# marvinli00/genie2

Hardware: AMD Instinct MI355X
Metric: denoise-steps/sec (N=256, T=1000, batch=8) (higher is better)
Workload: dtype f32 (pair-stack products as 3 f16 MFMAs on 2xf16-split operands, f32 accumulate); 1 GPU; unconditional N=256, T=1000, batch=8 per GPU, random-init base Denoiser (15.7M params), scale=0.6, reverse-loop steps 995..676; parallelism=replica per GPU x1, no data-path collective

## Files before the change

genie2_amd/csrc/common.h:

```cpp
#pragma once
#include <hip/hip_runtime.h>
#include <stdint.h>
#include "../../include/genie_hip.h"

typedef float f32x16 __attribute__((ext_vector_type(16)));
typedef float f32x4 __attribute__((ext_vector_type(4)));

#define GENIE_LN_EPS 1e-5f

#ifdef __HIPCC__

__device__ __forceinline__ f32x16 mfma_8k(const float4 a, const float4 b, f32x16 c) {
    c = __builtin_amdgcn_mfma_f32_32x32x2f32(a.x, b.x, c, 0, 0, 0);
    c = __builtin_amdgcn_mfma_f32_32x32x2f32(a.y, b.y, c, 0, 0, 0);
    c = __builtin_amdgcn_mfma_f32_32x32x2f32(a.z, b.z, c, 0, 0, 0);
    c = __builtin_amdgcn_mfma_f32_32x32x2f32(a.w, b.w, c, 0, 0, 0);
    return c;
}

__device__ __forceinline__ f32x16 zero16() {
    f32x16 z;
#pragma unroll
    for (int i = 0; i < 16; ++i) z[i] = 0.f;
    return z;
}

__device__ __forceinline__ int acc_row(int r, int lane) { return (r & 3) + 8 * (r >> 2) + 4 * (lane >> 5); }

__device__ __forceinline__ float4 wfrag(const float* __restrict__ wp, int KB, int nb, int kb, int lane) {
    return *reinterpret_cast<const float4*>(wp + ((size_t)(nb * KB + kb) * 64 + lane) * 4);
}

typedef float v4f __attribute__((ext_vector_type(4)));

__device__ __forceinline__ const float* wfrag_ptr(const float* __restrict__ wp, int KB, int nb, int kb, int lane) {
    return wp + ((size_t)(nb * KB + kb) * 64 + lane) * 4;
}
__device__ __forceinline__ void wf_issue(v4f& d, const float* p) {
    asm volatile("global_load_dwordx4 %0, %1, off" : "=v"(d) : "v"(p) : "memory");
}
template <int N>
__device__ __forceinline__ void wf_wait(v4f& a) {
    asm volatile("s_waitcnt vmcnt(%1)" : "+v"(a) : "i"(N) : "memory");
    __builtin_amdgcn_sched_barrier(0);
}
template <int N>
__device__ __forceinline__ void wf_wait(v4f& a, v4f& b) {
    asm volatile("s_waitcnt vmcnt(%2)" : "+v"(a), "+v"(b) : "i"(N) : "memory");
    __builtin_amdgcn_sched_barrier(0);
}
__device__ __forceinline__ f32x16 mfma_8k(const v4f a, const float4 b, f32x16 c) {
    c = __builtin_amdgcn_mfma_f32_32x32x2f32(a.x, b.x, c, 0, 0, 0);
    c = __builtin_amdgcn_mfma_f32_32x32x2f32(a.y, b.y, c, 0, 0, 0);
    c = __builtin_amdgcn_mfma_f32_32x32x2f32(a.z, b.z, c, 0, 0, 0);
    c = __builtin_amdgcn_mfma_f32_32x32x2f32(a.w, b.w, c, 0, 0, 0);
    return c;
}
__device__ __forceinline__ f32x16 mfma_8k(const float4 a, const v4f b, f32x16 c) {
    c = __builtin_amdgcn_mfma_f32_32x32x2f32(a.x, b.x, c, 0, 0, 0);
    c = __builtin_amdgcn_mfma_f32_32x32x2f32(a.y, b.y, c, 0, 0, 0);
    c = __builtin_amdgcn_mfma_f32_32x32x2f32(a.z, b.z, c, 0, 0, 0);
    c = __builtin_amdgcn_mfma_f32_32x32x2f32(a.w, b.w, c, 0, 0, 0);
    return c;
}

__device__ __forceinline__ float4 lfrag(const float* lds, int ld, int r0, int kb, int lane) {
    return *reinterpret_cast<const float4*>(lds + (r0 + (lane & 31)) * ld + kb * 8 + 4 * (lane >> 5));
}

__device__ __forceinline__ float4 lfrag_t(const float* lds, int ld, int i0, int kb, int lane) {
    const float* p = lds + (kb * 8 + 4 * (lane >> 5)) * ld + i0 + (lane & 31);
    return make_float4(p[0], p[ld], p[2 * ld], p[3 * ld]);
}

__device__ __forceinline__ float sigmoidf_(float x) { return 1.0f / (1.0f + expf(-x)); }

__device__ __forceinline__ void ln_rows_128(float* tile, int ld, const float* __restrict__ gamma,
                                            const float* __restrict__ beta, int tid) {
    const int row = tid >> 2, part = tid & 3;
    float* p = tile + row * ld + part * 32;
    float v[32];
#pragma unroll
    for (int q = 0; q < 8; ++q) {
        float4 t = *reinterpret_cast<float4*>(p + 4 * q);
        v[4 * q] = t.x; v[4 * q + 1] = t.y; v[4 * q + 2] = t.z; v[4 * q + 3] = t.w;
    }
    float s = 0.f;
#pragma unroll
    for (int q = 0; q < 32; ++q) s += v[q];
    s += __shfl_xor(s, 1); s += __shfl_xor(s, 2);
    const float mean = s * (1.0f / 128.0f);
    float ss = 0.f;
#pragma unroll
    for (int q = 0; q < 32; ++q) { float d = v[q] - mean; ss += d * d; }
    ss += __shfl_xor(ss, 1); ss += __shfl_xor(ss, 2);
    const float rstd = 1.0f / sqrtf(ss * (1.0f / 128.0f) + GENIE_LN_EPS);
#pragma unroll
    for (int q = 0; q < 8; ++q) {
        const int c = part * 32 + 4 * q;
        float4 g = *reinterpret_cast<const float4*>(gamma + c);
        float4 b = *reinterpret_cast<const float4*>(beta + c);
        float4 o;
        o.x = (v[4 * q] - mean) * rstd * g.x + b.x;
        o.y = (v[4 * q + 1] - mean) * rstd * g.y + b.y;
        o.z = (v[4 * q + 2] - mean) * rstd * g.z + b.z;
        o.w = (v[4 * q + 3] - mean) * rstd * g.w + b.w;
        *reinterpret_cast<float4*>(p + 4 * q) = o;
    }
}


__device__ __forceinline__ void rot_to_quat_dev(const float* r, int code, float* q) {
    const float xx = r[0], xy = r[1], xz = r[2], yx = r[3], yy = r[4], yz = r[5], zx = r[6], zy = r[7], zz = r[8];
    const float d0 = 1.f + xx + yy + zz, d1 = 1.f + xx - yy - zz, d2 = 1.f + yy - xx - zz, d3 = 1.f + zz - xx - yy;
    float c0, c1, c2, c3;
    if (d0 >= d1 && d0 >= d2 && d0 >= d3)      { c0 = d0;      c1 = zy - yz; c2 = xz - zx; c3 = yx - xy; }
    else if (d1 >= d2 && d1 >= d3)             { c0 = zy - yz; c1 = d1;      c2 = xy + yx; c3 = xz + zx; }
    else if (d2 >= d3)                         { c0 = xz - zx; c1 = xy + yx; c2 = d2;      c3 = yz + zy; }
    else                                       { c0 = yx - xy; c1 = xz + zx; c2 = yz + zy; c3 = d3; }
    const float inv = 1.0f / sqrtf(c0 * c0 + c1 * c1 + c2 * c2 + c3 * c3);
    q[0] = c0 * inv; q[1] = c1 * inv; q[2] = c2 * inv; q[3] = c3 * inv;
    if (code > 0) {
        const int m = (code - 1) >> 1;
        const bool want_neg = ((code - 1) & 1) != 0;
        const float comp = q[m];
        if ((comp < 0.f) != want_neg) { q[0] = -q[0]; q[1] = -q[1]; q[2] = -q[2]; q[3] = -q[3]; }
    }
}

#endif


enum KernelClass {
    KC_SINGLE_INPUT = 0, KC_GEMM_ROWS, KC_LAYERNORM, KC_PAIR_STATIC, KC_PAIR_INIT,
    KC_TRIMUL_PROJ, KC_TRIMUL_CONTRACT, KC_TRIMUL_OUT, KC_PAIR_TRANSITION,
    KC_IPA_BIAS, KC_IPA_PREP, KC_IPA_ATTN, KC_BB_UPDATE, KC_STRUCT_ROWS, KC_P_SAMPLE, KC_MISC, KC_PAIR_FUSED_A, KC_PAIR_FUSED_B,
    KC_TR_GEMM, KC_TR_EW, KC_TR_LN, KC_TR_TRANSPOSE, KC_TR_IPA, KC_TR_MISC,
    KC_TRIATT_PROJ, KC_TRIATT_CORE, KC_TRIATT_TRANSPOSE, KC_COUNT
};

struct HxTransW { const unsigned char* img; float *b1s, *b2s; float sx, c1, c2; };

struct HxTriW {
    const unsigned char *img_proj, *img_out;
    float *bias_proj, *bgs, *bzs;
    float sx, cpa, cpb, cg, cx, cgo, cz;
};
struct HxFusedW { const unsigned char* img; };
struct TriMulW {
    float *proj_w;
    float *proj_b;
    float *g_w, *g_b;
    float *z_w, *z_b;
    float *ln_in_g, *ln_in_b, *ln_out_g, *ln_out_b;
    HxTriW hx;
};
struct TriAttW {
    float *ln_g, *ln_b;
    float *wb;
    float *proj_w, *proj_b;
    float *out_w, *out_b;
    float sq, sk, sv;
};
struct PairLayerW {
    TriMulW out, in;
    TriAttW ta_start, ta_end;
    float *pt_ln_g, *pt_ln_b, *pt_w1, *pt_b1, *pt_w2, *pt_b2;
    HxTransW hx_pt;
    HxFusedW fa, fb;
};
struct StructLayerW {
    float *proj_w, *proj_b;
    float *head_w;
    float *out_w, *out_b;
    float *ln_ipa_g, *ln_ipa_b;
    float *t1_w, *t1_b, *t2_w, *t2_b, *t3_w, *t3_b;
    float *ln_tr_g, *ln_tr_b;
    float *bb_w, *bb_b;
};

struct HxGemmW { const float* w; const unsigned char* img; float inv_s; };

struct genie_train_ws;
struct genie_ctx {
    genie_dims_t d;
    genie_train_ws* train;
    int device;
    char err[512];

    bool have_weights;
    float* wdev;
    bool hx;
    unsigned char* hxdev;
    HxGemmW hxg[128]; int n_hxg;
    unsigned hx_launches;
    size_t wdev_floats;
    float *single_w;
    float *pij_w;
    float *relpos_t;
    float *templ_w;
    float *motif_w;
    float *ipa_bias_w, *ipa_bias_b;
    PairLayerW* pair;
    StructLayerW* st;

    bool have_tables;
    float *pos_tab, *chain_tab, *t_tab, *sched;
    int n_pos, n_chain;
    float* sched_host;

    int B, N, NP;
    bool have_feats, has_motif;
    int32_t *f_aatype, *f_rmask, *f_ridx, *f_cidx;
    float *f_pos;
    uint8_t *f_fsm, *f_fstm, *f_ifm;
    float *rmaskf;

    void* ws; size_t ws_bytes;
    float *p, *acm, *bcm, *xcm, *pstatic, *ipa_bias;
    float *spart;
    unsigned *pmax;
    float *xsingle, *s0, *s, *s1, *s2, *h1, *h2, *pij, *proj, *cat;
    float *kT, *v, *qp, *kpT, *vp;
    float *vf, *vmax;
    float *ta_tb, *ta_xn, *ta_qkvg;
    float *rots_w, *trans_w;
    int32_t* tsteps;
    float *loop_z;

    bool prof;
    struct ProfRec { int cls; hipEvent_t a, b; };
    ProfRec* prof_recs; int prof_n, prof_cap;
    double prof_ms[KC_COUNT]; int64_t prof_cnt[KC_COUNT];
    double train_gemm_flop;

    hipStream_t st2; hipEvent_t ev_fork, ev_join;
};

void launch_single_input(genie_ctx* h, hipStream_t st, const int32_t* timesteps);
void launch_gemm_rows(genie_ctx* h, hipStream_t st, const float* A, int lda, int M, int K,
                      const float* Wp, int Nout, const float* bias, const float* res, int ldr,
                      const float* rowmask, int relu, float* out, int ldo, int prof_class = KC_GEMM_ROWS);
void launch_layernorm_rows(genie_ctx* h, hipStream_t st, const float* in, float* out, int M, int C,
                           const float* g, const float* b);
void launch_pair_static(genie_ctx* h, hipStream_t st);
void launch_pair_init(genie_ctx* h, hipStream_t st, const float* trans, const float* rots,
                      const int8_t* codes);
void launch_trimul(genie_ctx* h, hipStream_t st, const TriMulW& w, bool outgoing);
void launch_pair_transition(genie_ctx* h, hipStream_t st, const PairLayerW& w);
void launch_triatt(genie_ctx* h, hipStream_t st, const TriAttW& w, bool starting);
void triatt_ws_floats(const genie_dims_t& d, int B, int N, size_t* tb, size_t* xn, size_t* qkvg);
bool launch_pair_stack_fused(genie_ctx* h, hipStream_t st, float* tap_trimul_out0, float* tap_layer0);
void launch_ipa_bias(genie_ctx* h, hipStream_t st);
void launch_ipa_prep(genie_ctx* h, hipStream_t st, int b0 = 0, int nb = -1);
void launch_ipa_attn(genie_ctx* h, hipStream_t st, int layer, const float* head_w, int b0 = 0, int nb = -1);
size_t ipa_vf_floats(const genie_dims_t& d, int B, int N);
bool ipa_attn_splits(const genie_ctx* h);
void launch_q_sample(genie_ctx* h, hipStream_t st, const float* x0, const float* z, const float* c0, const float* c1, float* trans_out);
void launch_training_loss(genie_ctx* h, hipStream_t st, const float* zp, const float* z, float w, float* losses, float* grad);
void launch_adam(hipStream_t st, size_t n, float* p, const float* g, float* m, float* v, double lr, double b1, double b2, double eps, int step);
void launch_any_nonzero(genie_ctx* h, hipStream_t st, const uint8_t* x, size_t n, unsigned* flag);
bool launch_struct_tail(genie_ctx* h, hipStream_t st, const StructLayerW& S, const float* trans_in, float* z_out, int b0 = 0, int nb = -1);
bool struct_tail_fused(const genie_ctx* h, const StructLayerW& S);
void launch_bb_update(genie_ctx* h, hipStream_t st, const StructLayerW& w, const float* trans_in,
                      float* z_out);
void launch_frenet(genie_ctx* h, hipStream_t st, int mode, int step, float scale, float* trans,
                   float* rots, const float* z, const float* eps);
void launch_reverse_step(genie_ctx* h, hipStream_t st, float a, float bz, float c_scaled, float* trans, float* rots, const float* z,
                         const float* eps);
void launch_fill_i32(genie_ctx* h, hipStream_t st, int32_t* p, int n, int v);
void train_ws_free(genie_ctx* h);

void prof_begin(genie_ctx* h, hipStream_t st, int cls);
void prof_end(genie_ctx* h, hipStream_t st);

struct ProfScope {
    genie_ctx* h; hipStream_t st; bool on;
    ProfScope(genie_ctx* h_, hipStream_t st_, int cls, bool enable = true) : h(h_), st(st_), on(enable && h_->prof) { if (on) prof_begin(h, st, cls); }
    ~ProfScope() { if (on) prof_end(h, st); }
};
```

genie2_amd/csrc/genie_api.hip:

```cpp
#include <stdio.h>
#include <stdlib.h>
#include <string.h>
#include <math.h>
#include <algorithm>
#include <cmath>
#include <new>
#include <string>
#include <vector>

#include "common.h"

void pair_kernels_init();
void pair_fused_kernels_init();
void single_kernels_init(const genie_dims_t& d, int n_max);
void launch_scale_copy(genie_ctx* h, hipStream_t st, const float* in, float* out, int n, float s);
size_t ipa_attn_lds(const genie_dims_t& d, int N);

static char g_create_err[512] = "";

void set_handle_free_error(const char* msg) { snprintf(g_create_err, sizeof g_create_err, "%s", msg); }

#define SET_ERR(h, ...) do { snprintf((h)->err, sizeof((h)->err), __VA_ARGS__); } while (0)
#define HIP_TRY(h, call) do { hipError_t e_ = (call); if (e_ != hipSuccess) { \
    SET_ERR(h, "%s failed: %s (%s:%d)", #call, hipGetErrorString(e_), __FILE__, __LINE__); return GENIE_E_HIP; } } while (0)

static const char* kKernelNames[KC_COUNT] = {
    "single_input", "gemm_rows", "layernorm_rows", "pair_static", "pair_init", "trimul_proj", "trimul_contract",
    "trimul_out", "pair_transition", "ipa_bias", "ipa_prep", "ipa_attn", "bb_update", "struct_rows", "p_sample_frenet", "misc",
    "pair_fused_a", "pair_fused_b", "train_gemm", "train_elementwise", "train_layernorm", "train_transpose", "train_ipa", "train_misc",
    "tri_att_proj", "tri_att_core", "tri_att_transpose"};

void prof_begin(genie_ctx* h, hipStream_t st, int cls) {
    if (h->prof_n == h->prof_cap) {
        const int nc = h->prof_cap ? h->prof_cap * 2 : 1024;
        h->prof_recs = (genie_ctx::ProfRec*)realloc(h->prof_recs, nc * sizeof(genie_ctx::ProfRec));
        h->prof_cap = nc;
    }
    genie_ctx::ProfRec& r = h->prof_recs[h->prof_n];
    r.cls = cls;
    (void)hipEventCreate(&r.a);
    (void)hipEventCreate(&r.b);
    (void)hipEventRecord(r.a, st);
}
void prof_end(genie_ctx* h, hipStream_t st) {
    (void)hipEventRecord(h->prof_recs[h->prof_n].b, st);
    h->prof_n++;
}

static int single_in(const genie_dims_t& d) { return d.c_pos_emb + d.c_chain_emb + d.c_timestep_emb + 23; }
static int ipa_proj_n(const genie_dims_t& d) {
    return d.n_head_ipa * (3 * d.c_hidden_ipa + 3 * d.n_qk_point + 3 * (d.n_qk_point + d.n_v_point));
}
static int ipa_cat_n(const genie_dims_t& d) { return d.n_head_ipa * (d.c_p + d.c_hidden_ipa + 4 * d.n_v_point); }

static const char* check_dims(const genie_dims_t& d) {
    if (d.c_p != 128 || d.c_hidden_mul != 128) return "kernels are specialised for c_p == c_hidden_mul == 128";
    if (d.c_s % 8 || d.c_s > 512) return "c_s must be a multiple of 8 and <= 512";
    if (d.template_dist_n_bin > 40 || d.template_dist_n_bin < 1) return "template_dist_n_bin must be in [1, 40]";
    if (d.n_head_ipa > 16) return "n_head_ipa must be <= 16";
    if (d.pair_transition_n < 1 || d.n_timestep < 1 || d.relpos_k < 0) return "bad dims";
    if (d.n_structure_layer < 1 || d.n_structure_block < 1 || d.n_pair_transform_layer < 0) return "bad layer counts";
    if ((d.n_head_ipa * d.c_hidden_ipa) % 4 || ipa_cat_n(d) % 4 || ipa_proj_n(d) % 4) return "IPA widths must be multiples of 4";
    if (d.n_head_tri < 0) return "n_head_tri must be >= 0";
    if (d.n_head_tri > 0 && d.c_hidden_tri_att != 16 && d.c_hidden_tri_att != 32) return "c_hidden_tri_att must be 16 or 32";
    if (d.n_head_tri > 0 && d.n_head_tri * d.c_hidden_tri_att != 128) return "n_head_tri * c_hidden_tri_att must be 128 (4 heads of 32 or 8 of 16)";
    return nullptr;
}

size_t genie_weight_count(const genie_dims_t* dp) {
    const genie_dims_t& d = *dp;
    size_t n = 0;
    const size_t cs = d.c_s, cp = d.c_p, ch = d.c_hidden_mul;
    n += cs * single_in(d);
    n += 2 * cp * cs + cp * (2 * d.relpos_k + 3) + cp * (d.template_dist_n_bin + 6) + cp * (d.template_dist_n_bin + 2);
    const size_t tm = 4 * (ch * cp + ch) + (cp * cp + cp) + (cp * ch + cp) + 2 * cp + 2 * ch;
    const size_t pt = 2 * cp + (d.pair_transition_n * cp * cp + d.pair_transition_n * cp) + (cp * d.pair_transition_n * cp + cp);
    const size_t hc = (size_t)d.n_head_tri * d.c_hidden_tri_att;
    const size_t ta = d.n_head_tri > 0 ? 2 * cp + d.n_head_tri * cp + 3 * hc * cp + (cp * hc + cp) + (hc * cp + hc) : 0;
    n += (size_t)d.n_pair_transform_layer * (2 * tm + 2 * ta + pt);
    const size_t H = d.n_head_ipa, C = d.c_hidden_ipa, Pq = d.n_qk_point, Pv = d.n_v_point;
    size_t sl = H;
    sl += (H * C) * cs + H * C + (2 * H * C) * cs + 2 * H * C + (3 * H * Pq) * cs + 3 * H * Pq + (3 * H * (Pq + Pv)) * cs + 3 * H * (Pq + Pv);
    sl += H * cp + H + cs * ipa_cat_n(d) + cs;
    sl += 2 * cs + 3 * (cs * cs + cs) + 2 * cs + 6 * cs + 6;
    n += (size_t)d.n_structure_layer * sl;
    return n;
}

int genie_create(const genie_dims_t* dims, int device, genie_handle_t* out) {
    if (!dims || !out) { snprintf(g_create_err, sizeof g_create_err, "genie_create: null argument"); return GENIE_E_ARG; }
    if (const char* m = check_dims(*dims)) { snprintf(g_create_err, sizeof g_create_err, "genie_create: %s", m); return GENIE_E_ARG; }
    int ndev = 0;
    if (hipGetDeviceCount(&ndev) != hipSuccess || device < 0 || device >= ndev) {
        snprintf(g_create_err, sizeof g_create_err, "genie_create: no HIP device %d (found %d)", device, ndev);
        return GENIE_E_HIP;
    }
    genie_ctx* h = new (std::nothrow) genie_ctx();
    if (!h) return GENIE_E_NOMEM;
    memset(h, 0, sizeof(*h));
    h->d = *dims;
    h->device = device;
    if (hipSetDevice(device) != hipSuccess) { delete h; snprintf(g_create_err, sizeof g_create_err, "hipSetDevice failed"); return GENIE_E_HIP; }
    h->pair = new PairLayerW[dims->n_pair_transform_layer > 0 ? dims->n_pair_transform_layer : 1]();
    h->st = new StructLayerW[dims->n_structure_layer]();
    pair_kernels_init();
    pair_fused_kernels_init();
    {
        const char* m = getenv("GENIE_MATH");
        h->hx = !(m && !strcmp(m, "f32"));
    }
    {
        int lo = 0, hi = 0;
        (void)hipDeviceGetStreamPriorityRange(&lo, &hi);
        if (hipStreamCreateWithPriority(&h->st2, hipStreamNonBlocking, hi) != hipSuccess) h->st2 = nullptr;
    }
    if (h->st2 && (hipEventCreateWithFlags(&h->ev_fork, hipEventDisableTiming) != hipSuccess ||
                   hipEventCreateWithFlags(&h->ev_join, hipEventDisableTiming) != hipSuccess)) {
        (void)hipStreamDestroy(h->st2);
        h->st2 = nullptr;
    }
    *out = h;
    return GENIE_OK;
}

static void free_batch(genie_ctx* h) {
    if (h->ws) { (void)hipFree(h->ws); h->ws = nullptr; h->ws_bytes = 0; }
    h->have_feats = false;
}

void genie_destroy(genie_handle_t h) {
    if (!h) return;
    (void)hipSetDevice(h->device);
    free_batch(h);
    train_ws_free(h);
    if (h->wdev) (void)hipFree(h->wdev);
    if (h->hxdev) (void)hipFree(h->hxdev);
    if (h->pos_tab) (void)hipFree(h->pos_tab);
    free(h->sched_host);
    for (int i = 0; i < h->prof_n; ++i) { (void)hipEventDestroy(h->prof_recs[i].a); (void)hipEventDestroy(h->prof_recs[i].b); }
    free(h->prof_recs);
    if (h->st2) { (void)hipStreamSynchronize(h->st2); (void)hipEventDestroy(h->ev_fork); (void)hipEventDestroy(h->ev_join); (void)hipStreamDestroy(h->st2); }
    delete[] h->pair;
    delete[] h->st;
    delete h;
}

const char* genie_last_error(genie_handle_t h) { return h ? h->err : g_create_err; }
size_t genie_workspace_bytes(genie_handle_t h) { return h ? h->ws_bytes : 0; }

namespace {
struct Img {
    std::vector<float> data;
    size_t add(size_t n) {
        const size_t off = (data.size() + 63) & ~(size_t)63;
        data.resize(off + n, 0.f);
        return off;
    }
    size_t raw(const float* src, size_t n) { const size_t o = add(n); memcpy(&data[o], src, n * sizeof(float)); return o; }
    size_t pack(const float* W, int rows, int cols) {
        const int NB = (rows + 31) / 32, KB = (cols + 7) / 8;
        const size_t o = add((size_t)NB * KB * 256);
        float* p = &data[o];
        for (int nb = 0; nb < NB; ++nb)
            for (int kb = 0; kb < KB; ++kb)
                for (int lane = 0; lane < 64; ++lane)
                    for (int e = 0; e < 4; ++e) {
                        const int r = nb * 32 + (lane & 31), k = kb * 8 + 4 * (lane >> 5) + e;
                        p[(((size_t)nb * KB + kb) * 64 + lane) * 4 + e] = (r < rows && k < cols) ? W[(size_t)r * cols + k] : 0.f;
                    }
        return o;
    }
};
uint16_t f2h(float f) {
    uint32_t x; memcpy(&x, &f, 4);
    const uint16_t sign = (uint16_t)((x >> 16) & 0x8000);
    x &= 0x7FFFFFFFu;
    if (x >= 0x7F800000u) return (uint16_t)(sign | (x > 0x7F800000u ? 0x7E00 : 0x7C00));
    if (x >= 0x477FF000u) return (uint16_t)(sign | 0x7C00);
    if (x < 0x38800000u) {
        float a; memcpy(&a, &x, 4);
        return (uint16_t)(sign | (uint16_t)nearbyintf(a * 16777216.0f));
    }
    const uint32_t mant = x & 0x7FFFFFu, rem = mant & 0x1FFFu;
    uint32_t r = (((x >> 23) - 112u) << 10) | (mant >> 13);
    if (rem > 0x1000u || (rem == 0x1000u && (r & 1u))) ++r;
    return (uint16_t)(sign | r);
}
float h2f(uint16_t v) {
    const int e = (v >> 10) & 31, m = v & 1023;
    float r = e == 0 ? ldexpf((float)m, -24) : e == 31 ? (m ? NAN : INFINITY) : ldexpf((float)(1024 + m), e - 25);
    return (v & 0x8000) ? -r : r;
}
float p2floor(double x) { return (x > 0 && std::isfinite(x)) ? (float)ldexp(1.0, (int)floor(log2(x))) : 1.0f; }
struct HxImg {
    std::vector<uint16_t> d;
    size_t begin() { d.resize((d.size() + 127) & ~(size_t)127); return d.size() * 2; }
    template <class F> void unit(F get) {
        const size_t o = d.size();
        d.resize(o + 1024);
        for (int lane = 0; lane < 64; ++lane)
            for (int e = 0; e < 8; ++e) {
                const float v = get(lane & 31, lane >> 5, e);
                const uint16_t hi = f2h(v);
                d[o + lane * 8 + e] = hi;
                d[o + 512 + lane * 8 + e] = f2h(v - h2f(hi));
            }
    }
};
double max_abs(const float* w, size_t n) { double m = 0; for (size_t i = 0; i < n; ++i) m = std::max(m, (double)fabsf(w[i])); return m; }
double hx_bound(const float* W, const float* b, int rows, int cols) {
    double m = 0;
    for (int r = 0; r < rows; ++r) {
        double ss = 0;
        for (int k = 0; k < cols; ++k) ss += (double)W[(size_t)r * cols + k] * W[(size_t)r * cols + k];
        m = std::max(m, sqrt(ss * cols) + fabs((double)b[r]));
    }
    return m;
}
constexpr float HX_SX = 1024.0f;

struct Cur {
    const float* p; size_t left;
    const float* take(size_t n) { if (n > left) { left = 0; return nullptr; } const float* r = p; p += n; left -= n; return r; }
};
void fold_ln(std::vector<float>& W, std::vector<float>& b, int rows, int cols, const float* g, const float* beta) {
    for (int r = 0; r < rows; ++r) {
        double acc = b[r];
        for (int k = 0; k < cols; ++k) acc += (double)W[(size_t)r * cols + k] * beta[k];
        b[r] = (float)acc;
        for (int k = 0; k < cols; ++k) W[(size_t)r * cols + k] *= g[k];
    }
}
std::vector<float> vcat(std::initializer_list<std::pair<const float*, size_t>> parts) {
    std::vector<float> v;
    for (auto& pr : parts) v.insert(v.end(), pr.first, pr.first + pr.second);
    return v;
}
}

int genie_load_weights(genie_handle_t h, const float* blob, size_t n_floats) {
    if (!h || !blob) return GENIE_E_ARG;
    const genie_dims_t& d = h->d;
    if (n_floats != genie_weight_count(&d)) {
        SET_ERR(h, "genie_load_weights: got %zu floats, dims need %zu", n_floats, genie_weight_count(&d));
        return GENIE_E_ARG;
    }
    HIP_TRY(h, hipSetDevice(h->device));
    const size_t cs = d.c_s, cp = d.c_p, ch = d.c_hidden_mul;
    Cur c{blob, n_floats};
    Img img;
    HxImg hx;
    std::vector<std::pair<float**, size_t>> fix;
    std::vector<std::pair<const unsigned char**, size_t>> hxfix;
    auto slot = [&](float** s, size_t off) { fix.push_back({s, off}); };
    struct GemmFix { float** slot; size_t hx_off; float inv_s; };
    std::vector<GemmFix> gfix;
    auto pack_gemm = [&](float** s, const float* W, int rows, int cols) {
        slot(s, img.pack(W, rows, cols));
        const float sw = p2floor(16384.0 / max_abs(W, (size_t)rows * cols));
        gfix.push_back({s, hx.begin(), 1.0f / sw});
        const int NB = (rows + 31) / 32, KC = (cols + 15) / 16;
        for (int nb = 0; nb < NB; ++nb)
            for (int kc = 0; kc < KC; ++kc)
                hx.unit([&](int j, int hh, int e) {
                    const int r = 32 * nb + j, k = 16 * kc + 8 * hh + e;
                    return (r < rows && k < cols) ? W[(size_t)r * cols + k] * sw : 0.f; });
    };

    size_t ones_off, zeros_off;
    {
        std::vector<float> one(512, 1.f), zero(512, 0.f);
        ones_off = img.raw(one.data(), one.size());
        zeros_off = img.raw(zero.data(), zero.size());
    }
    const int nsi = single_in(d);
    pack_gemm(&h->single_w, c.take(cs * nsi), (int)cs, nsi);
    {
        const float* wi = c.take(cp * cs);
        const float* wj = c.take(cp * cs);
        auto v = vcat({{wi, cp * cs}, {wj, cp * cs}});
        pack_gemm(&h->pij_w, v.data(), (int)(2 * cp), (int)cs);
    }
    {
        const int nr = 2 * d.relpos_k + 3;
        const float* w = c.take(cp * nr);
        std::vector<float> t((size_t)nr * cp);
        for (int o = 0; o < (int)cp; ++o) for (int k = 0; k < nr; ++k) t[(size_t)k * cp + o] = w[(size_t)o * nr + k];
        slot(&h->relpos_t, img.raw(t.data(), t.size()));
    }
    {
        const int kt = d.template_dist_n_bin + 6, km = d.template_dist_n_bin + 2;
        const float* wt = c.take(cp * kt);
        const float* wm = c.take(cp * km);
        std::vector<float> t((size_t)cp * 48, 0.f), m((size_t)cp * 48, 0.f);
        for (int o = 0; o < (int)cp; ++o) {
            for (int k = 0; k < kt; ++k) t[(size_t)o * 48 + k] = wt[(size_t)o * kt + k];
            for (int k = 0; k < km; ++k) m[(size_t)o * 48 + k] = wm[(size_t)o * km + k];
        }
        slot(&h->templ_w, img.pack(t.data(), (int)cp, 48));
        slot(&h->motif_w, img.pack(m.data(), (int)cp, 48));
    }
    struct TmSave { std::vector<float> w, gw, zw; float sp, sg, sgo, szo; };
    struct PtSave { std::vector<float> w1v, w2; float s1, s2; };
    std::vector<TmSave> tm_save(2 * (size_t)d.n_pair_transform_layer);
    std::vector<PtSave> pt_save(d.n_pair_transform_layer);
    for (int l = 0; l < d.n_pair_transform_layer; ++l) {
        PairLayerW& L = h->pair[l];
        for (int dir = 0; dir < 2; ++dir) {
            TriMulW& T = dir == 0 ? L.out : L.in;
            const float* ap_w = c.take(ch * cp); const float* ap_b = c.take(ch);
            const float* ag_w = c.take(ch * cp); const float* ag_b = c.take(ch);
            const float* bp_w = c.take(ch * cp); const float* bp_b = c.take(ch);
            const float* bg_w = c.take(ch * cp); const float* bg_b = c.take(ch);
            const float* g_w = c.take(cp * cp);  const float* g_b = c.take(cp);
            const float* z_w = c.take(cp * ch);  const float* z_b = c.take(cp);
            const float* li_g = c.take(cp); const float* li_b = c.take(cp);
            const float* lo_g = c.take(ch); const float* lo_b = c.take(ch);
            auto w = vcat({{ap_w, ch * cp}, {bp_w, ch * cp}, {ag_w, ch * cp}, {bg_w, ch * cp}});
            auto bb = vcat({{ap_b, ch}, {bp_b, ch}, {ag_b, ch}, {bg_b, ch}});
            fold_ln(w, bb, (int)(4 * ch), (int)cp, li_g, li_b);
            for (size_t r = 2 * ch; r < 4 * ch; ++r) {
                bb[r] = (float)(-1.4426950408889634 * bb[r]);
                for (size_t k = 0; k < cp; ++k) w[r * cp + k] = (float)(-1.4426950408889634 * w[r * cp + k]);
            }
            std::vector<float> gw(g_w, g_w + cp * cp), gb(g_b, g_b + cp), zw(z_w, z_w + cp * ch), zb(z_b, z_b + cp);
            fold_ln(gw, gb, (int)cp, (int)cp, li_g, li_b);
            for (size_t r = 0; r < cp; ++r) {
                gb[r] = (float)(-1.4426950408889634 * gb[r]);
                for (size_t k = 0; k < cp; ++k) gw[r * cp + k] = (float)(-1.4426950408889634 * gw[r * cp + k]);
            }
            fold_ln(zw, zb, (int)cp, (int)ch, lo_g, lo_b);
            slot(&T.proj_w, img.pack(w.data(), (int)(4 * ch), (int)cp));
            slot(&T.proj_b, img.raw(bb.data(), bb.size()));
            slot(&T.g_w, img.pack(gw.data(), (int)cp, (int)cp)); slot(&T.g_b, img.raw(gb.data(), cp));
            slot(&T.z_w, img.pack(zw.data(), (int)cp, (int)ch)); slot(&T.z_b, img.raw(zb.data(), cp));
            {
                HxTriW& X = T.hx;
                const float sp = p2floor(16384.0 / max_abs(w.data(), 2 * ch * cp)), sg = p2floor(16384.0 / max_abs(w.data() + 2 * ch * cp, 2 * ch * cp));
                const float sa = p2floor(32768.0 / hx_bound(w.data(), bb.data(), (int)ch, (int)cp));
                const float sb = p2floor(32768.0 / hx_bound(w.data() + ch * cp, bb.data() + ch, (int)ch, (int)cp));
                const float sgo = p2floor(16384.0 / max_abs(gw.data(), cp * cp)), szo = p2floor(16384.0 / max_abs(zw.data(), cp * ch));
                X.sx = HX_SX; X.cpa = sa / (HX_SX * sp); X.cpb = sb / (HX_SX * sp); X.cg = 1.0f / (HX_SX * sg); X.cx = 1.0f / (sa * sb);
                X.cgo = 1.0f / (HX_SX * sgo); X.cz = 1.0f / (HX_SX * szo);
                hxfix.push_back({&X.img_proj, hx.begin()});
                for (size_t pass = 0; pass < 8; ++pass)
                    for (int kc = 0; kc < 8; ++kc) {
                        hx.unit([&](int i, int hh, int e) { return w[(32 * pass + i) * cp + 16 * kc + 8 * hh + e] * sp; });
                        hx.unit([&](int i, int hh, int e) { return w[(2 * ch + 32 * pass + i) * cp + 16 * kc + 8 * hh + e] * sg; });
                    }
                hxfix.push_back({&X.img_out, hx.begin()});
                for (int st = 0; st < 4; ++st)
                    for (int obl = 0; obl < 2; ++obl)
                        for (int kc = 0; kc < 8; ++kc) {
                            const std::vector<float>& m = (st & 1) ? zw : gw;
                            const float sc = (st & 1) ? szo : sgo;
                            const size_t ob = 2 * (st >> 1) + obl;
                            hx.unit([&](int j, int hh, int e) { return m[(32 * ob + j) * cp + 16 * kc + 8 * hh + e] * sc; });
                        }
                std::vector<float> bp(4 * ch), bgs(cp), bzs(cp);
                for (size_t r = 0; r < 4 * ch; ++r) bp[r] = bb[r] * HX_SX * (r < 2 * ch ? sp : sg);
                for (size_t r = 0; r < cp; ++r) { bgs[r] = gb[r] * HX_SX * sgo; bzs[r] = zb[r] * HX_SX * szo; }
                slot(&X.bias_proj, img.raw(bp.data(), bp.size()));
                slot(&X.bgs, img.raw(bgs.data(), cp)); slot(&X.bzs, img.raw(bzs.data(), cp));
                tm_save[2 * l + dir] = TmSave{w, gw, zw, sp, sg, sgo, szo};
            }
            slot(&T.ln_in_g, ones_off); slot(&T.ln_in_b, zeros_off);
            slot(&T.ln_out_g, ones_off); slot(&T.ln_out_b, zeros_off);
        }
        for (int node = 0; node < (d.n_head_tri > 0 ? 2 : 0); ++node) {
            TriAttW& A = node == 0 ? L.ta_start : L.ta_end;
            const size_t hc = (size_t)d.n_head_tri * d.c_hidden_tri_att;
            const float* ln_g = c.take(cp); const float* ln_b = c.take(cp);
            const float* b_w = c.take(d.n_head_tri * cp);
            const float* q_w = c.take(hc * cp); const float* k_w = c.take(hc * cp); const float* v_w = c.take(hc * cp);
            const float* o_w = c.take(cp * hc); const float* o_b = c.take(cp);
            const float* g_w = c.take(hc * cp); const float* g_b = c.take(hc);
            if (!g_b) { SET_ERR(h, "genie_load_weights: blob too short"); return GENIE_E_ARG; }
            slot(&A.ln_g, img.raw(ln_g, cp)); slot(&A.ln_b, img.raw(ln_b, cp));
            slot(&A.wb, img.raw(b_w, d.n_head_tri * cp));
            auto w = vcat({{q_w, hc * cp}, {k_w, hc * cp}, {v_w, hc * cp}, {g_w, hc * cp}});
            std::vector<float> bv(4 * hc, 0.f);
            memcpy(&bv[3 * hc], g_b, hc * sizeof(float));
            pack_gemm(&A.proj_w, w.data(), (int)(4 * hc), (int)cp);
            slot(&A.proj_b, img.raw(bv.data(), bv.size()));
            pack_gemm(&A.out_w, o_w, (int)cp, (int)hc); slot(&A.out_b, img.raw(o_b, cp));
            auto scale_of = [&](const float* W) {
                std::vector<float> wf(W, W + hc * cp), bf(hc, 0.f);
                fold_ln(wf, bf, (int)hc, (int)cp, ln_g, ln_b);
                return p2floor(32768.0 / hx_bound(wf.data(), bf.data(), (int)hc, (int)cp));
            };
            A.sq = scale_of(q_w); A.sk = scale_of(k_w); A.sv = scale_of(v_w);
        }
        const size_t nh = (size_t)d.pair_transition_n * cp;
        const float* lg = c.take(cp); const float* lb = c.take(cp);
        const float* w1 = c.take(nh * cp); const float* b1 = c.take(nh);
        const float* w2 = c.take(cp * nh); const float* b2 = c.take(cp);
        {
            std::vector<float> w1v(w1, w1 + nh * cp), b1v(b1, b1 + nh);
            fold_ln(w1v, b1v, (int)nh, (int)cp, lg, lb);
            slot(&L.pt_ln_g, ones_off); slot(&L.pt_ln_b, zeros_off);
            slot(&L.pt_w1, img.pack(w1v.data(), (int)nh, (int)cp)); slot(&L.pt_b1, img.raw(b1v.data(), nh));
            HxTransW& X = L.hx_pt;
            const float s1 = p2floor(16384.0 / max_abs(w1v.data(), nh * cp)), s2 = p2floor(16384.0 / max_abs(w2, cp * nh));
            const float sh = p2floor(32768.0 / hx_bound(w1v.data(), b1v.data(), (int)nh, (int)cp));
            X.sx = HX_SX; X.c1 = sh / (HX_SX * s1); X.c2 = 1.0f / (sh * s2);
            hxfix.push_back({&X.img, hx.begin()});
            for (size_t hb = 0; hb < nh / 32; ++hb) {
                for (int kc = 0; kc < 8; ++kc)
                    hx.unit([&](int i, int hh, int e) { return w1v[(32 * hb + i) * cp + 16 * kc + 8 * hh + e] * s1; });
                for (int cc = 0; cc < 2; ++cc)
                    for (int ob = 0; ob < 4; ++ob)
                        hx.unit([&](int j, int hh, int e) {
                            return w2[(size_t)(32 * ob + j) * nh + 32 * hb + 16 * cc + (e & 3) + 8 * (e >> 2) + 4 * hh] * s2; });
            }
            std::vector<float> b1s(nh), b2s(cp);
            for (size_t r = 0; r < nh; ++r) b1s[r] = b1v[r] * HX_SX * s1;
            for (size_t r = 0; r < cp; ++r) b2s[r] = b2[r] * sh * s2;
            slot(&X.b1s, img.raw(b1s.data(), nh)); slot(&X.b2s, img.raw(b2s.data(), cp));
            pt_save[l] = PtSave{w1v, std::vector<float>(w2, w2 + cp * nh), s1, s2};
        }
        slot(&L.pt_w2, img.pack(w2, (int)cp, (int)nh)); slot(&L.pt_b2, img.raw(b2, cp));
    }
    {
        auto ck = [](int kc, int hh, int e) { return 16 * kc + (e & 3) + 8 * (e >> 2) + 4 * hh; };
        auto emit_O = [&](const TmSave& t) {
            for (int which = 0; which < 2; ++which)
                for (int st = 0; st < 2; ++st)
                    for (int obl = 0; obl < 2; ++obl)
                        for (int kc = 0; kc < 8; ++kc) {
                            const std::vector<float>& m = which == 0 ? t.zw : t.gw;
                            const float sc = which == 0 ? t.szo : t.sgo;
                            const size_t ob = 2 * st + obl;
                            hx.unit([&](int i, int hh, int e) { return m[(32 * ob + i) * cp + ck(kc, hh, e)] * sc; });
                        }
        };
        auto emit_T = [&](const PtSave& t) {
            const size_t nh = (size_t)d.pair_transition_n * cp;
            for (size_t hb = 0; hb < nh / 32; ++hb) {
                for (int kc = 0; kc < 8; ++kc)
                    hx.unit([&](int i, int hh, int e) { return t.w1v[(32 * hb + i) * cp + ck(kc, hh, e)] * t.s1; });
                for (int cc = 0; cc < 2; ++cc)
                    for (int ob = 0; ob < 4; ++ob)
                        hx.unit([&](int j, int hh, int e) { return t.w2[(size_t)(32 * ob + j) * nh + 32 * hb + ck(cc, hh, e)] * t.s2; });
            }
        };
        auto emit_P = [&](const TmSave& t) {
            for (size_t pass = 0; pass < 8; ++pass)
                for (int kc = 0; kc < 8; ++kc) {
                    hx.unit([&](int i, int hh, int e) { return t.w[(32 * pass + i) * cp + ck(kc, hh, e)] * t.sp; });
                    hx.unit([&](int i, int hh, int e) { return t.w[(2 * ch + 32 * pass + i) * cp + ck(kc, hh, e)] * t.sg; });
                }
        };
        for (int l = 0; l < d.n_pair_transform_layer; ++l) {
            hxfix.push_back({&h->pair[l].fa.img, hx.begin()});
            emit_O(tm_save[2 * l]); emit_P(tm_save[2 * l + 1]);
            hxfix.push_back({&h->pair[l].fb.img, hx.begin()});
            emit_O(tm_save[2 * l + 1]); emit_T(pt_save[l]);
            if (l + 1 < d.n_pair_transform_layer) emit_P(tm_save[2 * l + 2]);
        }
    }
    const size_t H = d.n_head_ipa, C = d.c_hidden_ipa, Pq = d.n_qk_point, Pv = d.n_v_point;
    const size_t ncat = ipa_cat_n(d);
    std::vector<float> wb_all, bb_all;
    for (int l = 0; l < d.n_structure_layer; ++l) {
        StructLayerW& S = h->st[l];
        const float* hw = c.take(H);
        const float* q_w = c.take(H * C * cs);            const float* q_b = c.take(H * C);
        const float* kv_w = c.take(2 * H * C * cs);       const float* kv_b = c.take(2 * H * C);
        const float* qp_w = c.take(3 * H * Pq * cs);      const float* qp_b = c.take(3 * H * Pq);
        const float* kp_w = c.take(3 * H * (Pq + Pv) * cs); const float* kp_b = c.take(3 * H * (Pq + Pv));
        const float* b_w = c.take(H * cp);                const float* b_b = c.take(H);
        const float* o_w = c.take(cs * ncat);             const float* o_b = c.take(cs);
        const float* li_g = c.take(cs); const float* li_b = c.take(cs);
        const float* t1w = c.take(cs * cs); const float* t1b = c.take(cs);
        const float* t2w = c.take(cs * cs); const float* t2b = c.take(cs);
        const float* t3w = c.take(cs * cs); const float* t3b = c.take(cs);
        const float* lt_g = c.take(cs); const float* lt_b = c.take(cs);
        const float* bw = c.take(6 * cs); const float* bbs = c.take(6);
        if (!bbs) { SET_ERR(h, "genie_load_weights: blob too short"); return GENIE_E_ARG; }
        slot(&S.head_w, img.raw(hw, H));
        auto w = vcat({{q_w, H * C * cs}, {kv_w, 2 * H * C * cs}, {qp_w, 3 * H * Pq * cs}, {kp_w, 3 * H * (Pq + Pv) * cs}});
        auto bv = vcat({{q_b, H * C}, {kv_b, 2 * H * C}, {qp_b, 3 * H * Pq}, {kp_b, 3 * H * (Pq + Pv)}});
        pack_gemm(&S.proj_w, w.data(), ipa_proj_n(d), (int)cs);
        slot(&S.proj_b, img.raw(bv.data(), bv.size()));
        wb_all.insert(wb_all.end(), b_w, b_w + H * cp);
        bb_all.insert(bb_all.end(), b_b, b_b + H);
        pack_gemm(&S.out_w, o_w, (int)cs, (int)ncat); slot(&S.out_b, img.raw(o_b, cs));
        slot(&S.ln_ipa_g, img.raw(li_g, cs)); slot(&S.ln_ipa_b, img.raw(li_b, cs));
        pack_gemm(&S.t1_w, t1w, (int)cs, (int)cs); slot(&S.t1_b, img.raw(t1b, cs));
        pack_gemm(&S.t2_w, t2w, (int)cs, (int)cs); slot(&S.t2_b, img.raw(t2b, cs));
        pack_gemm(&S.t3_w, t3w, (int)cs, (int)cs); slot(&S.t3_b, img.raw(t3b, cs));
        slot(&S.ln_tr_g, img.raw(lt_g, cs)); slot(&S.ln_tr_b, img.raw(lt_b, cs));
        slot(&S.bb_w, img.raw(bw, 6 * cs)); slot(&S.bb_b, img.raw(bbs, 6));
    }
    pack_gemm(&h->ipa_bias_w, wb_all.data(), (int)(d.n_structure_layer * H), (int)cp);
    slot(&h->ipa_bias_b, img.raw(bb_all.data(), bb_all.size()));
    if (c.left != 0) { SET_ERR(h, "genie_load_weights: %zu floats left over", c.left); return GENIE_E_ARG; }

    if (h->wdev) { (void)hipFree(h->wdev); h->wdev = nullptr; }
    img.add(64);
    HIP_TRY(h, hipMalloc((void**)&h->wdev, img.data.size() * sizeof(float)));
    HIP_TRY(h, hipMemcpy(h->wdev, img.data.data(), img.data.size() * sizeof(float), hipMemcpyHostToDevice));
    h->wdev_floats = img.data.size();
    for (auto& f : fix) *f.first = h->wdev + f.second;
    if (h->hxdev) { (void)hipFree(h->hxdev); h->hxdev = nullptr; }
    hx.begin();
    HIP_TRY(h, hipMalloc((void**)&h->hxdev, hx.d.size() * 2 + 256));
    HIP_TRY(h, hipMemcpy(h->hxdev, hx.d.data(), hx.d.size() * 2, hipMemcpyHostToDevice));
    for (auto& f : hxfix) *f.first = h->hxdev + f.second;
    h->n_hxg = 0;
    const int hxg_cap = (int)(sizeof(h->hxg) / sizeof(h->hxg[0]));
    if ((int)gfix.size() > hxg_cap) { SET_ERR(h, "genie_load_weights: %zu row-GEMM weights exceed the %d hx image slots", gfix.size(), hxg_cap); return GENIE_E_ARG; }
    for (auto& g : gfix) h->hxg[h->n_hxg++] = HxGemmW{*g.slot, h->hxdev + g.hx_off, g.inv_s};
    h->have_weights = true;
    return GENIE_OK;
}

int genie_set_tables(genie_handle_t h, const float* pos_tab, int n_pos, const float* chain_tab, int n_chain,
                     const float* t_tab, const float* sched) {
    if (!h || !pos_tab || !chain_tab || !t_tab || !sched || n_pos < 1 || n_chain < 1) return GENIE_E_ARG;
    HIP_TRY(h, hipSetDevice(h->device));
    const genie_dims_t& d = h->d;
    const size_t T1 = d.n_timestep + 1;
    const size_t a = (size_t)n_pos * d.c_pos_emb, b = (size_t)n_chain * d.c_chain_emb, c = T1 * d.c_timestep_emb, s = 4 * T1;
    if (h->pos_tab) (void)hipFree(h->pos_tab);
    HIP_TRY(h, hipMalloc((void**)&h->pos_tab, (a + b + c + s) * sizeof(float)));
    h->chain_tab = h->pos_tab + a;
    h->t_tab = h->chain_tab + b;
    h->sched = h->t_tab + c;
    HIP_TRY(h, hipMemcpy(h->pos_tab, pos_tab, a * sizeof(float), hipMemcpyHostToDevice));
    HIP_TRY(h, hipMemcpy(h->chain_tab, chain_tab, b * sizeof(float), hipMemcpyHostToDevice));
    HIP_TRY(h, hipMemcpy(h->t_tab, t_tab, c * sizeof(float), hipMemcpyHostToDevice));
    HIP_TRY(h, hipMemcpy(h->sched, sched, s * sizeof(float), hipMemcpyHostToDevice));
    free(h->sched_host);
    h->sched_host = (float*)malloc(s * sizeof(float));
    memcpy(h->sched_host, sched, s * sizeof(float));
    h->n_pos = n_pos;
    h->n_chain = n_chain;
    h->have_tables = true;
    return GENIE_OK;
}

__global__ void k_mask_to_float(const int32_t* m, float* f, int n) {
    const int i = blockIdx.x * blockDim.x + threadIdx.x;
    if (i < n) f[i] = (float)m[i];
}

int genie_prepare_features(genie_handle_t h, genie_stream_t stream, int B, int N, const genie_features_t* f) {
    if (!h || !f || B < 1 || N < 2) return GENIE_E_ARG;
    if (!h->have_weights) { SET_ERR(h, "genie_prepare_features: weights not loaded"); return GENIE_E_STATE; }
    const genie_dims_t& d = h->d;
    if (ipa_attn_lds(d, N) > 160 * 1024) { SET_ERR(h, "N = %d exceeds the attention kernel's LDS budget", N); return GENIE_E_ARG; }
    if ((size_t)24 * N * sizeof(float) > 160 * 1024) { SET_ERR(h, "N = %d exceeds the Frenet kernel's LDS budget (96 B per residue)", N); return GENIE_E_ARG; }
    {
        const size_t np = (size_t)((N + 31) / 32 * 32);
        const size_t pair_bytes = (size_t)B * np * np * d.c_p * sizeof(float);
        if (pair_bytes >= ((size_t)1 << 31)) {
            SET_ERR(h, "batch %d x N %d: a pair tensor of %zu bytes exceeds the 2 GiB the kernels address; split the batch", B, N, pair_bytes);
            return GENIE_E_ARG;
        }
    }
    HIP_TRY(h, hipSetDevice(h->device));
    hipStream_t st = (hipStream_t)stream;
    const int NP = (N + 31) / 32 * 32;
    const size_t M = (size_t)B * N, P = M * N;
    const size_t cs = d.c_s, cp = d.c_p;
    const int H = d.n_head_ipa, C = d.c_hidden_ipa, Pq = d.n_qk_point, Pv = d.n_v_point;
    const int ldx = (single_in(d) + 7) / 8 * 8;

    struct Seg { void** p; size_t bytes; };
    std::vector<Seg> segs;
    auto want = [&](void* pp, size_t bytes) { segs.push_back({(void**)pp, (bytes + 255) & ~(size_t)255}); };
    want(&h->p, P * cp * 4); want(&h->pstatic, P * cp * 4);
    want(&h->acm, (size_t)B * cp * NP * NP * 4); want(&h->bcm, (size_t)B * cp * NP * NP * 4); want(&h->xcm, (size_t)B * cp * NP * NP * 4);
    want(&h->ipa_bias, (size_t)d.n_structure_layer * H * P * 4);
    want(&h->xsingle, M * ldx * 4);
    want(&h->s0, M * cs * 4); want(&h->s, M * cs * 4); want(&h->s1, M * cs * 4); want(&h->s2, M * cs * 4);
    want(&h->h1, M * cs * 4); want(&h->h2, M * cs * 4);
    want(&h->pij, M * 2 * cp * 4); want(&h->proj, M * ipa_proj_n(d) * 4); want(&h->cat, M * ipa_cat_n(d) * 4);
    want(&h->kT, M * H * C * 4); want(&h->v, M * H * C * 4); want(&h->qp, M * H * Pq * 3 * 4);
    want(&h->kpT, M * H * Pq * 3 * 4); want(&h->vp, M * H * Pv * 3 * 4);
    want(&h->vf, ipa_vf_floats(d, B, N) * 4); want(&h->vmax, M * 2 * 4);
    want(&h->rots_w, M * 9 * 4); want(&h->trans_w, M * 3 * 4); want(&h->loop_z, M * 3 * 4);
    want(&h->tsteps, (size_t)B * 4); want(&h->rmaskf, M * 4); want(&h->pmax, 4); want(&h->spart, 3 * M * cs * 4);
    want(&h->f_aatype, M * 20 * 4); want(&h->f_rmask, M * 4); want(&h->f_ridx, M * 4); want(&h->f_cidx, M * 4);
    want(&h->f_pos, M * 3 * 4); want(&h->f_fsm, M); want(&h->f_fstm, P); want(&h->f_ifm, M);
    if (d.n_head_tri > 0) {
        size_t ntb, nxn, nq;
        triatt_ws_floats(d, B, N, &ntb, &nxn, &nq);
        want(&h->ta_tb, ntb * 4); want(&h->ta_xn, nxn * 4); want(&h->ta_qkvg, nq * 4);
    }
    size_t total = 0;
    for (auto& s : segs) total += s.bytes;
    if (total > h->ws_bytes) {
        free_batch(h);
        hipError_t e = hipMalloc(&h->ws, total);
        if (e != hipSuccess) { SET_ERR(h, "workspace hipMalloc(%zu MB) failed: %s", total >> 20, hipGetErrorString(e)); return GENIE_E_NOMEM; }
        h->ws_bytes = total;
    }
    size_t off = 0;
    for (auto& s : segs) { *s.p = (char*)h->ws + off; off += s.bytes; }
    h->B = B; h->N = N; h->NP = NP;

    HIP_TRY(h, hipMemcpyAsync(h->f_aatype, f->aatype, M * 20 * 4, hipMemcpyDeviceToDevice, st));
    HIP_TRY(h, hipMemcpyAsync(h->f_pos, f->atom_positions, M * 3 * 4, hipMemcpyDeviceToDevice, st));
    HIP_TRY(h, hipMemcpyAsync(h->f_rmask, f->residue_mask, M * 4, hipMemcpyDeviceToDevice, st));
    HIP_TRY(h, hipMemcpyAsync(h->f_ridx, f->residue_index, M * 4, hipMemcpyDeviceToDevice, st));
    HIP_TRY(h, hipMemcpyAsync(h->f_cidx, f->chain_index, M * 4, hipMemcpyDeviceToDevice, st));
    HIP_TRY(h, hipMemcpyAsync(h->f_fsm, f->fixed_sequence_mask, M, hipMemcpyDeviceToDevice, st));
    HIP_TRY(h, hipMemcpyAsync(h->f_fstm, f->fixed_structure_mask, P, hipMemcpyDeviceToDevice, st));
    HIP_TRY(h, hipMemcpyAsync(h->f_ifm, f->interface_mask, M, hipMemcpyDeviceToDevice, st));
    hipLaunchKernelGGL(k_mask_to_float, dim3((unsigned)((M + 255) / 256)), dim3(256), 0, st, h->f_rmask, h->rmaskf, (int)M);
    HIP_TRY(h, hipMemsetAsync(h->acm, 0, (size_t)B * cp * NP * NP * 4, st));
    HIP_TRY(h, hipMemsetAsync(h->vf, 0, ipa_vf_floats(d, B, N) * 4, st));
    HIP_TRY(h, hipMemsetAsync(h->bcm, 0, (size_t)B * cp * NP * NP * 4, st));
    single_kernels_init(d, N);
    {
        unsigned any = 0;
        HIP_TRY(h, hipMemsetAsync(h->pmax, 0, sizeof(unsigned), st));
        launch_any_nonzero(h, st, h->f_fstm, P, h->pmax);
        HIP_TRY(h, hipMemcpyAsync(&any, h->pmax, sizeof(unsigned), hipMemcpyDeviceToHost, st));
        HIP_TRY(h, hipStreamSynchronize(st));
        h->has_motif = any != 0;
    }
    launch_pair_static(h, st);
    HIP_TRY(h, hipGetLastError());
    h->have_feats = true;
    return GENIE_OK;
}

static int denoise_internal(genie_ctx* h, hipStream_t st, const float* trans, const float* rots, const int32_t* ts_dev,
                            const int8_t* codes, float* z_out, const genie_taps_t* taps) {
    const genie_dims_t& d = h->d;
    const int B = h->B, N = h->N, M = B * N;
    const size_t P = (size_t)M * N;
    const int cs = d.c_s, cp = d.c_p;
    const int ldx = (single_in(d) + 7) / 8 * 8;
    auto d2d = [&](void* dst, const void* src, size_t bytes) { return hipMemcpyAsync(dst, src, bytes, hipMemcpyDeviceToDevice, st); };

    h->hx_launches = 1;
    launch_scale_copy(h, st, trans, h->trans_w, M * 3, d.rescale);
    HIP_TRY(h, d2d(h->rots_w, rots, (size_t)M * 9 * 4));

    launch_single_input(h, st, ts_dev);
    launch_gemm_rows(h, st, h->xsingle, ldx, M, ldx, h->single_w, cs, nullptr, nullptr, 0, h->rmaskf, 0, h->s0, cs);
    if (taps && taps->s) HIP_TRY(h, d2d(taps->s, h->s0, (size_t)M * cs * 4));

    launch_gemm_rows(h, st, h->s0, cs, M, cs, h->pij_w, 2 * cp, nullptr, nullptr, 0, nullptr, 0, h->pij, 2 * cp);
    launch_pair_init(h, st, h->trans_w, h->rots_w, codes);
    if (taps && taps->p_init) HIP_TRY(h, d2d(taps->p_init, h->p, P * cp * 4));

    const bool fused = launch_pair_stack_fused(h, st, taps ? taps->p_trimul_out0 : nullptr, taps ? taps->p_layer0 : nullptr);
    for (int l = 0; l < (fused ? 0 : d.n_pair_transform_layer); ++l) {
        launch_trimul(h, st, h->pair[l].out, true);
        if (l == 0 && taps && taps->p_trimul_out0) HIP_TRY(h, d2d(taps->p_trimul_out0, h->p, P * cp * 4));
        launch_trimul(h, st, h->pair[l].in, false);
        if (d.n_head_tri > 0) {
            launch_triatt(h, st, h->pair[l].ta_start, true);
            launch_triatt(h, st, h->pair[l].ta_end, false);
            if (l == 0 && taps && taps->p_tri_att0) HIP_TRY(h, d2d(taps->p_tri_att0, h->p, P * cp * 4));
        }
        launch_pair_transition(h, st, h->pair[l]);
        if (l == 0 && taps && taps->p_layer0) HIP_TRY(h, d2d(taps->p_layer0, h->p, P * cp * 4));
    }
    if (taps && taps->p) HIP_TRY(h, d2d(taps->p, h->p, P * cp * 4));

    launch_ipa_bias(h, st);
    HIP_TRY(h, d2d(h->s, h->s0, (size_t)M * cs * 4));
    if (taps && taps->states) HIP_TRY(h, d2d(taps->states, h->s0, (size_t)M * cs * 4));
    int n_state = 1;
    const int nproj = ipa_proj_n(d), ncat = ipa_cat_n(d);
    bool split = h->st2 && B >= 2 && M >= 1024 && ipa_attn_splits(h) && !getenv("GENIE_NO_STRUCT_SPLIT");
    for (int l = 0; split && l < d.n_structure_layer; ++l) split = struct_tail_fused(h, h->st[l]);
    const int n_half = split ? 2 : 1;
    const int n_layers = d.n_structure_block * d.n_structure_layer;
    hipStream_t hstream[2] = {st, h->st2};
    if (split) {
        HIP_TRY(h, hipEventRecord(h->ev_fork, st));
        HIP_TRY(h, hipStreamWaitEvent(h->st2, h->ev_fork, 0));
    }
    for (int half = 0; half < n_half; ++half) {
        hipStream_t hs = hstream[half];
        const int b0 = (int)((long long)B * half / n_half), nb = (int)((long long)B * (half + 1) / n_half) - b0;
        const size_t r0 = (size_t)b0 * N, nr = (size_t)nb * N;
        int li = 0;
        for (int blk = 0; blk < d.n_structure_block; ++blk) {
            for (int l = 0; l < d.n_structure_layer; ++l, ++li) {
                const StructLayerW& S = h->st[l];
                const bool last = li == n_layers - 1;
                launch_gemm_rows(h, hs, h->s + r0 * cs, cs, (int)nr, cs, S.proj_w, nproj, S.proj_b, nullptr, 0, nullptr, 0, h->proj + r0 * nproj, nproj);
                launch_ipa_prep(h, hs, b0, nb);
                launch_ipa_attn(h, hs, l, S.head_w, b0, nb);
                if (li == 0 && taps && taps->ipa_cat0) HIP_TRY(h, hipMemcpyAsync(taps->ipa_cat0 + r0 * ncat, h->cat + r0 * ncat, nr * ncat * 4, hipMemcpyDeviceToDevice, hs));
                auto state_tap = [&]() -> hipError_t {
                    return (taps && taps->states) ? hipMemcpyAsync(taps->states + (size_t)(1 + li) * M * cs + r0 * cs, h->s + r0 * cs, nr * cs * 4, hipMemcpyDeviceToDevice, hs)
                                                  : hipSuccess;
                };
                if (launch_struct_tail(h, hs, S, last ? trans : nullptr, last ? z_out : nullptr, b0, nb)) { HIP_TRY(h, state_tap()); continue; }
                launch_gemm_rows(h, hs, h->cat, ncat, M, ncat, S.out_w, cs, S.out_b, h->s, cs, nullptr, 0, h->s1, cs);
                launch_layernorm_rows(h, hs, h->s1, h->s2, M, cs, S.ln_ipa_g, S.ln_ipa_b);
                launch_gemm_rows(h, hs, h->s2, cs, M, cs, S.t1_w, cs, S.t1_b, nullptr, 0, nullptr, 1, h->h1, cs);
                launch_gemm_rows(h, hs, h->h1, cs, M, cs, S.t2_w, cs, S.t2_b, nullptr, 0, nullptr, 1, h->h2, cs);
                launch_gemm_rows(h, hs, h->h2, cs, M, cs, S.t3_w, cs, S.t3_b, h->s2, cs, nullptr, 0, h->s1, cs);
                launch_layernorm_rows(h, hs, h->s1, h->s, M, cs, S.ln_tr_g, S.ln_tr_b);
                launch_bb_update(h, hs, S, last ? trans : nullptr, last ? z_out : nullptr);
                HIP_TRY(h, state_tap());
            }
        }
    }
    if (split) {
        for (int q = 1; q < n_half; ++q) {
            HIP_TRY(h, hipEventRecord(h->ev_join, hstream[q]));
            HIP_TRY(h, hipStreamWaitEvent(st, h->ev_join, 0));
        }
    }
    (void)n_state;
    if (taps && taps->s_final) HIP_TRY(h, d2d(taps->s_final, h->s, (size_t)M * cs * 4));
    if (taps && taps->rots_out) HIP_TRY(h, d2d(taps->rots_out, h->rots_w, (size_t)M * 9 * 4));
    if (taps && taps->trans_out) launch_scale_copy(h, st, h->trans_w, taps->trans_out, M * 3, 1.0f / d.rescale);
    HIP_TRY(h, hipGetLastError());
    return GENIE_OK;
}

static int check_ready(genie_ctx* h, const char* who) {
    if (!h) return GENIE_E_ARG;
    if (!h->have_weights || !h->have_tables || !h->have_feats) {
        SET_ERR(h, "%s: call genie_load_weights, genie_set_tables and genie_prepare_features first", who);
        return GENIE_E_STATE;
    }
    if (hipSetDevice(h->device) != hipSuccess) { SET_ERR(h, "hipSetDevice failed"); return GENIE_E_HIP; }
    return GENIE_OK;
}

int genie_denoise(genie_handle_t h, genie_stream_t stream, const float* trans, const float* rots, const int32_t* timesteps,
                  const int8_t* quat_codes, float* z_out, const genie_taps_t* taps) {
    if (int rc = check_ready(h, "genie_denoise")) return rc;
    if (!trans || !rots || !timesteps || !z_out) { SET_ERR(h, "genie_denoise: null tensor"); return GENIE_E_ARG; }
    return denoise_internal(h, (hipStream_t)stream, trans, rots, timesteps, quat_codes, z_out, taps);
}

int genie_frenet(genie_handle_t h, genie_stream_t stream, const float* trans, float* rots_out) {
    if (!h || !h->have_feats) { if (h) SET_ERR(h, "genie_frenet: no batch bound"); return h ? GENIE_E_STATE : GENIE_E_ARG; }
    if (!trans || !rots_out) return GENIE_E_ARG;
    HIP_TRY(h, hipSetDevice(h->device));
    launch_frenet(h, (hipStream_t)stream, 0, 0, 0.f, const_cast<float*>(trans), rots_out, nullptr, nullptr);
    HIP_TRY(h, hipGetLastError());
    return GENIE_OK;
}

int genie_adam_step(genie_stream_t stream, size_t n, float* p, const float* g, float* m, float* v, double lr, double beta1, double beta2,
                    double eps, int step) {
    if (!p || !g || !m || !v || step < 1) return GENIE_E_ARG;
    if (n == 0) return GENIE_OK;
    launch_adam((hipStream_t)stream, n, p, g, m, v, lr, beta1, beta2, eps, step);
    return hipGetLastError() == hipSuccess ? GENIE_OK : GENIE_E_HIP;
}

int genie_q_sample(genie_handle_t h, genie_stream_t stream, const float* x0, const float* z, const float* c_x0, const float* c_z,
                   float* trans_out, float* rots_out) {
    if (!h || !h->have_feats) { if (h) SET_ERR(h, "genie_q_sample: no batch bound"); return h ? GENIE_E_STATE : GENIE_E_ARG; }
    if (!x0 || !z || !c_x0 || !c_z || !trans_out || !rots_out) { SET_ERR(h, "genie_q_sample: null tensor"); return GENIE_E_ARG; }
    HIP_TRY(h, hipSetDevice(h->device));
    launch_q_sample(h, (hipStream_t)stream, x0, z, c_x0, c_z, trans_out);
    launch_frenet(h, (hipStream_t)stream, 0, 0, 0.f, trans_out, rots_out, nullptr, nullptr);
    HIP_TRY(h, hipGetLastError());
    return GENIE_OK;
}

int genie_training_loss(genie_handle_t h, genie_stream_t stream, const float* z_pred, const float* z, float condition_loss_weight,
                        float* losses_out, float* grad_out) {
    if (!h || !h->have_feats) { if (h) SET_ERR(h, "genie_training_loss: no batch bound"); return h ? GENIE_E_STATE : GENIE_E_ARG; }
    if (!z_pred || !z || !losses_out) { SET_ERR(h, "genie_training_loss: null tensor"); return GENIE_E_ARG; }
    HIP_TRY(h, hipSetDevice(h->device));
    launch_training_loss(h, (hipStream_t)stream, z_pred, z, condition_loss_weight, losses_out, grad_out);
    HIP_TRY(h, hipGetLastError());
    return GENIE_OK;
}

int genie_p_sample(genie_handle_t h, genie_stream_t stream, int step, float scale, float* trans_inout, float* rots_out,
                   const float* z, const float* eps) {
    if (int rc = check_ready(h, "genie_p_sample")) return rc;
    if (step < 1 || step > h->d.n_timestep || !trans_inout || !rots_out || !z) { SET_ERR(h, "genie_p_sample: bad argument"); return GENIE_E_ARG; }
    launch_frenet(h, (hipStream_t)stream, 1, step, scale, trans_inout, rots_out, z, eps);
    HIP_TRY(h, hipGetLastError());
    return GENIE_OK;
}

int genie_sample_loop(genie_handle_t h, genie_stream_t stream, float scale, const float* noise, const int8_t* quat_codes,
                      int first_step, int last_step, float* trans_io, float* rots_io, float* record) {
    if (int rc = check_ready(h, "genie_sample_loop")) return rc;
    const int T = h->d.n_timestep;
    if (!noise || !trans_io || !rots_io || first_step > T || last_step < 1 || first_step < last_step) {
        SET_ERR(h, "genie_sample_loop: bad argument");
        return GENIE_E_ARG;
    }
    hipStream_t st = (hipStream_t)stream;
    const size_t n3 = (size_t)h->B * h->N * 3, nn = (size_t)h->B * h->N * h->N;
    if (first_step == T) {
        HIP_TRY(h, hipMemcpyAsync(trans_io, noise, n3 * 4, hipMemcpyDeviceToDevice, st));
        launch_frenet(h, st, 0, 0, 0.f, trans_io, rots_io, nullptr, nullptr);
    }
    int it = 0;
    for (int step = first_step; step >= last_step; --step, ++it) {
        launch_fill_i32(h, st, h->tsteps, h->B, step);
        const int8_t* codes = quat_codes ? quat_codes + (size_t)it * nn : nullptr;
        if (int rc = denoise_internal(h, st, trans_io, rots_io, h->tsteps, codes, h->loop_z, nullptr)) return rc;
        const float* eps = (step == 1) ? nullptr : noise + (size_t)(T - step + 1) * n3;
        launch_frenet(h, st, 1, step, scale, trans_io, rots_io, h->loop_z, eps);
        if (record) HIP_TRY(h, hipMemcpyAsync(record + (size_t)it * n3, trans_io, n3 * 4, hipMemcpyDeviceToDevice, st));
    }
    HIP_TRY(h, hipGetLastError());
    return GENIE_OK;
}

int genie_reverse_step(genie_handle_t h, genie_stream_t stream, float a, float bz, float c_scaled, float* trans_inout, float* rots_out,
                       const float* z, const float* eps) {
    if (int rc = check_ready(h, "genie_reverse_step")) return rc;
    if (!trans_inout || !rots_out || !z) { SET_ERR(h, "genie_reverse_step: null tensor"); return GENIE_E_ARG; }
    if (!std::isfinite(a) || !std::isfinite(bz) || !std::isfinite(c_scaled)) {
        SET_ERR(h, "genie_reverse_step: non-finite coefficient (a = %g, bz = %g, c_scaled = %g)", a, bz, c_scaled);
        return GENIE_E_ARG;
    }
    launch_reverse_step(h, (hipStream_t)stream, a, bz, c_scaled, trans_inout, rots_out, z, eps);
    HIP_TRY(h, hipGetLastError());
    return GENIE_OK;
}

int genie_sample_loop_steps(genie_handle_t h, genie_stream_t stream, int n_iter, const int32_t* steps, const float* coef, const float* noise,
                            const int8_t* quat_codes, int start_from_noise, float* trans_io, float* rots_io, float* record) {
    if (int rc = check_ready(h, "genie_sample_loop_steps")) return rc;
    const int T = h->d.n_timestep;
    if (n_iter < 1) { SET_ERR(h, "genie_sample_loop_steps: n_iter = %d, needs at least 1", n_iter); return GENIE_E_ARG; }
    if (!steps || !coef || !trans_io || !rots_io) { SET_ERR(h, "genie_sample_loop_steps: null steps, coef, trans_io or rots_io"); return GENIE_E_ARG; }
    if (!noise && (start_from_noise || n_iter > 1)) {
        SET_ERR(h, "genie_sample_loop_steps: null noise (needed for the initial state and for every iteration but the last)");
        return GENIE_E_ARG;
    }
    for (int i = 0; i < n_iter; ++i) {
        if (steps[i] < 1 || steps[i] > T) { SET_ERR(h, "genie_sample_loop_steps: steps[%d] = %d outside 1..%d", i, steps[i], T); return GENIE_E_ARG; }
        if (i && steps[i] >= steps[i - 1]) {
            SET_ERR(h, "genie_sample_loop_steps: steps not strictly decreasing (steps[%d] = %d after %d)", i, steps[i], steps[i - 1]);
            return GENIE_E_ARG;
        }
        for (int k = 0; k < 3; ++k)
            if (!std::isfinite(coef[3 * i + k])) { SET_ERR(h, "genie_sample_loop_steps: non-finite coefficient coef[%d][%d]", i, k); return GENIE_E_ARG; }
    }
    hipStream_t st = (hipStream_t)stream;
    const size_t n3 = (size_t)h->B * h->N * 3, nn = (size_t)h->B * h->N * h->N;
    if (start_from_noise) {
        HIP_TRY(h, hipMemcpyAsync(trans_io, noise, n3 * 4, hipMemcpyDeviceToDevice, st));
        launch_frenet(h, st, 0, 0, 0.f, trans_io, rots_io, nullptr, nullptr);
    }
    for (int it = 0; it < n_iter; ++it) {
        launch_fill_i32(h, st, h->tsteps, h->B, steps[it]);
        const int8_t* codes = quat_codes ? quat_codes + (size_t)it * nn : nullptr;
        if (int rc = denoise_internal(h, st, trans_io, rots_io, h->tsteps, codes, h->loop_z, nullptr)) return rc;
        const float* eps = (it == n_iter - 1) ? nullptr : noise + (size_t)(it + 1) * n3;
        launch_reverse_step(h, st, coef[3 * it], coef[3 * it + 1], coef[3 * it + 2], trans_io, rots_io, h->loop_z, eps);
        if (record) HIP_TRY(h, hipMemcpyAsync(record + (size_t)it * n3, trans_io, n3 * 4, hipMemcpyDeviceToDevice, st));
    }
    HIP_TRY(h, hipGetLastError());
    return GENIE_OK;
}

int genie_set_math(genie_handle_t h, int mode) {
    if (!h || (mode != GENIE_MATH_F32 && mode != GENIE_MATH_HX)) return GENIE_E_ARG;
    h->hx = mode == GENIE_MATH_HX;
    return GENIE_OK;
}
int genie_get_math(genie_handle_t h) { return h && h->hx ? GENIE_MATH_HX : GENIE_MATH_F32; }

int genie_profile_enable(genie_handle_t h, int enable) {
    if (!h) return GENIE_E_ARG;
    h->prof = enable != 0;
    return GENIE_OK;
}

int genie_profile_read(genie_handle_t h, const char** names, double* total_ms, int64_t* launches, int cap) {
    if (!h) return GENIE_E_ARG;
    (void)hipSetDevice(h->device);
    for (int i = 0; i < h->prof_n; ++i) {
        genie_ctx::ProfRec& r = h->prof_recs[i];
        (void)hipEventSynchronize(r.b);
        float ms = 0.f;
        if (hipEventElapsedTime(&ms, r.a, r.b) == hipSuccess) { h->prof_ms[r.cls] += ms; h->prof_cnt[r.cls] += 1; }
        (void)hipEventDestroy(r.a);
        (void)hipEventDestroy(r.b);
    }
    h->prof_n = 0;
    int n = 0;
    for (int k = 0; k < KC_COUNT && n < cap; ++k) {
        if (names) names[n] = kKernelNames[k];
        if (total_ms) total_ms[n] = h->prof_ms[k];
        if (launches) launches[n] = h->prof_cnt[k];
        ++n;
    }
    for (int k = 0; k < KC_COUNT; ++k) { h->prof_ms[k] = 0; h->prof_cnt[k] = 0; }
    return n;
}
```

genie2_amd/csrc/hx_fused.h:

```cpp
#pragma once
#include "hx_pair.h"

#define FZ_SB_BZ 0
#define FZ_SB_BG 128
#define FZ_SB_B1 256
#define FZ_SB_B2 768
#define FZ_SB_BP 896
#define FZ_SB_FLOATS 1408
#define FZ_OOR 0x7FFFFFF0
#define FZ_COMPILER_FENCE() asm volatile("" ::: "memory")

struct FusedArgs {
    float* z; const float* xcm; const float* rmask; const unsigned char* wimg;
    const float *bzs, *bgs, *b1s, *b2s, *bproj;
    unsigned *acm, *bcm;
    int N, NP, n_wtiles, n_hb;
    unsigned cm_bytes, z_bytes;
    float sx, cgo, cz, c1, c2, inv_c2, cpa, cpb, cg;
    int rev;
};

__device__ __forceinline__ void fz_zt_read(float4 (&raw)[16], const unsigned char* zt, int pl, int h, int half) {
#pragma unroll
    for (int q = 0; q < 4; ++q) {
        const int g = 4 * q + h;
        raw[2 * (4 * half + q)] = *reinterpret_cast<const float4*>(zt + pl * 256 + ((g ^ (pl & 15)) << 4));
        raw[2 * (4 * half + q) + 1] = *reinterpret_cast<const float4*>(zt + pl * 256 + (((g + 2) ^ (pl & 15)) << 4));
    }
}

__device__ __forceinline__ void fz_zt_chunk(float4& a, float4& b, const unsigned char* zt, int pl, int h, int q) {
    const int g = 4 * q + h;
    a = *reinterpret_cast<const float4*>(zt + pl * 256 + ((g ^ (pl & 15)) << 4));
    b = *reinterpret_cast<const float4*>(zt + pl * 256 + (((g + 2) ^ (pl & 15)) << 4));
}

__device__ __forceinline__ void fz_store_half(rsrc_t rz, unsigned char* zt, const f32x16& v0, const f32x16& v1, int lane, int soff,
                                              int row_stride, int nvalid, int hf) {
    const int pl = lane & 31, h = lane >> 5;
    FZ_COMPILER_FENCE();
#pragma unroll
    for (int q = 0; q < 4; ++q) {
        const f32x16& v = (q < 2) ? v0 : v1;
        const int r0 = 8 * (q & 1);
        const int g = 4 * q + h;
        *reinterpret_cast<float4*>(zt + pl * 256 + ((g ^ (pl & 15)) << 4)) = make_float4(v[r0], v[r0 + 1], v[r0 + 2], v[r0 + 3]);
        *reinterpret_cast<float4*>(zt + pl * 256 + (((g + 2) ^ (pl & 15)) << 4)) = make_float4(v[r0 + 4], v[r0 + 5], v[r0 + 6], v[r0 + 7]);
    }
    hx_lds_done();
#pragma unroll
    for (int j = 0; j < 8; ++j) {
        const int r = 4 * j + (lane >> 4);
        u32x4 d = *reinterpret_cast<const u32x4*>(zt + j * 1024 + lane * 16);
        const int g = (lane & 15) ^ (r & 15);
        const int voff = r < nvalid ? r * row_stride + (g << 4) : FZ_OOR;
        __builtin_amdgcn_raw_buffer_store_b128(d, rz, voff, soff + hf * 256, 0);
        asm volatile("s_nop 1" : "+v"(d) : : "memory");
    }
    FZ_COMPILER_FENCE();
}

__device__ __forceinline__ void fz_stats(const f32x16 (&v)[4], float sx, float& mean, float& sc) {
    float s = 0.f;
#pragma unroll
    for (int ob = 0; ob < 4; ++ob)
#pragma unroll
        for (int r = 0; r < 16; ++r) s += v[ob][r];
    s += __shfl_xor(s, 32);
    mean = s * (1.0f / 128.0f);
    float ss = 0.f;
#pragma unroll
    for (int ob = 0; ob < 4; ++ob)
#pragma unroll
        for (int r = 0; r < 16; ++r) { const float d = v[ob][r] - mean; ss += d * d; }
    ss += __shfl_xor(ss, 32);
    sc = sx / sqrtf(ss * (1.0f / 128.0f) + GENIE_LN_EPS);
}
__device__ __forceinline__ void fz_split_tile(h8 (&zh)[8], h8 (&zl)[8], const f32x16 (&v)[4], float mean, float sc) {
#pragma unroll
    for (int c = 0; c < 8; ++c) {
        float x[8];
#pragma unroll
        for (int e = 0; e < 8; ++e) x[e] = v[c >> 1][8 * (c & 1) + e] - mean;
        hx_split8(x, sc, zh[c], zl[c]);
    }
}
```

genie2_amd/csrc/pair_fused_kernels.hip:

```cpp
#include <string.h>
#include "hx_fused.h"

#define FZ_LDS_BYTES (2 * HX_STAGE_BYTES + 6144 + 8 * HX_ZT_BYTES)

template <bool COL, bool HAS_T, bool HAS_P = true>
__global__ __launch_bounds__(512, 1) void k_pair_fused(const FusedArgs A) {
    extern __shared__ __attribute__((aligned(16))) unsigned char smb[];
    float* sb = reinterpret_cast<float*>(smb + 2 * HX_STAGE_BYTES);
    const int lane = threadIdx.x & 63, wave = UNI(threadIdx.x >> 6);
    const int h = lane >> 5, pl = lane & 31;
    const int N = A.N, NP = A.NP, n_wtiles = A.n_wtiles;
    const int ntile = (N + 31) >> 5;
    const int n_tiles = (n_wtiles + 7) / 8;
    const int rev = A.rev;
    const int n_hb = HAS_T ? A.n_hb : 0;
    const int PBASE = 4 + n_hb;
    const rsrc_t rw = hx_rsrc(A.wimg, (unsigned)((PBASE + (HAS_P ? 8 : 0)) * HX_STAGE_BYTES));
    const rsrc_t rx = hx_rsrc(A.xcm, A.cm_bytes), rz = hx_rsrc(A.z, A.z_bytes);
    const rsrc_t ra = hx_rsrc(A.acm, A.cm_bytes), rb = hx_rsrc(A.bcm, A.cm_bytes);
    const int lane16 = lane * 16;
    const int sstride = NP * NP * 4;
    const int zstride = COL ? N * 512 : 512;
    auto issue = [&](int s, int buf) {
        if (wave >= 4) {
#pragma unroll
            for (int q = 0; q < 8; ++q) {
                const int p = 8 * (wave - 4) + q;
                hx_dma(rw, smb + buf * HX_STAGE_BYTES + p * 1024, lane16, s * HX_STAGE_BYTES + p * 1024);
            }
        }
    };
    unsigned char* zt = smb + 2 * HX_STAGE_BYTES + 6144 + wave * HX_ZT_BYTES;
    auto tile_geom = [&](int tile, int& zsoff, int& nv, int& cmoff) {
        const int wt = min(HX_PHYS(tile) * 8 + wave, n_wtiles - 1);
        const int st = wt % ntile, line = (wt / ntile) % N, b = wt / (ntile * N);
        nv = min(32, N - st * 32);
        zsoff = COL ? ((b * N + st * 32) * N + line) * 512 : ((b * N + line) * N + st * 32) * 512;
        cmoff = ((b * 128 * NP + line) * NP + st * 32) * 4;
    };
    const int vx = (4 * h * NP * NP + pl) * 4;
#define FZ_XLOAD(c, xoff) do {                                                                                              \
        raw[2 * (c)].x = hx_load(rx, vx, (xoff) + (16 * (c) + 0) * sstride); raw[2 * (c)].y = hx_load(rx, vx, (xoff) + (16 * (c) + 1) * sstride); \
        raw[2 * (c)].z = hx_load(rx, vx, (xoff) + (16 * (c) + 2) * sstride); raw[2 * (c)].w = hx_load(rx, vx, (xoff) + (16 * (c) + 3) * sstride); \
        raw[2 * (c) + 1].x = hx_load(rx, vx, (xoff) + (16 * (c) + 8) * sstride); raw[2 * (c) + 1].y = hx_load(rx, vx, (xoff) + (16 * (c) + 9) * sstride); \
        raw[2 * (c) + 1].z = hx_load(rx, vx, (xoff) + (16 * (c) + 10) * sstride); raw[2 * (c) + 1].w = hx_load(rx, vx, (xoff) + (16 * (c) + 11) * sstride); \
    } while (0)

    int tile = blockIdx.x;
    issue(0, 0);
    for (int u = threadIdx.x; u < FZ_SB_FLOATS; u += 512) {
        float v = 0.f;
        if (u < FZ_SB_BG) v = A.bzs[u];
        else if (u < FZ_SB_B1) v = A.bgs[u - FZ_SB_BG];
        else if (u < FZ_SB_B2) { if (HAS_T && u - FZ_SB_B1 < n_hb * 32) v = A.b1s[u - FZ_SB_B1]; }
        else if (u < FZ_SB_BP) { if (HAS_T) v = A.b2s[u - FZ_SB_B2]; }
        else if (HAS_P) v = A.bproj[u - FZ_SB_BP];
        sb[u] = v;
    }
    float4 raw[16];
    {
        int zs, nv, cm;
        tile_geom(tile, zs, nv, cm);
        hx_zt_dma(rz, zt, lane, zs, zstride, nv, 1);
    }
    hx_stage_landed();
    __syncthreads();

#pragma unroll 1
    for (; tile < n_tiles; tile += gridDim.x) {
        const int wt_raw = HX_PHYS(tile) * 8 + wave;
        const bool act = wt_raw < n_wtiles;
        const int wt = act ? wt_raw : n_wtiles - 1;
        const int st = wt % ntile, line = (wt / ntile) % N, b = wt / (ntile * N);
        const int t0i = st * 32;
        const int nvalid = act ? min(32, N - t0i) : 0;
        int zsoff, znv, cmoff;
        tile_geom(tile, zsoff, znv, cmoff);
        int bo = 0;
        asm volatile("" : "+v"(bo));
        const float* sbt = sb + bo;
        int lane_t = lane;
        asm volatile("" : "+v"(lane_t));
        const int pl_t = lane_t & 31, h_t = lane_t >> 5;
#pragma unroll
        for (int c = 0; c < 8; ++c) FZ_XLOAD(c, cmoff);
        const float msk = (pl < nvalid) ? A.rmask[b * N + line] * A.rmask[b * N + t0i + pl] : 0.f;
        const bool more = tile + (int)gridDim.x < n_tiles;
        int n_zsoff = 0, n_nv = 1, n_cmoff = 0;
        if (more) tile_geom(tile + gridDim.x, n_zsoff, n_nv, n_cmoff);
        hx_vm_done();
        f32x16 v[4];

        {
            h8 xh[8], xl[8];
            hx_norm_split(xh, xl, raw, A.sx);
            PIPE_FENCE();
            float4 rz1[8];
            float zsh = 0.f, zs1 = 0.f, zs2 = 0.f;
#pragma unroll
            for (int half = 0; half < 2; ++half) {
                issue(half + 1, half ^ 1);
                const unsigned char* stage = smb + half * HX_STAGE_BYTES;
#pragma unroll
                for (int r = 0; r < 16; ++r) {
                    v[2 * half][r] = sbt[FZ_SB_BZ + (2 * half) * 32 + acc_row(r, lane)];
                    v[2 * half + 1][r] = sbt[FZ_SB_BZ + (2 * half + 1) * 32 + acc_row(r, lane)];
                }
                h8 f0 = hx_frag(stage, 0, 0, lane), f0l = hx_frag(stage, 0, 1, lane), f1 = hx_frag(stage, 8, 0, lane),
                   f1l = hx_frag(stage, 8, 1, lane);
#pragma unroll
                for (int kc = 0; kc < 8; ++kc) {
                    const int kn = min(kc + 1, 7);
                    const h8 n0 = hx_frag(stage, kn, 0, lane), n0l = hx_frag(stage, kn, 1, lane), n1 = hx_frag(stage, 8 + kn, 0, lane),
                             n1l = hx_frag(stage, 8 + kn, 1, lane);
                    PIPE_FENCE();
                    MFH3(f0, f0l, xh[kc], xl[kc], v[2 * half]);
                    MFH3(f1, f1l, xh[kc], xl[kc], v[2 * half + 1]);
                    PIPE_FENCE();
                    f0 = n0; f0l = n0l; f1 = n1; f1l = n1l;
                    if (half == 0 && kc == 0) {
#pragma unroll
                        for (int q = 0; q < 4; ++q) fz_zt_chunk(rz1[2 * q], rz1[2 * q + 1], zt, pl_t, h_t, q);
                    }
                    if (half == 0 && kc == 2) { hx_lds_done(); hx_zt_dma(rz, zt, lane_t, zsoff, zstride, znv, 0); }
                    if (half == 1 && kc == 1) {
                        zsh = __shfl(rz1[0].x, lane & 31);
#pragma unroll
                        for (int q = 0; q < 8; ++q) {
                            const float a = rz1[q].x - zsh, bq = rz1[q].y - zsh, c = rz1[q].z - zsh, d = rz1[q].w - zsh;
                            zs1 += (a + bq) + (c + d); zs2 += (a * a + bq * bq) + (c * c + d * d);
                        }
                    }
                    if (half == 1 && kc >= 2 && kc <= 5) {
                        float4 ta, tb;
                        fz_zt_chunk(ta, tb, zt, pl_t, h_t, kc - 2);
                        const float a = ta.x - zsh, bq = ta.y - zsh, c = ta.z - zsh, d = ta.w - zsh;
                        const float e = tb.x - zsh, f = tb.y - zsh, g = tb.z - zsh, hh = tb.w - zsh;
                        zs1 += ((a + bq) + (c + d)) + ((e + f) + (g + hh));
                        zs2 += ((a * a + bq * bq) + (c * c + d * d)) + ((e * e + f * f) + (g * g + hh * hh));
                    }
                }
                hx_stage_landed();
                hx_stage_barrier();
            }
            zs1 += __shfl_xor(zs1, 32); zs2 += __shfl_xor(zs2, 32);
            const float zm_s = zs1 * (1.0f / 128.0f);
            const float zmean = zsh + zm_s;
            const float zsc = A.sx / sqrtf(fmaxf(zs2 * (1.0f / 128.0f) - zm_s * zm_s, 0.f) + GENIE_LN_EPS);
#pragma unroll
            for (int half = 0; half < 2; ++half) {
                if (half == 0) issue(3, 1);
                else issue(4, 0);
                const unsigned char* stage = smb + half * HX_STAGE_BYTES;
                f32x16 ga, gb;
#pragma unroll
                for (int r = 0; r < 16; ++r) {
                    ga[r] = sbt[FZ_SB_BG + (2 * half) * 32 + acc_row(r, lane)];
                    gb[r] = sbt[FZ_SB_BG + (2 * half + 1) * 32 + acc_row(r, lane)];
                }
                h8 f0 = hx_frag(stage, 0, 0, lane), f0l = hx_frag(stage, 0, 1, lane), f1 = hx_frag(stage, 8, 0, lane),
                   f1l = hx_frag(stage, 8, 1, lane);
#pragma unroll
                for (int kc = 0; kc < 8; ++kc) {
                    const int kn = min(kc + 1, 7);
                    const h8 n0 = hx_frag(stage, kn, 0, lane), n0l = hx_frag(stage, kn, 1, lane), n1 = hx_frag(stage, 8 + kn, 0, lane),
                             n1l = hx_frag(stage, 8 + kn, 1, lane);
                    float4 ca, cb;
                    if (kc < 4) fz_zt_chunk(ca, cb, zt, pl_t, h_t, kc);
                    else { ca = rz1[2 * (kc - 4)]; cb = rz1[2 * (kc - 4) + 1]; }
                    const float xz[8] = {ca.x - zmean, ca.y - zmean, ca.z - zmean, ca.w - zmean, cb.x - zmean, cb.y - zmean, cb.z - zmean, cb.w - zmean};
                    h8 sh, sl;
                    hx_split8(xz, zsc, sh, sl);
                    PIPE_FENCE();
                    MFH3(f0, f0l, sh, sl, ga);
                    MFH3(f1, f1l, sh, sl, gb);
                    PIPE_FENCE();
                    f0 = n0; f0l = n0l; f1 = n1; f1l = n1l;
                }
                float4 res[8];
                if (half == 0) {
#pragma unroll
                    for (int q = 0; q < 4; ++q) fz_zt_chunk(res[2 * q], res[2 * q + 1], zt, pl_t, h_t, q);
                } else {
#pragma unroll
                    for (int q = 0; q < 8; ++q) res[q] = rz1[q];
                }
#pragma unroll
                for (int r = 0; r < 16; ++r) {
                    const float g0 = A.cz * __builtin_amdgcn_rcpf(1.0f + __builtin_amdgcn_exp2f(ga[r] * A.cgo));
                    const float g1 = A.cz * __builtin_amdgcn_rcpf(1.0f + __builtin_amdgcn_exp2f(gb[r] * A.cgo));
                    const float4 za = res[2 * (r >> 3) + ((r & 7) >> 2)], zb = res[2 * (2 + (r >> 3)) + ((r & 7) >> 2)];
                    const float z0 = (r & 3) == 0 ? za.x : (r & 3) == 1 ? za.y : (r & 3) == 2 ? za.z : za.w;
                    const float z1 = (r & 3) == 0 ? zb.x : (r & 3) == 1 ? zb.y : (r & 3) == 2 ? zb.z : zb.w;
                    v[2 * half][r] = fmaf(v[2 * half][r], g0, z0);
                    v[2 * half + 1][r] = fmaf(v[2 * half + 1][r], g1, z1);
                }
                hx_stage_landed();
                hx_stage_barrier();
            }
        }

        h8 zh[8], zl[8];
        if constexpr (HAS_T) {
            float mean, sc;
            fz_stats(v, A.sx, mean, sc);
            fz_split_tile(zh, zl, v, mean, sc);
#pragma unroll
            for (int ob = 0; ob < 4; ++ob)
#pragma unroll
                for (int r = 0; r < 16; ++r) v[ob][r] = fmaf(v[ob][r], A.inv_c2, sbt[FZ_SB_B2 + ob * 32 + acc_row(r, lane)]);
            f32x16 d;
#pragma unroll
            for (int r = 0; r < 16; ++r) d[r] = sbt[FZ_SB_B1 + acc_row(r, lane)];
            auto t_stage = [&](int hb) {
                if (HAS_P || hb + 1 < n_hb) issue(4 + hb + 1, (hb + 1) & 1);
                else if (more) issue(0, 0);
                const unsigned char* stage = smb + (hb & 1) * HX_STAGE_BYTES;
                {
                    h8 wh = hx_frag(stage, 0, 0, lane), wl = hx_frag(stage, 0, 1, lane);
#pragma unroll
                    for (int kc = 0; kc < 8; ++kc) {
                        const h8 nh = hx_frag(stage, min(kc + 1, 7), 0, lane), nl = hx_frag(stage, min(kc + 1, 7), 1, lane);
                        PIPE_FENCE();
                        MFH3(wh, wl, zh[kc], zl[kc], d);
                        PIPE_FENCE();
                        wh = nh; wl = nl;
                    }
                }
                h8 ah[2], al[2];
#pragma unroll
                for (int c = 0; c < 2; ++c) {
                    float x[8];
#pragma unroll
                    for (int e = 0; e < 8; ++e) x[e] = fmaxf(d[8 * c + e], 0.f);
                    hx_split8(x, A.c1, ah[c], al[c]);
                }
                {
                    h8 bh = hx_frag(stage, 8, 0, lane), bl = hx_frag(stage, 8, 1, lane);
#pragma unroll
                    for (int u = 0; u < 8; ++u) {
                        const h8 nh = hx_frag(stage, 8 + min(u + 1, 7), 0, lane), nl = hx_frag(stage, 8 + min(u + 1, 7), 1, lane);
                        PIPE_FENCE();
                        MFH3(bh, bl, ah[u >> 2], al[u >> 2], v[u & 3]);
                        PIPE_FENCE();
                        bh = nh; bl = nl;
                        if (u == 1) {
#pragma unroll
                            for (int r = 0; r < 16; ++r) d[r] = sbt[FZ_SB_B1 + (hb + 1) * 32 + acc_row(r, lane)];
                        }
                    }
                }
                hx_stage_landed();
                hx_stage_barrier();
            };
#pragma unroll 1
            for (int hb = 0; hb < n_hb; ++hb) t_stage(hb);
            const float m2 = msk * A.c2;
#pragma unroll
            for (int ob = 0; ob < 4; ++ob)
#pragma unroll
                for (int r = 0; r < 16; ++r) v[ob][r] *= m2;
        }

        fz_store_half(rz, zt, v[0], v[1], lane_t, zsoff, zstride, nvalid, 0);
        FZ_COMPILER_FENCE();
        fz_store_half(rz, zt, v[2], v[3], lane_t, zsoff, zstride, nvalid, 1);
        FZ_COMPILER_FENCE();
        if constexpr (HAS_P) {
            float mean, sc;
            fz_stats(v, A.sx, mean, sc);
            fz_split_tile(zh, zl, v, mean, sc);
        }
        hx_lds_done();
        if constexpr (!HAS_P) {
            if (more) hx_zt_dma(rz, zt, lane_t, n_zsoff, zstride, n_nv, 1);
        }

        if constexpr (HAS_P) {
            const float* sbias = sbt + FZ_SB_BP;
            const float cg = A.cg;
            const float ma = msk * A.cpa, mb = msk * A.cpb;
            const int voff = (pl < nvalid) ? (4 * h * NP * NP + pl) * 4 : FZ_OOR;
            const int sbase = ((b * 128 * NP + line) * NP + t0i) * 4;
            unsigned wst[8];
            f32x16 apA, agA, apB, agB;
#pragma unroll
            for (int r = 0; r < 16; ++r) { apB[r] = 0.f; agB[r] = 0.f; apA[r] = sbias[acc_row(r, lane)]; agA[r] = sbias[256 + acc_row(r, lane)]; }
#pragma unroll 1
            for (int pp = 0; pp < 4; ++pp) {
                {
                    const int pass = 2 * pp;
                    issue(PBASE + pass + 1, 1);
                    const unsigned char* stage = smb;
                    const rsrc_t e_rd = pp > 2 ? rb : ra;
                    const int e_voff = pp == 0 ? FZ_OOR : voff;
                    const int e_so = sbase + ((pass - 1) & 3) * 32 * sstride;
                    const float e_pm = pp > 2 ? mb : ma;
                    HX_PROJ_STAGE(apA, agA, apB, agB);
                    asm volatile("s_waitcnt vmcnt(16)" ::: "memory");
                    if (more) {
                        if (pp == 2) hx_zt_dma(rz, zt, lane_t, n_zsoff, zstride, n_nv, 1, 0, 4);
                    }
                    hx_stage_barrier();
                }
                {
                    const int pass = 2 * pp + 1;
                    if (pp < 3) issue(PBASE + pass + 1, 0);
                    else if (more) issue(0, 0);
                    const unsigned char* stage = smb + HX_STAGE_BYTES;
                    const rsrc_t e_rd = pp < 2 ? ra : rb;
                    const int e_voff = voff;
                    const int e_so = sbase + ((pass - 1) & 3) * 32 * sstride;
                    const float e_pm = pp < 2 ? ma : mb;
                    HX_PROJ_STAGE(apB, agB, apA, agA);
                    asm volatile("s_waitcnt vmcnt(16)" ::: "memory");
                    if (more) {
                        if (pp == 2) hx_zt_dma(rz, zt, lane_t, n_zsoff, zstride, n_nv, 1, 4, 4);
                    }
                    hx_stage_barrier();
                }
            }
            {
                const rsrc_t e_rd = rb;
                const int e_voff = voff, e_so = sbase + 3 * 32 * sstride;
                const float e_pm = mb;
                float t[16], u[16];
#pragma unroll
                for (int r = 0; r < 16; ++r) {
                    HX_PROJ_PIECE_A(agB, r, t[r]);
                    HX_PROJ_PIECE_B(apB, r, t[r], u[r]);
                }
                PIPE_FENCE();
#pragma unroll
                for (int r = 0; r < 16; ++r) HX_PROJ_PIECE_C_NOW(r, t[r], u[r]);
            }
        }
    }
#undef FZ_XLOAD
}

static int fz_num_cu() {
    static int n = 0;
    if (!n) { int dev = 0; hipDeviceProp_t pr; (void)hipGetDevice(&dev); (void)hipGetDeviceProperties(&pr, dev); n = pr.multiProcessorCount > 0 ? pr.multiProcessorCount : 256; }
    return n;
}

void pair_fused_kernels_init() {
    (void)hipFuncSetAttribute(reinterpret_cast<const void*>(k_pair_fused<true, false>), hipFuncAttributeMaxDynamicSharedMemorySize, FZ_LDS_BYTES);
    (void)hipFuncSetAttribute(reinterpret_cast<const void*>(k_pair_fused<false, true>), hipFuncAttributeMaxDynamicSharedMemorySize, FZ_LDS_BYTES);
    (void)hipFuncSetAttribute(reinterpret_cast<const void*>(k_pair_fused<false, true, false>), hipFuncAttributeMaxDynamicSharedMemorySize, FZ_LDS_BYTES);
}

void launch_pair_fused(genie_ctx* h, hipStream_t st, const HxFusedW& f, const HxTriW& o, const HxTransW* t, const HxTriW* pp, bool col) {
    const HxTriW& p = pp ? *pp : o;
    const int N = h->N, NP = h->NP, ntile = (N + 31) / 32;
    FusedArgs a;
    a.z = h->p; a.xcm = h->xcm; a.rmask = h->rmaskf; a.wimg = f.img;
    a.bzs = o.bzs; a.bgs = o.bgs; a.b1s = t ? t->b1s : nullptr; a.b2s = t ? t->b2s : nullptr; a.bproj = p.bias_proj;
    a.acm = reinterpret_cast<unsigned*>(h->acm); a.bcm = reinterpret_cast<unsigned*>(h->bcm);
    a.N = N; a.NP = NP; a.n_wtiles = h->B * N * ntile; a.n_hb = t ? h->d.pair_transition_n * 4 : 0;
    a.cm_bytes = (unsigned)((size_t)h->B * 128 * NP * NP * 4);
    a.z_bytes = (unsigned)((size_t)h->B * N * N * 512);
    a.sx = o.sx; a.cgo = o.cgo; a.cz = o.cz;
    a.c1 = t ? t->c1 : 0.f; a.c2 = t ? t->c2 : 1.f; a.inv_c2 = t ? 1.0f / t->c2 : 1.f;
    a.cpa = p.cpa; a.cpb = p.cpb; a.cg = p.cg;
    a.rev = (int)(h->hx_launches++ & 1);
    const long long n_tiles = ((long long)a.n_wtiles + 7) / 8;
    const unsigned grid = (unsigned)(n_tiles < fz_num_cu() ? n_tiles : fz_num_cu());
    if (!pp) hipLaunchKernelGGL((k_pair_fused<false, true, false>), dim3(grid), dim3(512), FZ_LDS_BYTES, st, a);
    else if (col) hipLaunchKernelGGL((k_pair_fused<true, false>), dim3(grid), dim3(512), FZ_LDS_BYTES, st, a);
    else hipLaunchKernelGGL((k_pair_fused<false, true>), dim3(grid), dim3(512), FZ_LDS_BYTES, st, a);
}
```

genie2_amd/csrc/pair_hx_kernels.hip:

```cpp
#include "hx_pair.h"


template <int NW>
__global__ __launch_bounds__(NW * 64, NW == 8 ? 1 : 2) void k_pair_transition_hx(
    float* __restrict__ z, const float* __restrict__ rmask, const unsigned char* __restrict__ wimg,
    const float* __restrict__ b1s, const float* __restrict__ b2s, int N, long long M, int n_hb, float sx, float c1, float c2, int rev) {
    extern __shared__ __attribute__((aligned(16))) unsigned char smb[];
    float* sb1 = reinterpret_cast<float*>(smb + 2 * HX_STAGE_BYTES);
    const int lane = threadIdx.x & 63, wave = UNI(threadIdx.x >> 6);
    const int h = lane >> 5, pl = lane & 31;
    const int n_wt = (int)((M + 31) / 32);
    const int n_tiles = (n_wt + NW - 1) / NW;
    const rsrc_t rw = hx_rsrc(wimg, (unsigned)(n_hb * HX_STAGE_BYTES));
    const rsrc_t rz = hx_rsrc(z, (unsigned)(M * 512));
    const rsrc_t rnull = hx_rsrc(z, 0u);
    const int lane16 = lane * 16;
    constexpr int PW = 32 / NW;
    auto issue = [&](int hb, int buf) {
#pragma unroll
        for (int q = 0; q < PW; ++q) {
            const int p = PW * wave + q;
            hx_dma(rw, smb + buf * HX_STAGE_BYTES + p * 1024, lane16, hb * HX_STAGE_BYTES + p * 1024);
        }
    };
// ... 589 lines not shown
                    }
                }
                h8 f0 = hx_frag(stage, 0, 0, lane), f0l = hx_frag(stage, 0, 1, lane), f1 = hx_frag(stage, 8, 0, lane),
                   f1l = hx_frag(stage, 8, 1, lane);
#pragma unroll
                for (int kc = 0; kc < 8; ++kc) {
                    const int kn = min(kc + 1, 7);
                    const h8 n0 = hx_frag(stage, kn, 0, lane), n0l = hx_frag(stage, kn, 1, lane), n1 = hx_frag(stage, 8 + kn, 0, lane),
                             n1l = hx_frag(stage, 8 + kn, 1, lane);
                    PIPE_FENCE();
                    MFH3(xh[kc], xl[kc], f0, f0l, a0);
                    MFH3(xh[kc], xl[kc], f1, f1l, a1);
                    PIPE_FENCE();
                    f0 = n0; f0l = n0l; f1 = n1; f1l = n1l;
                }
#pragma unroll
                for (int r0 = 0; r0 < 16; r0 += 8) {
                    float zr0[8], zr1[8];
                    int vo[8];
#pragma unroll
                    for (int q = 0; q < 8; ++q) {
                        const int rc = ((r0 + q) & 3) + 8 * ((r0 + q) >> 2);
                        const int so = (prow0 + rc) * 512 + ob * 128;
                        vo[q] = (h4 < nvalid - rc) ? voff : 0x7FFFFFF0;
                        if (half == 1) { zr0[q] = zp0[r0 + q]; zr1[q] = zp1[r0 + q]; }
                        else { zr0[q] = hx_load(rz, vo[q], so); zr1[q] = hx_load(rz, vo[q], so + 128); }
                    }
#pragma unroll
                    for (int q = 0; q < 8; ++q) {
                        const int rc = ((r0 + q) & 3) + 8 * ((r0 + q) >> 2);
                        const int so = (prow0 + rc) * 512 + ob * 128;
                        const float u0 = a0[r0 + q], u1 = a1[r0 + q], g0 = ga[r0 + q], g1 = gb[r0 + q];
                        hx_store(rz, fmaf(u0, g0, zr0[q]), vo[q], so);
                        hx_store(rz, fmaf(u1, g1, zr1[q]), vo[q], so + 128);
                    }
                    PIPE_FENCE();
                }
            }
        }
    }
}

static int g_hx_cu = 0;
static int hx_num_cu() {
    if (!g_hx_cu) { int dev = 0; hipDeviceProp_t pr; (void)hipGetDevice(&dev); (void)hipGetDeviceProperties(&pr, dev); g_hx_cu = pr.multiProcessorCount > 0 ? pr.multiProcessorCount : 256; }
    return g_hx_cu;
}
static int hx_nw() { return 8; }
static unsigned hx_grid(long long n_tiles, int nw) {
    const long long cap = (nw == 8 ? 1LL : 2LL) * hx_num_cu();
    return (unsigned)(n_tiles < cap ? n_tiles : cap);
}

void launch_pair_transition_hx(genie_ctx* h, hipStream_t st, const PairLayerW& w) {
    const int N = h->N;
    const long long M = (long long)h->B * N * N;
    const long long n_wt = (M + 31) / 32;
    const int n_hb = h->d.pair_transition_n * 4;
    const HxTransW& x = w.hx_pt;
    hipLaunchKernelGGL(k_pair_transition_hx<8>, dim3(hx_grid((n_wt + 7) / 8, 8)), dim3(512), HX_LDS_BYTES, st, h->p, h->rmaskf, x.img,
                       x.b1s, x.b2s, N, M, n_hb, x.sx, x.c1, x.c2, (int)(h->hx_launches++ & 1));
}

struct HxTriGeom {
    int N, NP, ntile, nw, n_wt;
    unsigned cm_bytes, z_bytes;
};
static HxTriGeom tri_geom(const genie_ctx* h) {
    HxTriGeom g;
    g.N = h->N; g.NP = h->NP; g.ntile = (g.N + 31) / 32; g.nw = hx_nw();
    g.n_wt = h->B * g.N * g.ntile;
    g.cm_bytes = (unsigned)((size_t)h->B * 128 * g.NP * g.NP * 4);
    g.z_bytes = (unsigned)((size_t)h->B * g.N * g.N * 512);
    return g;
}

static void hx_trimul_proj(genie_ctx* h, hipStream_t st, const TriMulW& w, bool outgoing) {
    const HxTriGeom g = tri_geom(h);
    const HxTriW& x = w.hx;
    unsigned* acm = reinterpret_cast<unsigned*>(h->acm);
    unsigned* bcm = reinterpret_cast<unsigned*>(h->bcm);
    ProfScope ps(h, st, KC_TRIMUL_PROJ);
    const dim3 grid(hx_grid((g.n_wt + g.nw - 1) / g.nw, g.nw)), block(g.nw * 64);
    const int rev = (int)(h->hx_launches++ & 1);
#define HX_PROJ(OUT, NWV) hipLaunchKernelGGL((k_trimul_proj_hx<OUT, NWV>), grid, block, HX_LDS_BYTES, st, h->p, h->rmaskf, x.img_proj, \
                                         x.bias_proj, acm, bcm, g.N, g.NP, g.n_wt, g.cm_bytes, g.z_bytes, x.sx, x.cpa, x.cpb, x.cg, rev)
    if (outgoing) HX_PROJ(true, 8);
    else HX_PROJ(false, 8);
#undef HX_PROJ
}

static void hx_trimul_contract(genie_ctx* h, hipStream_t st, const TriMulW& w, bool transposed) {
    const HxTriGeom g = tri_geom(h);
    const HxTriW& x = w.hx;
    ProfScope ps(h, st, KC_TRIMUL_CONTRACT);
    const int BC = h->B * h->d.c_hidden_mul;
    const int ncu = hx_num_cu();
    const int rev = (int)(h->hx_launches++ & 1);
    const unsigned* acm = reinterpret_cast<const unsigned*>(h->acm);
    const unsigned* bcm = reinterpret_cast<const unsigned*>(h->bcm);
    const unsigned* pa = transposed ? bcm : acm;
    const unsigned* pb = transposed ? acm : bcm;
    if (g.NP > 192 && g.NP <= 256) {
        hipLaunchKernelGGL(k_trimul_contract_hx_big, dim3(BC < ncu ? BC : ncu), dim3(512), 4 * CB_PLANE, st, pa, pb, h->xcm, g.NP, BC, g.cm_bytes,
                           x.cx, rev);
    } else if (g.NP >= 128) {
        const int tiles = (g.NP + 127) / 128;
        const int n_tiles = tiles * tiles * ((BC + 7) / 8) * 8;
        hipLaunchKernelGGL(k_trimul_contract_hx<2>, dim3(n_tiles < 3 * ncu ? n_tiles : 3 * ncu), dim3(256), 2 * 4 * 128 * CX_ROWB, st,
                           pa, pb, h->xcm, g.NP, BC, g.cm_bytes, x.cx, rev);
    } else {
        const int tiles = (g.NP + 63) / 64;
        const int n_tiles = tiles * tiles * ((BC + 7) / 8) * 8;
        hipLaunchKernelGGL(k_trimul_contract_hx<1>, dim3(n_tiles < 4 * ncu ? n_tiles : 4 * ncu), dim3(256), 2 * 4 * 64 * CX_ROWB, st,
                           pa, pb, h->xcm, g.NP, BC, g.cm_bytes, x.cx, rev);
    }
}

static void hx_trimul_out(genie_ctx* h, hipStream_t st, const TriMulW& w) {
    const HxTriGeom g = tri_geom(h);
    const HxTriW& x = w.hx;
    ProfScope ps(h, st, KC_TRIMUL_OUT);
    hipLaunchKernelGGL(k_trimul_out_hx_r<8>, dim3(hx_grid((g.n_wt + 7) / 8, 8)), dim3(512), 4 * HX_STAGE_BYTES, st, h->p, h->xcm,
                       x.img_out, x.bgs, x.bzs, g.N, g.NP, g.n_wt, g.cm_bytes, g.z_bytes, x.sx, x.cgo, x.cz, (int)(h->hx_launches++ & 1));
}

void launch_trimul_hx(genie_ctx* h, hipStream_t st, const TriMulW& w, bool outgoing) {
    hx_trimul_proj(h, st, w, outgoing);
    hx_trimul_contract(h, st, w, false);
    hx_trimul_out(h, st, w);
}

void launch_pair_fused(genie_ctx* h, hipStream_t st, const HxFusedW& f, const HxTriW& o, const HxTransW* t, const HxTriW* p, bool col);
bool launch_pair_stack_fused(genie_ctx* h, hipStream_t st, float* tap_trimul_out0, float* tap_layer0) {
    const int L = h->d.n_pair_transform_layer;
    if (!h->hx || L < 1 || getenv("GENIE_NO_PAIR_FUSE")) return false;
    if (h->d.n_head_tri > 0) return false;
    const size_t pbytes = (size_t)h->B * h->N * h->N * h->d.c_p * 4;
    hx_trimul_proj(h, st, h->pair[0].out, true);
    for (int l = 0; l < L; ++l) {
        const PairLayerW& W = h->pair[l];
        hx_trimul_contract(h, st, W.out, true);
        { ProfScope ps(h, st, KC_PAIR_FUSED_A); launch_pair_fused(h, st, W.fa, W.out.hx, nullptr, &W.in.hx, true); }
        if (l == 0 && tap_trimul_out0) (void)hipMemcpyAsync(tap_trimul_out0, h->p, pbytes, hipMemcpyDeviceToDevice, st);
        hx_trimul_contract(h, st, W.in, false);
        {
            ProfScope ps(h, st, KC_PAIR_FUSED_B);
            launch_pair_fused(h, st, W.fb, W.in.hx, &W.hx_pt, l + 1 < L ? &h->pair[l + 1].out.hx : nullptr, false);
        }
        if (l == 0 && tap_layer0) (void)hipMemcpyAsync(tap_layer0, h->p, pbytes, hipMemcpyDeviceToDevice, st);
    }
    return true;
}


#define IB_UNITS 24
__global__ __launch_bounds__(256) void k_ipa_bias_hx(const float* __restrict__ z, const unsigned char* __restrict__ wimg, float inv_sw,
                                                     const float* __restrict__ bias, float* __restrict__ out, int B, int N, int LH,
                                                     int n_tiles, int rev, unsigned* pmax) {
    extern __shared__ __attribute__((aligned(16))) unsigned char ibw[];
    float* sbias = reinterpret_cast<float*>(ibw + IB_UNITS * 2048);
    const int tid = threadIdx.x, lane = tid & 63, wave = tid >> 6;
    for (int u = tid; u < IB_UNITS * 128; u += 256) reinterpret_cast<uint4*>(ibw)[u] = reinterpret_cast<const uint4*>(wimg)[u];
    if (tid < 96) sbias[tid] = tid < LH ? bias[tid] : 0.f;
    __syncthreads();
    const int n = lane & 31, hf = lane >> 5;
    const int jt = (N + 31) >> 5;
    float amax = 0.f;
    for (int t = blockIdx.x * 4 + wave; t < n_tiles; t += gridDim.x * 4) {
        const int tt = rev ? n_tiles - 1 - t : t;
        const int j0 = (tt % jt) * 32;
        const int bi = tt / jt;
        const int j = min(j0 + n, N - 1);
        const float* row = z + ((size_t)bi * N + j) * 128 + 8 * hf;
        float4 x[8][2];
#pragma unroll
        for (int s = 0; s < 8; ++s) {
            x[s][0] = *reinterpret_cast<const float4*>(row + 16 * s);
            x[s][1] = *reinterpret_cast<const float4*>(row + 16 * s + 4);
        }
        float m = 0.f;
#pragma unroll
        for (int s = 0; s < 8; ++s) {
            m = fmaxf(m, fmaxf(fmaxf(fabsf(x[s][0].x), fabsf(x[s][0].y)), fmaxf(fabsf(x[s][0].z), fabsf(x[s][0].w))));
            m = fmaxf(m, fmaxf(fmaxf(fabsf(x[s][1].x), fabsf(x[s][1].y)), fmaxf(fabsf(x[s][1].z), fabsf(x[s][1].w))));
        }
        m = fmaxf(m, __shfl_xor(m, 32));
        amax = fmaxf(amax, m);
        const int e = (int)((__builtin_bit_cast(unsigned, m) >> 23) & 255u);
        const bool tiny = e < 16;
        const float sc = tiny ? 1.0f : __builtin_bit_cast(float, (unsigned)(268 - e) << 23);
        const float isc = (tiny ? 1.0f : __builtin_bit_cast(float, (unsigned)(e - 14) << 23)) * inv_sw;
        f32x16 acc[3];
#pragma unroll
        for (int blk = 0; blk < 3; ++blk)
#pragma unroll
            for (int r = 0; r < 16; ++r) acc[blk][r] = 0.f;
#pragma unroll
        for (int s = 0; s < 8; ++s) {
            const float xs[8] = {x[s][0].x, x[s][0].y, x[s][0].z, x[s][0].w, x[s][1].x, x[s][1].y, x[s][1].z, x[s][1].w};
            h8 bh, bl;
            hx_split8(xs, sc, bh, bl);
#pragma unroll
            for (int blk = 0; blk < 3; ++blk) {
                const h8 ah = hx_frag(ibw, blk * 8 + s, 0, lane), al = hx_frag(ibw, blk * 8 + s, 1, lane);
                MFH3(ah, al, bh, bl, acc[blk]);
            }
        }
        if (j0 + n < N) {
            const int b = bi / N, i = bi - b * N;
#pragma unroll
            for (int blk = 0; blk < 3; ++blk)
#pragma unroll
                for (int r = 0; r < 16; ++r) {
                    const int o = blk * 32 + (r & 3) + 8 * (r >> 2) + 4 * hf;
                    if (o < LH) out[((((size_t)o * B + b) * N + i) * N) + j0 + n] = fmaf(acc[blk][r], isc, sbias[o]);
                }
        }
    }
#pragma unroll
    for (int o = 32; o > 0; o >>= 1) amax = fmaxf(amax, __shfl_xor(amax, o));
    if (lane == 0 && __float_as_uint(amax) > *reinterpret_cast<volatile unsigned*>(pmax)) atomicMax(pmax, __float_as_uint(amax));
}

bool launch_ipa_bias_hx(genie_ctx* h, hipStream_t st) {
    const int LH = h->d.n_structure_layer * h->d.n_head_ipa;
    if (!h->hx || LH > 96) return false;
    const HxGemmW* w = nullptr;
    for (int i = 0; i < h->n_hxg; ++i)
        if (h->hxg[i].w == h->ipa_bias_w) w = &h->hxg[i];
    if (!w) return false;
    const int N = h->N, n_tiles = h->B * N * ((N + 31) / 32);
    const int grid = n_tiles / 4 < 2 * hx_num_cu() ? (n_tiles + 3) / 4 : 2 * hx_num_cu();
    (void)hipMemsetAsync(h->pmax, 0, sizeof(unsigned), st);
    hipLaunchKernelGGL(k_ipa_bias_hx, dim3(grid), dim3(256), IB_UNITS * 2048 + 96 * 4, st, h->p, w->img, w->inv_s, h->ipa_bias_b, h->ipa_bias,
                       h->B, N, LH, n_tiles, (int)(h->hx_launches & 1), h->pmax);
    return true;
}

void pair_hx_kernels_init() {
#define HX_ATTR(k) (void)hipFuncSetAttribute(reinterpret_cast<const void*>(k), hipFuncAttributeMaxDynamicSharedMemorySize, HX_LDS_BYTES)
    HX_ATTR((k_trimul_proj_hx<true, 8>)); HX_ATTR((k_trimul_proj_hx<false, 8>));
    HX_ATTR(k_trimul_out_hx_r<8>);
    (void)hipFuncSetAttribute(reinterpret_cast<const void*>(k_trimul_contract_hx_big), hipFuncAttributeMaxDynamicSharedMemorySize, 4 * CB_PLANE);
#undef HX_ATTR
    (void)hipFuncSetAttribute(reinterpret_cast<const void*>(k_pair_transition_hx<8>), hipFuncAttributeMaxDynamicSharedMemorySize, HX_LDS_BYTES);
    (void)hipFuncSetAttribute(reinterpret_cast<const void*>(k_ipa_bias_hx), hipFuncAttributeMaxDynamicSharedMemorySize, IB_UNITS * 2048 + 96 * 4);
}
```

genie2_amd/csrc/single_kernels.hip:

```cpp
#include <algorithm>
#include <type_traits>
#include "hx.h"

__global__ void k_single_input(float* __restrict__ x, int ldx, const float* __restrict__ pos_tab, int n_pos, int c_pos,
                               const float* __restrict__ chain_tab, int n_chain, int c_chain,
                               const float* __restrict__ t_tab, int c_t, const int32_t* __restrict__ timesteps,
                               const int32_t* __restrict__ ridx, const int32_t* __restrict__ cidx,
                               const int32_t* __restrict__ aatype, const uint8_t* __restrict__ fsm,
                               const uint8_t* __restrict__ ifm, int N, int n_timestep) {
    const int row = blockIdx.x;
    const int b = row / N;
    float* xr = x + (size_t)row * ldx;
    const int ri = min(max(ridx[row], 0), n_pos - 1);
    const int ci = min(max(cidx[row], 0), n_chain - 1);
    const int ts = min(max(timesteps[b], 0), n_timestep);
    const float f = fsm[row] ? 1.f : 0.f;
    const int o1 = c_pos, o2 = o1 + c_chain, o3 = o2 + c_t, o4 = o3 + 20;
    for (int c = threadIdx.x; c < ldx; c += blockDim.x) {
        float v;
        if (c < o1) v = pos_tab[(size_t)ri * c_pos + c];
        else if (c < o2) v = chain_tab[(size_t)ci * c_chain + (c - o1)];
        else if (c < o3) v = t_tab[(size_t)ts * c_t + (c - o2)];
        else if (c < o4) v = (float)aatype[(size_t)row * 20 + (c - o3)] * f;
        else if (c < o4 + 2) v = f;
        else if (c == o4 + 2) v = ifm[row] ? 1.f : 0.f;
        else v = 0.f;
        xr[c] = v;
    }
}

#define LDA 68
#define GR_PD 8
__global__ __launch_bounds__(256) void k_gemm_rows(const float* __restrict__ A, int lda, int M, int K,
                                                   const float* __restrict__ Wp, int Nout,
                                                   const float* __restrict__ bias, const float* __restrict__ res, int ldr,
                                                   const float* __restrict__ rowmask, int relu, float* __restrict__ out, int ldo) {
    __shared__ __attribute__((aligned(16))) float sa[2][32 * LDA];
    const int tid = threadIdx.x, lane = tid & 63, wave = tid >> 6;
    const int r0 = blockIdx.x * 32;
    const int nb = min((int)(blockIdx.y * 4 + wave), (Nout + 31) / 32 - 1);
    const bool active = (int)(blockIdx.y * 4 + wave) * 32 < Nout;
    const int KB = (K + 7) >> 3;
    const int nkc = (K + 63) >> 6;
    const int lr = tid >> 4, c4 = tid & 15;
    const float* wbase = Wp + ((size_t)nb * KB * 64 + lane) * 4;

    v4f wq[GR_PD];
#pragma unroll
    for (int s = 0; s < GR_PD; ++s) wf_issue(wq[s], wbase + (size_t)min(s, KB - 1) * 256);

    v4f ra0, ra1;
    auto a_addr = [&](int kc, int u) {
        const int r = min(r0 + lr + 16 * u, M - 1), k = min(kc * 64 + c4 * 4, K - 4);
        return A + (size_t)r * lda + k;
    };
    auto a_store = [&](int kc, int buf) {
        const bool kok = kc * 64 + c4 * 4 < K;
        const v4f z4 = {0.f, 0.f, 0.f, 0.f};
        const v4f v0 = (kok && r0 + lr < M) ? ra0 : z4;
        const v4f v1 = (kok && r0 + lr + 16 < M) ? ra1 : z4;
        *reinterpret_cast<v4f*>(&sa[buf][lr * LDA + c4 * 4]) = v0;
        *reinterpret_cast<v4f*>(&sa[buf][(lr + 16) * LDA + c4 * 4]) = v1;
    };
    wf_issue(ra0, a_addr(0, 0));
    wf_issue(ra1, a_addr(0, 1));
    wf_wait<0>(ra0, ra1);
    a_store(0, 0);
    __syncthreads();

    f32x16 acc = zero16();
    for (int kc = 0; kc < nkc; ++kc) {
        const int kcn = min(kc + 1, nkc - 1);
        wf_issue(ra0, a_addr(kcn, 0));
        wf_issue(ra1, a_addr(kcn, 1));
        const float* cur = sa[kc & 1];
#pragma unroll
        for (int kb = 0; kb < 8; ++kb) {
            const float4 af = lfrag(cur, LDA, 0, kb, lane);
            wf_wait<GR_PD + 1>(wq[kb]);
            if (kc * 8 + kb < KB) acc = mfma_8k(af, wq[kb], acc);
            __builtin_amdgcn_sched_barrier(0);
            wf_issue(wq[kb], wbase + (size_t)min(kc * 8 + kb + GR_PD, KB - 1) * 256);
        }
        wf_wait<GR_PD>(ra0, ra1);
        a_store(kcn, (kc + 1) & 1);
        __syncthreads();
    }
#pragma unroll
    for (int s = 0; s < GR_PD; ++s) wf_wait<0>(wq[s]);
    if (!active) return;
    const int col = nb * 32 + (lane & 31);
    if (col >= Nout) return;
    const float bc = bias ? bias[col] : 0.f;
#pragma unroll
    for (int r = 0; r < 16; ++r) {
        const int row = r0 + acc_row(r, lane);
        if (row < M) {
            float v = acc[r] + bc;
            if (relu) v = fmaxf(v, 0.f);
            if (res) v += res[(size_t)row * ldr + col];
            if (rowmask) v *= rowmask[row];
            out[(size_t)row * ldo + col] = v;
        }
    }
}

#define GH_ROWB 144
#define GH_PD 8
#define GH_AD 4
__global__ __launch_bounds__(256) void k_gemm_rows_hx(const float* __restrict__ A, int lda, int M, int K,
                                                      const unsigned char* __restrict__ Wx, int Nout, float inv_sw,
                                                      const float* __restrict__ bias, const float* __restrict__ res, int ldr,
                                                      const float* __restrict__ rowmask, int relu, float* __restrict__ out, int ldo,
                                                      size_t zstride) {
    __shared__ __attribute__((aligned(16))) unsigned char sa[2][2][32 * GH_ROWB];
    __shared__ __attribute__((aligned(16))) float sinv[2][32];
    const int tid = threadIdx.x, lane = tid & 63, wave = tid >> 6;
    const int r0 = blockIdx.x * 32;
    const int nb = min((int)(blockIdx.y * 4 + wave), (Nout + 31) / 32 - 1);
    const bool active = (int)(blockIdx.y * 4 + wave) * 32 < Nout;
    const int KCt = (K + 15) >> 4, nkct = (K + 63) >> 6;
    const int c0 = (int)blockIdx.z * nkct / (int)gridDim.z, c1 = ((int)blockIdx.z + 1) * nkct / (int)gridDim.z;
    const float* wbase = reinterpret_cast<const float*>(Wx + ((size_t)nb * KCt + (size_t)c0 * 4) * 2048) + lane * 4;
    A += c0 * 64;
    K = min(K, c1 * 64) - c0 * 64;
    out += (size_t)blockIdx.z * zstride;
    const int KC = (K + 15) >> 4;
    const int nkc = (K + 63) >> 6;
    const int lr = tid >> 4, c4 = tid & 15;

    v4f wh[GH_PD], wl[GH_PD];
#pragma unroll
    for (int s = 0; s < GH_PD; ++s) {
        const float* p = wbase + (size_t)min(s, KC - 1) * 512;
        wf_issue(wh[s], p);
        wf_issue(wl[s], p + 256);
    }
    v4f ra[GH_AD][2];
    auto a_addr = [&](int kc, int u) {
        const int r = min(r0 + lr + 16 * u, M - 1), k = min(kc * 64 + c4 * 4, K - 4);
        return A + (size_t)r * lda + k;
    };
    auto split_store = [&](v4f v, int row, int buf) {
        float m = fmaxf(fmaxf(fabsf(v.x), fabsf(v.y)), fmaxf(fabsf(v.z), fabsf(v.w)));
        m = fmaxf(m, __shfl_xor(m, 1)); m = fmaxf(m, __shfl_xor(m, 2)); m = fmaxf(m, __shfl_xor(m, 4)); m = fmaxf(m, __shfl_xor(m, 8));
        const int e = (int)((__builtin_bit_cast(unsigned, m) >> 23) & 255u);
        const bool tiny = e < 16;
        const float sc = tiny ? 1.0f : __builtin_bit_cast(float, (unsigned)(268 - e) << 23);
        const float isc = tiny ? 1.0f : __builtin_bit_cast(float, (unsigned)(e - 14) << 23);
        unsigned h01, l01, h23, l23;
        hx_split2(v.x, v.y, sc, h01, l01);
        hx_split2(v.z, v.w, sc, h23, l23);
        *reinterpret_cast<uint2*>(&sa[buf][0][row * GH_ROWB + c4 * 8]) = make_uint2(h01, h23);
        *reinterpret_cast<uint2*>(&sa[buf][1][row * GH_ROWB + c4 * 8]) = make_uint2(l01, l23);
        if (c4 == 0) sinv[buf][row] = isc;
    };
    auto a_store = [&](v4f v0, v4f v1, int kc, int buf) {
        const bool kok = kc * 64 + c4 * 4 < K;
        const v4f z4 = {0.f, 0.f, 0.f, 0.f};
        split_store((kok && r0 + lr < M) ? v0 : z4, lr, buf);
        split_store((kok && r0 + lr + 16 < M) ? v1 : z4, lr + 16, buf);
    };
#pragma unroll
    for (int c = 0; c < GH_AD; ++c) {
        wf_issue(ra[c][0], a_addr(min(c, nkc - 1), 0));
        wf_issue(ra[c][1], a_addr(min(c, nkc - 1), 1));
    }
    wf_wait<2 * (GH_AD - 1)>(ra[0][0], ra[0][1]);
// ... 679 lines not shown
            const float mean = row16_sum(sum) / (float)C;
            float ss = 0.f;
#pragma unroll
            for (int q = 0; q < C / 64; ++q) {
                const float dx = v[q].x - mean, dy = v[q].y - mean, dz = v[q].z - mean, dw = v[q].w - mean;
                ss += (dx * dx + dy * dy) + (dz * dz + dw * dw);
            }
            const float rstd = 1.0f / sqrtf(row16_sum(ss) / (float)C + GENIE_LN_EPS);
#pragma unroll
            for (int q = 0; q < C / 64; ++q) {
                const int c = 64 * q + 4 * l16;
                const float4 gq = *reinterpret_cast<const float4*>(g + c), bq = *reinterpret_cast<const float4*>(bta + c);
                float4 y;
                y.x = (v[q].x - mean) * rstd * gq.x + bq.x; y.y = (v[q].y - mean) * rstd * gq.y + bq.y;
                y.z = (v[q].z - mean) * rstd * gq.z + bq.z; y.w = (v[q].w - mean) * rstd * gq.w + bq.w;
                *reinterpret_cast<float4*>(T + rrow * SR_LD + c) = y;
                if (gout && r0 + rrow < M) *reinterpret_cast<float4*>(gout + (size_t)(r0 + rrow) * C + c) = y;
            }
        }
        __syncthreads();
    };

    auto dpp_max = [](float m, auto ctrl_tag) {
        constexpr int CTRL = decltype(ctrl_tag)::value;
        return fmaxf(m, __builtin_bit_cast(float, __builtin_amdgcn_update_dpp(0, __builtin_bit_cast(int, m), CTRL, 0xf, 0xf, false)));
    };
    auto split_store = [&](float4 v, int row, int kc) {
        float m = fmaxf(fmaxf(fabsf(v.x), fabsf(v.y)), fmaxf(fabsf(v.z), fabsf(v.w)));
        m = dpp_max(m, std::integral_constant<int, 0xB1>{});
        m = dpp_max(m, std::integral_constant<int, 0x4E>{});
        m = dpp_max(m, std::integral_constant<int, 0x124>{});
        m = dpp_max(m, std::integral_constant<int, 0x128>{});
        const int e = (int)((__builtin_bit_cast(unsigned, m) >> 23) & 255u);
        const bool tiny = e < 16;
        const float sc = tiny ? 1.0f : __builtin_bit_cast(float, (unsigned)(268 - e) << 23);
        const float isc = tiny ? 1.0f : __builtin_bit_cast(float, (unsigned)(e - 14) << 23);
        unsigned h01, l01, h23, l23;
        hx_split2(v.x, v.y, sc, h01, l01);
        hx_split2(v.z, v.w, sc, h23, l23);
        unsigned char* d = sa + kc * (2 * 32 * GH_ROWB) + row * GH_ROWB + l16 * 8;
        *reinterpret_cast<uint2*>(d) = make_uint2(h01, h23);
        *reinterpret_cast<uint2*>(d + 32 * GH_ROWB) = make_uint2(l01, l23);
        if (l16 == 0) sinv[kc * 32 + row] = isc;
    };

    auto linear = [&](const float* A, const unsigned char* __restrict__ Wx, const unsigned char* Wnext, float inv_sw,
                      const float* bias, bool relu, const float* res, float* out) {
        const unsigned char* wb = Wx + (size_t)wsel * KC * 2048;
#pragma unroll
        for (int i = 0; i < 32 * (C / 4) / NT; ++i) {
            const int u = tid + i * NT, rc = u >> 4, row = rc / NKC, kc = rc - row * NKC;
            split_store(*reinterpret_cast<const float4*>(A + row * SR_LD + kc * 64 + l16 * 4), row, kc);
        }
        __syncthreads();
        f32x16 acc = zero16();
        const int foff = (lane & 31) * GH_ROWB + (lane >> 5) * 16;
#pragma unroll 1
        for (int kc = 0; kc < NKC; ++kc) {
            const unsigned char* cur = sa + kc * (2 * 32 * GH_ROWB) + foff;
            f32x16 part = zero16();
#pragma unroll
            for (int q = 0; q < 4; ++q) {
                const h8 ah = *reinterpret_cast<const h8*>(cur + q * 32);
                const h8 al = *reinterpret_cast<const h8*>(cur + 32 * GH_ROWB + q * 32);
                wf_wait<2 * SR_PD - 2>(wh[q], wl[q]);
                const h8 bh = __builtin_bit_cast(h8, wh[q]), bl = __builtin_bit_cast(h8, wl[q]);
                MFH3(ah, al, bh, bl, part);
                __builtin_amdgcn_sched_barrier(0);
                unit_issue(wb, wh[q], wl[q], kc * 4 + q + SR_PD);
            }
            const float* si = sinv + kc * 32 + 4 * (lane >> 5);
#pragma unroll
            for (int g = 0; g < 4; ++g) {
                const float4 iv = *reinterpret_cast<const float4*>(si + 8 * g);
                acc[4 * g] = fmaf(part[4 * g], iv.x, acc[4 * g]); acc[4 * g + 1] = fmaf(part[4 * g + 1], iv.y, acc[4 * g + 1]);
                acc[4 * g + 2] = fmaf(part[4 * g + 2], iv.z, acc[4 * g + 2]); acc[4 * g + 3] = fmaf(part[4 * g + 3], iv.w, acc[4 * g + 3]);
            }
        }
#pragma unroll
        for (int u = 0; u < SR_PD; ++u) wf_wait<0>(wh[u], wl[u]);
        if (Wnext) ring_fill(Wnext);
        const int col = wave * 32 + (lane & 31);
        const float bc = bias[col];
#pragma unroll
        for (int r = 0; r < 16; ++r) {
            const int row = acc_row(r, lane);
            float v = fmaf(acc[r], inv_sw, bc);
            if (relu) v = fmaxf(v, 0.f);
            if (res) v += res[row * SR_LD + col];
            out[row * SR_LD + col] = v;
        }
        __syncthreads();
    };

    layernorm(T0, g1, be1, nullptr);
    linear(T0, W1, W2, i1, b1, true, nullptr, T1);
    linear(T1, W2, W3, i2, b2, true, nullptr, T1);
    linear(T1, W3, nullptr, i3, b3, false, T0, T1);
    for (int u = tid; u < 6 * C / 4; u += NT)
        reinterpret_cast<float4*>(T0)[u] = reinterpret_cast<const float4*>(bbw)[u];
    layernorm(T1, g2, be2, s_out);

    if (splitter) {
        float acc[6] = {0.f, 0.f, 0.f, 0.f, 0.f, 0.f};
#pragma unroll
        for (int q = 0; q < C / 64; ++q) {
            const int c = 64 * q + 4 * l16;
            const float4 xv = *reinterpret_cast<const float4*>(T1 + rrow * SR_LD + c);
#pragma unroll
            for (int o = 0; o < 6; ++o) {
                const float4 wv = *reinterpret_cast<const float4*>(T0 + o * C + c);
                acc[o] += (xv.x * wv.x + xv.y * wv.y) + (xv.z * wv.z + xv.w * wv.w);
            }
        }
#pragma unroll
        for (int o = 0; o < 6; ++o) acc[o] = row16_sum(acc[o]) + bbb[o];
        const int row = r0 + rrow;
        if (l16 == 0 && row < M) {
            const float qb = acc[0], qc = acc[1], qd = acc[2];
            const float den = sqrtf(((qb * qb + qc * qc) + qd * qd) + 1.0f);
            const float a = 1.0f / den, bq = qb / den, c = qc / den, d = qd / den;
            float U[9];
            U[0] = a * a + bq * bq - c * c - d * d; U[1] = 2 * bq * c - 2 * a * d;          U[2] = 2 * bq * d + 2 * a * c;
            U[3] = 2 * bq * c + 2 * a * d;          U[4] = a * a - bq * bq + c * c - d * d; U[5] = 2 * c * d - 2 * a * bq;
            U[6] = 2 * bq * d - 2 * a * c;          U[7] = 2 * c * d + 2 * a * bq;          U[8] = a * a - bq * bq - c * c + d * d;
            float* R = rots + (size_t)row * 9;
            float* t = trans + (size_t)row * 3;
            float Rn[9], rr[9];
#pragma unroll
            for (int k = 0; k < 9; ++k) rr[k] = frm[rrow * 12 + k];
#pragma unroll
            for (int xx = 0; xx < 3; ++xx)
#pragma unroll
                for (int y = 0; y < 3; ++y) Rn[xx * 3 + y] = rr[xx * 3 + 0] * U[0 * 3 + y] + rr[xx * 3 + 1] * U[1 * 3 + y] + rr[xx * 3 + 2] * U[2 * 3 + y];
            const float tx = rr[0] * acc[3] + rr[1] * acc[4] + rr[2] * acc[5] + frm[rrow * 12 + 9];
            const float ty = rr[3] * acc[3] + rr[4] * acc[4] + rr[5] * acc[5] + frm[rrow * 12 + 10];
            const float tz = rr[6] * acc[3] + rr[7] * acc[4] + rr[8] * acc[5] + frm[rrow * 12 + 11];
#pragma unroll
            for (int k = 0; k < 9; ++k) R[k] = Rn[k];
            t[0] = tx; t[1] = ty; t[2] = tz;
            if (z_out) {
                z_out[(size_t)row * 3 + 0] = trans_in[(size_t)row * 3 + 0] - tx * inv_rescale;
                z_out[(size_t)row * 3 + 1] = trans_in[(size_t)row * 3 + 1] - ty * inv_rescale;
                z_out[(size_t)row * 3 + 2] = trans_in[(size_t)row * 3 + 2] - tz * inv_rescale;
            }
        }
    }
}

__global__ __launch_bounds__(256) void k_p_sample_frenet(int mode, float* __restrict__ trans, float* __restrict__ rots,
                                                         const float* __restrict__ z, const float* __restrict__ eps,
                                                         const int32_t* __restrict__ rmask, const int32_t* __restrict__ cidx,
                                                         int N, float alpha, float sqrt_alpha, float somac, float sqrt_beta,
                                                         float scale, float a, float bz, float c_scaled) {
    extern __shared__ __attribute__((aligned(16))) float sm[];
    float* x = sm;
    float* tv = x + 3 * N;
    float* base = tv + 3 * N;
    float* st1 = base + 9 * N;
    __shared__ int s_len;
    const int b = blockIdx.x, tid = threadIdx.x;
    float* tr = trans + (size_t)b * N * 3;
    if (tid == 0) s_len = 0;
    __syncthreads();
    int cnt = 0;
    for (int n = tid; n < N; n += 256) cnt += rmask[b * N + n];
    atomicAdd(&s_len, cnt);
    if (mode == 1) {
        const float w_z = (1.0f - alpha) / somac;
        const float inv_sa = 1.0f / sqrt_alpha;
        for (int u = tid; u < 3 * N; u += 256) {
            const float m = (float)rmask[b * N + u / 3];
            float v = inv_sa * (tr[u] - w_z * z[(size_t)b * N * 3 + u]);
            v = v * m;
            if (eps) { v = v + scale * sqrt_beta * eps[(size_t)b * N * 3 + u]; v = v * m; }
            x[u] = v;
            tr[u] = v;
        }
    } else if (mode == 2) {
        for (int u = tid; u < 3 * N; u += 256) {
            const float m = (float)rmask[b * N + u / 3];
            float v = a * tr[u] + bz * z[(size_t)b * N * 3 + u];
            v = v * m;
            if (eps) { v = v + c_scaled * eps[(size_t)b * N * 3 + u]; v = v * m; }
            x[u] = v;
            tr[u] = v;
        }
    } else {
        for (int u = tid; u < 3 * N; u += 256) x[u] = tr[u];
    }
    __syncthreads();
    const int len = s_len;
    for (int n = tid; n < N - 1; n += 256) {
        const float dx = x[3 * n + 3] - x[3 * n], dy = x[3 * n + 4] - x[3 * n + 1], dz = x[3 * n + 5] - x[3 * n + 2];
        const float nr = sqrtf(1e-10f + ((dx * dx + dy * dy) + dz * dz));
        tv[3 * n] = dx / nr; tv[3 * n + 1] = dy / nr; tv[3 * n + 2] = dz / nr;
    }
    __syncthreads();
    for (int n = tid; n < N; n += 256) {
        float R[9] = {1.f, 0.f, 0.f, 0.f, 1.f, 0.f, 0.f, 0.f, 1.f};
        if (n >= 1 && n < len - 1) {
            const int m = n - 1;
            const float ax = tv[3 * m], ay = tv[3 * m + 1], az = tv[3 * m + 2];
            const float bx = tv[3 * m + 3], by = tv[3 * m + 4], bz = tv[3 * m + 5];
            float cx = ay * bz - az * by, cy = az * bx - ax * bz, cz = ax * by - ay * bx;
            const float nr = sqrtf(1e-10f + ((cx * cx + cy * cy) + cz * cz));
            cx /= nr; cy /= nr; cz /= nr;
            const float nx = cy * bz - cz * by, ny = cz * bx - cx * bz, nz = cx * by - cy * bx;
            R[0] = bx; R[1] = cx; R[2] = nx;
            R[3] = by; R[4] = cy; R[5] = ny;
            R[6] = bz; R[7] = cz; R[8] = nz;
        }
#pragma unroll
        for (int k = 0; k < 9; ++k) base[9 * n + k] = R[k];
    }
    __syncthreads();
    const int32_t* ch = cidx + b * N;
    for (int n = tid; n < N; n += 256) {
        int srcn = n;
        if (n < len && (n == 0 || ch[n] != ch[n - 1])) srcn = n + 1;
#pragma unroll
        for (int k = 0; k < 9; ++k) st1[9 * n + k] = (srcn < N) ? base[9 * srcn + k] : ((k % 4 == 0) ? 1.f : 0.f);
    }
    __syncthreads();
    float* ro = rots + (size_t)b * N * 9;
    for (int n = tid; n < N; n += 256) {
        int k = n;
        if (n < len) {
            while (k >= 0 && (k == len - 1 || ch[k] != ch[k + 1])) --k;
            if (k < 0) k = N - 1;
        }
#pragma unroll
        for (int q = 0; q < 9; ++q) ro[9 * n + q] = st1[9 * k + q];
    }
}

__global__ void k_fill_i32(int32_t* p, int n, int v) {
    const int i = blockIdx.x * blockDim.x + threadIdx.x;
    if (i < n) p[i] = v;
}

__global__ void k_scale_copy(const float* __restrict__ in, float* __restrict__ out, int n, float s) {
    const int i = blockIdx.x * blockDim.x + threadIdx.x;
    if (i < n) out[i] = in[i] * s;
}

template <int H, int C, int PQ, int PV, int Q, int MF>
__global__ __launch_bounds__(MF ? 128 * Q : 512, MF ? 4 : 1) void k_ipa_attn_q(const float* __restrict__ proj, int ldp, const float* __restrict__ kT,
                                                    const float* __restrict__ v, const float* __restrict__ qp,
                                                    const float* __restrict__ kpT, const float* __restrict__ vp,
                                                    const float* __restrict__ bias, const float* __restrict__ z,
                                                    const float* __restrict__ rots, const float* __restrict__ trans,
                                                    const float* __restrict__ rmask, const float* __restrict__ head_w,
                                                    float* __restrict__ cat, int B, int N, int layer, int rev,
                                                    const unsigned* __restrict__ pmax, int b0,
                                                    const float* __restrict__ vf, const float* __restrict__ vmax) {
    constexpr int NT = MF ? 128 * Q : 512;
    constexpr int CP = 128, HC = H * C, NQP = H * PQ * 3, NPT = H * PV * 3, NCAT = HC + H * PV * 4 + H * CP, HH = H / (NT / 256);
    static_assert(H % (NT / 256) == 0 && C % 4 == 0 && HC + NPT <= 512, "shape");
    static_assert(!MF || H <= 16, "matrix-pipe o_pair: 2 Q waves = Q queries x 2 channel halves");
    extern __shared__ __attribute__((aligned(16))) float sm[];
    const int NP8 = (N + 7) & ~7;
    const int NPA = NP8 + 4;
    float* att = sm;
    float* sq = att + Q * H * NPA;
    float* sqp = sq + Q * HC;
    float* shw = sqp + Q * NQP;
    float* opt = shw + 16;
    float* red = opt + Q * NPT;
    const int tid = threadIdx.x, lane = tid & 63, wave = tid >> 6;
    const int groups = (N + Q - 1) / Q;
    const int bid = rev ? (int)(gridDim.x - 1 - blockIdx.x) : (int)blockIdx.x;
    const int b = b0 + bid / groups, i0 = (bid % groups) * Q;
    const int nq = min(Q, N - i0);
    for (int u = tid; u < Q * HC; u += NT) { const int q = u / HC; sq[u] = proj[(size_t)(b * N + min(i0 + q, N - 1)) * ldp + (u - q * HC)]; }
    for (int u = tid; u < Q * NQP; u += NT) { const int q = u / NQP; sqp[u] = qp[(size_t)(b * N + min(i0 + q, N - 1)) * NQP + (u - q * NQP)]; }
    if (tid < H) {
        const float g = head_w[tid];
        const float sp = (g > 20.f) ? g : log1pf(expf(g));
        shw[tid] = sp * sqrtf(1.0f / (3.0f * ((float)PQ * 9.0f / 2.0f)));
    }
    __syncthreads();
    const float s_qk = sqrtf(1.0f / (3.0f * (float)C)), s_b = sqrtf(1.0f / 3.0f);
    {
        const int hg = tid >> 8;
        for (int j = tid & 255; j < NP8; j += 256) {
            const int jc = min(j, N - 1);
            const float mj = rmask[b * N + jc];
            float sqm[Q];
#pragma unroll
            for (int q = 0; q < Q; ++q) sqm[q] = 1e5f * (rmask[b * N + min(i0 + q, N - 1)] * mj - 1.0f);
#pragma unroll 1
            for (int h2 = 0; h2 < HH; ++h2) {
                const int hh = hg * HH + h2;
                const float* kc = kT + (((size_t)b * H + hh) * C) * N + jc;
                float kv[C];
#pragma unroll
                for (int c = 0; c < C; ++c) kv[c] = kc[(size_t)c * N];
                const float* kp = kpT + ((((size_t)b * H + hh) * PQ) * 3) * N + jc;
                float kpv[PQ * 3];
#pragma unroll
                for (int c = 0; c < PQ * 3; ++c) kpv[c] = kp[(size_t)c * N];
                float bia[Q];
#pragma unroll
                for (int q = 0; q < Q; ++q) bia[q] = bias[((((size_t)layer * H + hh) * B + b) * N + min(i0 + q, N - 1)) * N + jc];
                const float hw = shw[hh];
#pragma unroll
                for (int q = 0; q < Q; ++q) {
                    const float* qv = sq + q * HC + hh * C;
                    float qk = 0.f;
#pragma unroll
                    for (int c = 0; c < C; ++c) qk += qv[c] * kv[c];
                    float a = qk * s_qk;
                    a += s_b * bia[q];
                    const float* qpv = sqp + q * NQP + hh * PQ * 3;
                    float pt = 0.f;
#pragma unroll
                    for (int pp = 0; pp < PQ; ++pp) {
                        const float dx = qpv[pp * 3 + 0] - kpv[pp * 3 + 0];
                        const float dy = qpv[pp * 3 + 1] - kpv[pp * 3 + 1];
                        const float dz = qpv[pp * 3 + 2] - kpv[pp * 3 + 2];
                        pt += ((dx * dx + dy * dy) + dz * dz) * hw;
                    }
                    a += pt * (-0.5f);
                    a += sqm[q];
                    att[(q * H + hh) * NPA + j] = (j < N) ? a : -3.0e38f;
                }
            }
        }
    }
    __syncthreads();
    {
        auto dpp = [](float m, auto ctrl_tag) {
            constexpr int CTRL = decltype(ctrl_tag)::value;
            return __builtin_bit_cast(float, __builtin_amdgcn_update_dpp(0, __builtin_bit_cast(int, m), CTRL, 0xf, 0xf, false));
        };
        const int l16 = lane & 15;
        for (int rr = wave * 4 + (lane >> 4); rr < Q * H; rr += NT / 16) {
            float* ar = att + rr * NPA;
            float mx = -3.0e38f;
            for (int j = 4 * l16; j < NP8; j += 64) {
                const float4 v = *reinterpret_cast<const float4*>(ar + j);
                mx = fmaxf(mx, fmaxf(fmaxf(v.x, v.y), fmaxf(v.z, v.w)));
            }
            mx = fmaxf(mx, dpp(mx, std::integral_constant<int, 0xB1>{})); mx = fmaxf(mx, dpp(mx, std::integral_constant<int, 0x4E>{}));
            mx = fmaxf(mx, dpp(mx, std::integral_constant<int, 0x124>{})); mx = fmaxf(mx, dpp(mx, std::integral_constant<int, 0x128>{}));
            float sum = 0.f;
            for (int j = 4 * l16; j < NP8; j += 64) {
                float4 v = *reinterpret_cast<const float4*>(ar + j);
                v.x = expf(v.x - mx); v.y = expf(v.y - mx); v.z = expf(v.z - mx); v.w = expf(v.w - mx);
                *reinterpret_cast<float4*>(ar + j) = v;
                sum += (v.x + v.y) + (v.z + v.w);
            }
            sum += dpp(sum, std::integral_constant<int, 0xB1>{}); sum += dpp(sum, std::integral_constant<int, 0x4E>{});
            sum += dpp(sum, std::integral_constant<int, 0x124>{}); sum += dpp(sum, std::integral_constant<int, 0x128>{});
            for (int j = 4 * l16; j < NP8; j += 64) {
                float4 v = *reinterpret_cast<const float4*>(ar + j);
                v.x /= sum; v.y /= sum; v.z /= sum; v.w /= sum;
                *reinterpret_cast<float4*>(ar + j) = v;
            }
        }
    }
    __syncthreads();
    constexpr int JP = MF ? (NT / 64 >= H ? 1 : 2) : 1;
    constexpr int PARTS = JP;
    float* osum = opt + Q * NPT;
    if constexpr (MF) {
        static_assert(Q <= 16 && Q % 4 == 0 && C == 16 && PV * 3 <= 32 && (JP == 1 || ((NT / 64) % JP == 0 && H % (NT / 64 / JP) == 0)), "matrix-pipe o / o_pt");
        constexpr int HG = JP == 1 ? H : NT / 64 / JP, HL = H / HG, NBK = 1 + (PV * 3 + 15) / 16;
        const int KS = (N + 31) >> 5, ksm = (KS + JP - 1) / JP;
        const int hg = wave / JP, jh = wave % JP, m = lane & 15, g = lane >> 4;
        const int ks0 = jh * ksm, nks = hg < HG ? max(min(KS - ks0, ksm), 0) : 0, nit = nks * HL;
        float mv = 0.f, mp = 0.f;
        for (int j = lane; j < (N + 7) >> 3; j += 64) {
            const float2 t = *reinterpret_cast<const float2*>(vmax + ((size_t)b * ((N + 7) >> 3) + j) * 2);
            mv = fmaxf(mv, t.x); mp = fmaxf(mp, t.y);
        }
#pragma unroll
        for (int o = 32; o > 0; o >>= 1) { mv = fmaxf(mv, __shfl_xor(mv, o)); mp = fmaxf(mp, __shfl_xor(mp, o)); }
        const int exv = min(max((int)((__float_as_uint(mv) >> 23) & 0xff), 28), 254), exp_ = min(max((int)((__float_as_uint(mp) >> 23) & 0xff), 28), 254);
        const float sv = __uint_as_float((unsigned)(267 - exv) << 23), sp = __uint_as_float((unsigned)(267 - exp_) << 23);
        const float iv = __uint_as_float((unsigned)(exv - 27) << 23), ip = __uint_as_float((unsigned)(exp_ - 27) << 23);
        const float sa = (m < Q) ? 16384.0f : 0.0f;
        const float* ar = att + (size_t)min(m, Q - 1) * H * NPA + 8 * g;
        const float* vb = vf + ((size_t)b * H * NBK * KS) * 512 + lane * 8;
        f32x4 acc[NBK];
#pragma unroll
        for (int c = 0; c < NBK; ++c) acc[c] = f32x4{0.f, 0.f, 0.f, 0.f};
        float4 bb[2][NBK][2];
        auto fetch = [&](int it, float4 (&dst)[NBK][2]) {
            const int hh = hg * HL + it / nks, ks = ks0 + it % nks;
#pragma unroll
// ... 157 lines not shown
    for (int q = 0; q < nq; ++q) {
        const int row = b * N + i0 + q;
        float4 acc[H];
#pragma unroll
        for (int hh = 0; hh < H; ++hh) acc[hh] = make_float4(0.f, 0.f, 0.f, 0.f);
        const float* zr = z + ((size_t)row * N) * CP + c4 * 4;
        const float* aq = att + q * H * NPA;
        for (int jb = jg * 8; jb < NP8; jb += 128) {
            float4 zz[8];
#pragma unroll
            for (int k = 0; k < 8; ++k) zz[k] = *reinterpret_cast<const float4*>(zr + (size_t)min(jb + k, N - 1) * CP);
#pragma unroll
            for (int hh = 0; hh < H; ++hh) {
                const float4 a0 = *reinterpret_cast<const float4*>(aq + hh * NPA + jb), a1 = *reinterpret_cast<const float4*>(aq + hh * NPA + jb + 4);
                const float a[8] = {a0.x, a0.y, a0.z, a0.w, a1.x, a1.y, a1.z, a1.w};
#pragma unroll
                for (int k = 0; k < 8; ++k) {
                    acc[hh].x += a[k] * zz[k].x; acc[hh].y += a[k] * zz[k].y; acc[hh].z += a[k] * zz[k].z; acc[hh].w += a[k] * zz[k].w;
                }
            }
        }
#pragma unroll
        for (int hh = 0; hh < H; ++hh) {
            acc[hh].x += __shfl_xor(acc[hh].x, 32); acc[hh].y += __shfl_xor(acc[hh].y, 32);
            acc[hh].z += __shfl_xor(acc[hh].z, 32); acc[hh].w += __shfl_xor(acc[hh].w, 32);
        }
        if (wave < 4 && lane < 32) {
#pragma unroll
            for (int hh = 0; hh < H; ++hh) *reinterpret_cast<float4*>(red + ((size_t)wave * H + hh) * CP + c4 * 4) = acc[hh];
        }
        __syncthreads();
        if (wave >= 4 && lane < 32) {
#pragma unroll
            for (int hh = 0; hh < H; ++hh) {
                float4* pr = reinterpret_cast<float4*>(red + ((size_t)(wave - 4) * H + hh) * CP + c4 * 4);
                float4 t = *pr;
                t.x += acc[hh].x; t.y += acc[hh].y; t.z += acc[hh].z; t.w += acc[hh].w;
                *pr = t;
            }
        }
        __syncthreads();
        {
            float* op = cat + (size_t)row * NCAT + HC + H * PV * 4;
            constexpr int tot = H * CP;
            for (int u = tid; u < tot; u += 512) op[u] = (red[u] + red[tot + u]) + (red[2 * tot + u] + red[3 * tot + u]);
        }
        __syncthreads();
    }
    }
    if constexpr (PARTS == 2) {
        for (int u = tid; u < nq * (HC + NPT); u += NT) {
            const int q = u / (HC + NPT), col = u - q * (HC + NPT);
            const float sum = osum[q * (HC + NPT) + col] + osum[(Q + q) * (HC + NPT) + col];
            if (col < HC) cat[(size_t)(b * N + i0 + q) * NCAT + col] = sum;
            else opt[q * NPT + (col - HC)] = sum;
        }
        __syncthreads();
    }
    {
        constexpr int np = H * PV;
        for (int u = tid; u < nq * np; u += NT) {
            const int q = u / np, w = u - q * np;
            const int row = b * N + i0 + q;
            const float* R = rots + (size_t)row * 9;
            const float* t = trans + (size_t)row * 3;
            const float* o3 = opt + q * NPT + w * 3;
            const float x = o3[0] - t[0], y = o3[1] - t[1], zc = o3[2] - t[2];
            const float lx = R[0] * x + R[3] * y + R[6] * zc;
            const float ly = R[1] * x + R[4] * y + R[7] * zc;
            const float lz = R[2] * x + R[5] * y + R[8] * zc;
            float* crow = cat + (size_t)row * NCAT;
            crow[HC + w] = lx;
            crow[HC + np + w] = ly;
            crow[HC + 2 * np + w] = lz;
            crow[HC + 3 * np + w] = sqrtf(((lx * lx + ly * ly) + lz * lz) + 1e-8f);
        }
    }
}

__global__ void k_q_sample(const float* __restrict__ x0, const float* __restrict__ z, const float* __restrict__ c0,
                           const float* __restrict__ c1, float* __restrict__ out, int n_per_b, int total) {
    const int u = blockIdx.x * blockDim.x + threadIdx.x;
    if (u < total) { const int b = u / n_per_b; out[u] = c0[b] * x0[u] + c1[b] * z[u]; }
}

__global__ __launch_bounds__(256) void k_training_loss(const float* __restrict__ zp, const float* __restrict__ z,
                                                       const int32_t* __restrict__ rmask, const uint8_t* __restrict__ fsm, int B, int N,
                                                       float w, float* __restrict__ losses, float* __restrict__ stats, float* __restrict__ grad) {
    __shared__ float red[4][4];
    const int b = blockIdx.x, tid = threadIdx.x, lane = tid & 63, wave = tid >> 6;
    float v[4] = {0.f, 0.f, 0.f, 0.f};
    for (int n = tid; n < N; n += 256) {
        const size_t o = ((size_t)b * N + n) * 3;
        const float dx = zp[o] - z[o], dy = zp[o + 1] - z[o + 1], dz = zp[o + 2] - z[o + 2];
        const float err = sqrtf(1e-10f + ((dx * dx + dy * dy) + dz * dz));
        const float m = (float)rmask[b * N + n], f = fsm[b * N + n] ? 1.f : 0.f;
        const float mc = m * f, mi = m * (1.f - f);
        v[0] += err * mc; v[1] += err * mi; v[2] += mc; v[3] += mi;
    }
#pragma unroll
    for (int k = 0; k < 4; ++k) {
#pragma unroll
        for (int o = 32; o > 0; o >>= 1) v[k] += __shfl_xor(v[k], o);
        if (lane == 0) red[wave][k] = v[k];
    }
    __syncthreads();
#pragma unroll
    for (int k = 0; k < 4; ++k) v[k] = (red[0][k] + red[1][k]) + (red[2][k] + red[3][k]);
    if (tid == 0) {
        losses[2 + b] = v[0]; losses[2 + B + b] = v[1];
        stats[2 * b] = (v[0] + v[1]) / (v[2] + v[3]);
        stats[2 * b + 1] = (w * v[0] + v[1]) / (w * v[2] + v[3]);
    }
    if (grad) {
        const float coef = 1.0f / ((float)B * (w * v[2] + v[3]));
        for (int n = tid; n < N; n += 256) {
            const size_t o = ((size_t)b * N + n) * 3;
            const float dx = zp[o] - z[o], dy = zp[o + 1] - z[o + 1], dz = zp[o + 2] - z[o + 2];
            const float err = sqrtf(1e-10f + ((dx * dx + dy * dy) + dz * dz));
            const float m = (float)rmask[b * N + n], f = fsm[b * N + n] ? 1.f : 0.f;
            const float g = coef * (w * m * f + m * (1.f - f)) / err;
            grad[o] = g * dx; grad[o + 1] = g * dy; grad[o + 2] = g * dz;
        }
    }
}
__global__ void k_training_loss_mean(const float* __restrict__ stats, int B, float* __restrict__ losses) {
    if (threadIdx.x == 0) {
        float u = 0.f, wl = 0.f;
        for (int b = 0; b < B; ++b) { u += stats[2 * b]; wl += stats[2 * b + 1]; }
        losses[0] = u / (float)B; losses[1] = wl / (float)B;
    }
}

__global__ __launch_bounds__(256) void k_adam(float* __restrict__ p, const float* __restrict__ g, float* __restrict__ m,
                                              float* __restrict__ v, size_t n, float omb1, float b2, float omb2, float eps,
                                              float step_size, float sqrt_bc2) {
    for (size_t i = (size_t)blockIdx.x * 256 + threadIdx.x; i < n; i += (size_t)gridDim.x * 256) {
        const float gi = g[i];
        const float mi = m[i] + (gi - m[i]) * omb1;
        const float vi = v[i] * b2 + omb2 * (gi * gi);
        m[i] = mi; v[i] = vi;
        const float denom = sqrtf(vi) / sqrt_bc2 + eps;
        p[i] = p[i] - step_size * (mi / denom);
    }
}
void launch_adam(hipStream_t st, size_t n, float* p, const float* g, float* m, float* v, double lr, double b1, double b2, double eps,
                 int step) {
    const double bc1 = 1.0 - pow(b1, step), bc2 = 1.0 - pow(b2, step);
    const size_t blocks = (n + 255) / 256;
    hipLaunchKernelGGL(k_adam, dim3((unsigned)(blocks < 4096 ? blocks : 4096)), dim3(256), 0, st, p, g, m, v, n,
                       (float)(1.0 - b1), (float)b2, (float)(1.0 - b2), (float)eps, (float)(lr / bc1), (float)sqrt(bc2));
}

void launch_single_input(genie_ctx* h, hipStream_t st, const int32_t* timesteps) {
    ProfScope ps(h, st, KC_SINGLE_INPUT);
    const genie_dims_t& d = h->d;
    const int ldx = (d.c_pos_emb + d.c_chain_emb + d.c_timestep_emb + 23 + 7) / 8 * 8;
    hipLaunchKernelGGL(k_single_input, dim3(h->B * h->N), dim3(256), 0, st, h->xsingle, ldx, h->pos_tab, h->n_pos, d.c_pos_emb,
                       h->chain_tab, h->n_chain, d.c_chain_emb, h->t_tab, d.c_timestep_emb, timesteps, h->f_ridx, h->f_cidx,
                       h->f_aatype, h->f_fsm, h->f_ifm, h->N, d.n_timestep);
}

void launch_gemm_rows(genie_ctx* h, hipStream_t st, const float* A, int lda, int M, int K, const float* Wp, int Nout,
                      const float* bias, const float* res, int ldr, const float* rowmask, int relu, float* out, int ldo, int prof_class) {
    ProfScope ps(h, st, prof_class);
    dim3 grid((M + 31) / 32, (Nout + 127) / 128);
    if (h->hx) {
        for (int i = 0; i < h->n_hxg; ++i)
            if (h->hxg[i].w == Wp) {
                hipLaunchKernelGGL(k_gemm_rows_hx, grid, dim3(256), 0, st, A, lda, M, K, h->hxg[i].img, Nout, h->hxg[i].inv_s, bias, res,
                                   ldr, rowmask, relu, out, ldo, (size_t)0);
                return;
            }
    }
    hipLaunchKernelGGL(k_gemm_rows, grid, dim3(256), 0, st, A, lda, M, K, Wp, Nout, bias, res, ldr, rowmask, relu, out, ldo);
}

void launch_layernorm_rows(genie_ctx* h, hipStream_t st, const float* in, float* out, int M, int C, const float* g,
                           const float* b) {
    ProfScope ps(h, st, KC_LAYERNORM);
    hipLaunchKernelGGL(k_layernorm_rows, dim3((M + 3) / 4), dim3(256), 0, st, in, out, M, C, g, b);
}

static bool ipa_attn_mfma_av(const genie_ctx* h);
void launch_ipa_prep(genie_ctx* h, hipStream_t st, int b0, int nb) {
    ProfScope ps(h, st, KC_IPA_PREP);
    const genie_dims_t& d = h->d;
    if (nb < 0) { b0 = 0; nb = h->B; }
    const int ldp = d.n_head_ipa * (3 * d.c_hidden_ipa + 3 * d.n_qk_point + 3 * (d.n_qk_point + d.n_v_point));
    if (ipa_attn_mfma_av(h)) {
        hipLaunchKernelGGL(k_ipa_prep_frag, dim3(nb * ((h->N + 7) / 8)), dim3(256), 0, st, h->proj, ldp, h->rots_w, h->trans_w, h->kT, h->qp,
                           h->kpT, h->vf, h->vmax, h->N, d.n_head_ipa, d.c_hidden_ipa, d.n_qk_point, d.n_v_point, b0);
        return;
    }
    hipLaunchKernelGGL(k_ipa_prep, dim3(nb * h->N), dim3(256), 0, st, h->proj, ldp, h->rots_w, h->trans_w, h->kT, h->v, h->qp,
                       h->kpT, h->vp, h->N, d.n_head_ipa, d.c_hidden_ipa, d.n_qk_point, d.n_v_point, b0 * h->N);
}

static bool ipa_is_base(const genie_dims_t& d) {
    return d.n_head_ipa == 12 && d.c_hidden_ipa == 16 && d.n_qk_point == 4 && d.n_v_point == 8 && d.c_p == 128;
}
#define IPA_Q 4
static size_t ipa_attn_t1_lds(const genie_dims_t& d, int N) {
    return ((size_t)d.n_head_ipa * ((N + 7) & ~7) + 4 * d.n_head_ipa * d.c_p + d.n_head_ipa * d.n_v_point * 3) * sizeof(float);
}
static size_t ipa_attn_q_lds(const genie_dims_t& d, int N, bool mf = false);
static bool ipa_use_q(const genie_dims_t& d, int N) { return ipa_attn_q_lds(d, N) <= 160 * 1024; }
static size_t ipa_attn_t_lds(const genie_dims_t& d, int N) { return ipa_use_q(d, N) ? ipa_attn_q_lds(d, N) : ipa_attn_t1_lds(d, N); }
static size_t ipa_attn_q_lds(const genie_dims_t& d, int N, bool mf) {
    const size_t H = d.n_head_ipa, Q = IPA_Q;
    return (Q * H * (((N + 7) & ~7) + 4) + Q * H * d.c_hidden_ipa + Q * H * d.n_qk_point * 3 + 16 +
            Q * H * d.n_v_point * 3 + (mf ? 0 : 4 * H * d.c_p) +
            (mf ? 2 * Q * H * (d.c_hidden_ipa + 3 * d.n_v_point) : 0)) * sizeof(float);
}
size_t ipa_attn_lds(const genie_dims_t& d, int N) {
    if (ipa_is_base(d)) return ipa_attn_t_lds(d, N);
    return ((size_t)d.n_head_ipa * N + 8 * d.n_head_ipa * d.c_p + d.n_head_ipa * d.n_v_point * 3) * sizeof(float);
}

static bool ipa_attn_mfma_av(const genie_ctx* h) { return h->hx && ipa_is_base(h->d) && ipa_use_q(h->d, h->N); }
size_t ipa_vf_floats(const genie_dims_t& d, int B, int N) {
    return ipa_is_base(d) ? (size_t)B * d.n_head_ipa * (1 + (3 * d.n_v_point + 15) / 16) * ((N + 31) / 32) * 512 : 64;
}
bool ipa_attn_splits(const genie_ctx* h) { return ipa_is_base(h->d) && ipa_use_q(h->d, h->N); }
void launch_ipa_attn(genie_ctx* h, hipStream_t st, int layer, const float* head_w, int b0, int nb) {
    ProfScope ps(h, st, KC_IPA_ATTN);
    const genie_dims_t& d = h->d;
    if (nb < 0 || !ipa_attn_splits(h)) { b0 = 0; nb = h->B; }
    const int ldp = d.n_head_ipa * (3 * d.c_hidden_ipa + 3 * d.n_qk_point + 3 * (d.n_qk_point + d.n_v_point));
    if (ipa_is_base(d) && !ipa_use_q(d, h->N)) {
        hipLaunchKernelGGL((k_ipa_attn_t<12, 16, 4, 8>), dim3(h->B * h->N), dim3(256), ipa_attn_t1_lds(d, h->N), st, h->proj, ldp,
                           h->kT, h->v, h->qp, h->kpT, h->vp, h->ipa_bias, h->p, h->rots_w, h->trans_w, h->rmaskf, head_w, h->cat,
                           h->B, h->N, layer);
        return;
    }
    if (ipa_is_base(d)) {
        const dim3 grid(nb * ((h->N + IPA_Q - 1) / IPA_Q));
        const int rev = (int)((layer ^ h->hx_launches ^ 1) & 1);
        if (h->hx)
            hipLaunchKernelGGL((k_ipa_attn_q<12, 16, 4, 8, IPA_Q, 1>), grid, dim3(512), ipa_attn_q_lds(d, h->N, true), st, h->proj, ldp,
                               h->kT, h->v, h->qp, h->kpT, h->vp, h->ipa_bias, h->p, h->rots_w, h->trans_w, h->rmaskf, head_w, h->cat,
                               h->B, h->N, layer, rev, h->pmax, b0, h->vf, h->vmax);
        else
            hipLaunchKernelGGL((k_ipa_attn_q<12, 16, 4, 8, IPA_Q, 0>), grid, dim3(512), ipa_attn_q_lds(d, h->N), st, h->proj, ldp,
                               h->kT, h->v, h->qp, h->kpT, h->vp, h->ipa_bias, h->p, h->rots_w, h->trans_w, h->rmaskf, head_w, h->cat,
                               h->B, h->N, layer, rev, h->pmax, b0, nullptr, nullptr);
        return;
    }
    hipLaunchKernelGGL(k_ipa_attn, dim3(h->B * h->N), dim3(256), ipa_attn_lds(d, h->N), st, h->proj, ldp, h->kT, h->v, h->qp,
                       h->kpT, h->vp, h->ipa_bias, h->p, h->rots_w, h->trans_w, h->rmaskf, head_w, h->cat, h->B, h->N,
                       d.n_head_ipa, d.c_hidden_ipa, d.n_qk_point, d.n_v_point, d.c_p, layer);
}

void launch_bb_update(genie_ctx* h, hipStream_t st, const StructLayerW& w, const float* trans_in, float* z_out) {
    ProfScope ps(h, st, KC_BB_UPDATE);
    const int M = h->B * h->N;
    hipLaunchKernelGGL(k_bb_update, dim3((M + 3) / 4), dim3(256), 0, st, h->s, h->d.c_s, w.bb_w, w.bb_b, h->rots_w, h->trans_w,
                       M, trans_in, z_out, 1.0f / h->d.rescale);
}

static size_t struct_rows_lds() { return (size_t)2 * 32 * SR_LD * 4 + 6 * (2 * 32 * GH_ROWB + 32 * 4) + 32 * 12 * 4; }
static const HxGemmW* hx_image(const genie_ctx* h, const float* Wp) {
    for (int i = 0; i < h->n_hxg; ++i)
        if (h->hxg[i].w == Wp) return &h->hxg[i];
    return nullptr;
}
bool struct_tail_fused(const genie_ctx* h, const StructLayerW& S) {
    if (!h->hx || h->d.c_s != 384 || getenv("GENIE_NO_STRUCT_FUSE")) return false;
    return hx_image(h, S.out_w) && hx_image(h, S.t1_w) && hx_image(h, S.t2_w) && hx_image(h, S.t3_w);
}
bool launch_struct_tail(genie_ctx* h, hipStream_t st, const StructLayerW& S, const float* trans_in, float* z_out, int b0, int nb) {
    if (!struct_tail_fused(h, S)) return false;
    const HxGemmW *w0 = hx_image(h, S.out_w), *w1 = hx_image(h, S.t1_w), *w2 = hx_image(h, S.t2_w), *w3 = hx_image(h, S.t3_w);
    if (nb < 0) { b0 = 0; nb = h->B; }
    const int Mall = h->B * h->N, M = nb * h->N, cs = h->d.c_s, ncat = h->d.n_head_ipa * (h->d.c_p + h->d.c_hidden_ipa + 4 * h->d.n_v_point);
    const size_t zs = (size_t)Mall * cs, r0 = (size_t)b0 * h->N;
    {
        ProfScope ps(h, st, KC_GEMM_ROWS);
        hipLaunchKernelGGL(k_gemm_rows_hx, dim3((M + 31) / 32, (cs + 127) / 128, SR_KSPLIT), dim3(256), 0, st, h->cat + r0 * ncat, ncat, M, ncat,
                           w0->img, cs, w0->inv_s, nullptr, nullptr, 0, nullptr, 0, h->spart + r0 * cs, cs, zs);
    }
    ProfScope ps(h, st, KC_STRUCT_ROWS);
    const int nrb = (M + 31) / 32;
    hipLaunchKernelGGL((k_struct_rows_hx<12>), dim3(nrb + 64), dim3(768), struct_rows_lds(), st, h->spart + r0 * cs, SR_KSPLIT, zs, S.out_b, h->s + r0 * cs,
                       S.ln_ipa_g, S.ln_ipa_b, w1->img, w1->inv_s, S.t1_b, w2->img, w2->inv_s, S.t2_b, w3->img, w3->inv_s, S.t3_b,
                       S.ln_tr_g, S.ln_tr_b, S.bb_w, S.bb_b, h->s + r0 * cs, h->rots_w + r0 * 9, h->trans_w + r0 * 3, M, trans_in ? trans_in + r0 * 3 : nullptr,
                       z_out ? z_out + r0 * 3 : nullptr, 1.0f / h->d.rescale, nrb);
    return true;
}

void launch_q_sample(genie_ctx* h, hipStream_t st, const float* x0, const float* z, const float* c0, const float* c1, float* trans_out) {
    ProfScope ps(h, st, KC_MISC);
    const int total = h->B * h->N * 3;
    hipLaunchKernelGGL(k_q_sample, dim3((total + 255) / 256), dim3(256), 0, st, x0, z, c0, c1, trans_out, h->N * 3, total);
}
void launch_training_loss(genie_ctx* h, hipStream_t st, const float* zp, const float* z, float w, float* losses, float* grad) {
    ProfScope ps(h, st, KC_MISC);
    float* stats = h->loop_z;
    hipLaunchKernelGGL(k_training_loss, dim3(h->B), dim3(256), 0, st, zp, z, h->f_rmask, h->f_fsm, h->B, h->N, w, losses, stats, grad);
    hipLaunchKernelGGL(k_training_loss_mean, dim3(1), dim3(64), 0, st, stats, h->B, losses);
}

void launch_frenet(genie_ctx* h, hipStream_t st, int mode, int step, float scale, float* trans, float* rots, const float* z,
                   const float* eps) {
    ProfScope ps(h, st, KC_P_SAMPLE);
    float al = 1.f, sa = 1.f, so = 1.f, sb = 0.f;
    if (mode == 1) {
        const int T1 = h->d.n_timestep + 1;
        al = h->sched_host[0 * T1 + step];
        sa = h->sched_host[1 * T1 + step];
        so = h->sched_host[2 * T1 + step];
        sb = h->sched_host[3 * T1 + step];
    }
    const size_t lds = (size_t)(3 + 3 + 9 + 9) * h->N * sizeof(float);
    hipLaunchKernelGGL(k_p_sample_frenet, dim3(h->B), dim3(256), lds, st, mode, trans, rots, z, eps, h->f_rmask, h->f_cidx, h->N,
                       al, sa, so, sb, scale, 0.f, 0.f, 0.f);
}

void launch_reverse_step(genie_ctx* h, hipStream_t st, float a, float bz, float c_scaled, float* trans, float* rots, const float* z,
                         const float* eps) {
    ProfScope ps(h, st, KC_P_SAMPLE);
    const size_t lds = (size_t)(3 + 3 + 9 + 9) * h->N * sizeof(float);
    hipLaunchKernelGGL(k_p_sample_frenet, dim3(h->B), dim3(256), lds, st, 2, trans, rots, z, eps, h->f_rmask, h->f_cidx, h->N,
                       1.f, 1.f, 1.f, 0.f, 0.f, a, bz, c_scaled);
}

int genie_frenet_frames(genie_stream_t stream, int B, int N, const float* coords, const int32_t* chains, const int32_t* mask,
                        float* rots_out) {
    if (!coords || !chains || !mask || !rots_out || B < 1 || N < 2) return GENIE_E_ARG;
    const size_t lds = (size_t)24 * N * sizeof(float);
    if (lds > 160 * 1024) return GENIE_E_ARG;
    if (lds > 64 * 1024)
        (void)hipFuncSetAttribute(reinterpret_cast<const void*>(k_p_sample_frenet), hipFuncAttributeMaxDynamicSharedMemorySize, (int)lds);
    hipLaunchKernelGGL(k_p_sample_frenet, dim3(B), dim3(256), lds, (hipStream_t)stream, 0, const_cast<float*>(coords), rots_out,
                       (const float*)nullptr, (const float*)nullptr, mask, chains, N, 1.f, 1.f, 1.f, 0.f, 0.f, 0.f, 0.f, 0.f);
    return hipGetLastError() == hipSuccess ? GENIE_OK : GENIE_E_HIP;
}

void launch_fill_i32(genie_ctx* h, hipStream_t st, int32_t* p, int n, int v) {
    ProfScope ps(h, st, KC_MISC);
    hipLaunchKernelGGL(k_fill_i32, dim3((n + 255) / 256), dim3(256), 0, st, p, n, v);
}

void launch_scale_copy(genie_ctx* h, hipStream_t st, const float* in, float* out, int n, float s) {
    ProfScope ps(h, st, KC_MISC);
    hipLaunchKernelGGL(k_scale_copy, dim3((n + 255) / 256), dim3(256), 0, st, in, out, n, s);
}

void single_kernels_init(const genie_dims_t& d, int n_max) {
    (void)hipFuncSetAttribute(reinterpret_cast<const void*>(k_p_sample_frenet), hipFuncAttributeMaxDynamicSharedMemorySize,
                        (int)std::min<size_t>((size_t)24 * n_max * sizeof(float), 160 * 1024));
    (void)hipFuncSetAttribute(reinterpret_cast<const void*>(k_struct_rows_hx<12>), hipFuncAttributeMaxDynamicSharedMemorySize,
                        (int)struct_rows_lds());
    if (ipa_is_base(d)) {
        if (ipa_use_q(d, n_max)) {
            (void)hipFuncSetAttribute(reinterpret_cast<const void*>(k_ipa_attn_q<12, 16, 4, 8, IPA_Q, 0>),
                                hipFuncAttributeMaxDynamicSharedMemorySize, (int)ipa_attn_q_lds(d, n_max));
            (void)hipFuncSetAttribute(reinterpret_cast<const void*>(k_ipa_attn_q<12, 16, 4, 8, IPA_Q, 1>),
                                hipFuncAttributeMaxDynamicSharedMemorySize, (int)ipa_attn_q_lds(d, n_max, true));
        } else
            (void)hipFuncSetAttribute(reinterpret_cast<const void*>(k_ipa_attn_t<12, 16, 4, 8>), hipFuncAttributeMaxDynamicSharedMemorySize,
                                (int)ipa_attn_t1_lds(d, n_max));
    } else
        (void)hipFuncSetAttribute(reinterpret_cast<const void*>(k_ipa_attn), hipFuncAttributeMaxDynamicSharedMemorySize,
                            (int)ipa_attn_lds(d, n_max));
}
```

Measured before the change: 110.8 batch-steps/s.

## Fuse IPA bias into last pair layer, prefetch next timestep's single embedding on side stream

Folds the IPA pair-bias projection into the final fused pair-stack kernel as extra f16-split weight stages, tracking the abs-max for pmax inside it, so the separate launch_ipa_bias pass over the pair tensor is skipped. It also computes the next step's single-input embedding and pij projection on the secondary stream while the current step runs, using double buffers s/s0 and pij/pij2. The reverse-step kernel now writes trans_w/rots_w directly, which removes the scale-copy and memcpy, and the timestep fill kernel is replaced by a scalar argument. These add scaling and precision risk on the bias path, extra event synchronisation, and more workspace.

```diff
diff --git a/genie2_amd/csrc/common.h b/genie2_amd/csrc/common.h
--- a/genie2_amd/csrc/common.h
+++ b/genie2_amd/csrc/common.h
@@ -146,7 +146,7 @@
     float *bias_proj, *bgs, *bzs;
     float sx, cpa, cpb, cg, cx, cgo, cz;
 };
-struct HxFusedW { const unsigned char* img; };
+struct HxFusedW { const unsigned char* img; int n_bias; float bias_inv_s; };
 struct TriMulW {
     float *proj_w;
     float *proj_b;
@@ -220,12 +220,11 @@
     float *p, *acm, *bcm, *xcm, *pstatic, *ipa_bias;
     float *spart;
     unsigned *pmax;
-    float *xsingle, *s0, *s, *s1, *s2, *h1, *h2, *pij, *proj, *cat;
+    float *xsingle, *s0, *s, *s1, *s2, *h1, *h2, *pij, *pij2, *proj, *cat;
     float *kT, *v, *qp, *kpT, *vp;
     float *vf, *vmax;
     float *ta_tb, *ta_xn, *ta_qkvg;
     float *rots_w, *trans_w;
-    int32_t* tsteps;
     float *loop_z;
 
     bool prof;
@@ -235,9 +234,10 @@
     double train_gemm_flop;
 
     hipStream_t st2; hipEvent_t ev_fork, ev_join;
-};
-
-void launch_single_input(genie_ctx* h, hipStream_t st, const int32_t* timesteps);
+    hipEvent_t ev_pre_go, ev_pre_done;
+};
+
+void launch_single_input(genie_ctx* h, hipStream_t st, const int32_t* timesteps, int uniform_ts = 0);
 void launch_gemm_rows(genie_ctx* h, hipStream_t st, const float* A, int lda, int M, int K,
                       const float* Wp, int Nout, const float* bias, const float* res, int ldr,
                       const float* rowmask, int relu, float* out, int ldo, int prof_class = KC_GEMM_ROWS);
@@ -251,6 +251,7 @@
 void launch_triatt(genie_ctx* h, hipStream_t st, const TriAttW& w, bool starting);
 void triatt_ws_floats(const genie_dims_t& d, int B, int N, size_t* tb, size_t* xn, size_t* qkvg);
 bool launch_pair_stack_fused(genie_ctx* h, hipStream_t st, float* tap_trimul_out0, float* tap_layer0);
+bool pair_stack_fused_has_bias(const genie_ctx* h);
 void launch_ipa_bias(genie_ctx* h, hipStream_t st);
 void launch_ipa_prep(genie_ctx* h, hipStream_t st, int b0 = 0, int nb = -1);
 void launch_ipa_attn(genie_ctx* h, hipStream_t st, int layer, const float* head_w, int b0 = 0, int nb = -1);
@@ -265,10 +266,9 @@
 void launch_bb_update(genie_ctx* h, hipStream_t st, const StructLayerW& w, const float* trans_in,
                       float* z_out);
 void launch_frenet(genie_ctx* h, hipStream_t st, int mode, int step, float scale, float* trans,
-                   float* rots, const float* z, const float* eps);
+                   float* rots, const float* z, const float* eps, bool working = false);
 void launch_reverse_step(genie_ctx* h, hipStream_t st, float a, float bz, float c_scaled, float* trans, float* rots, const float* z,
-                         const float* eps);
-void launch_fill_i32(genie_ctx* h, hipStream_t st, int32_t* p, int n, int v);
+                         const float* eps, bool working = false);
 void train_ws_free(genie_ctx* h);
 
 void prof_begin(genie_ctx* h, hipStream_t st, int cls);
diff --git a/genie2_amd/csrc/genie_api.hip b/genie2_amd/csrc/genie_api.hip
--- a/genie2_amd/csrc/genie_api.hip
+++ b/genie2_amd/csrc/genie_api.hip
@@ -114,10 +114,15 @@
         (void)hipDeviceGetStreamPriorityRange(&lo, &hi);
         if (hipStreamCreateWithPriority(&h->st2, hipStreamNonBlocking, hi) != hipSuccess) h->st2 = nullptr;
     }
-    if (h->st2 && (hipEventCreateWithFlags(&h->ev_fork, hipEventDisableTiming) != hipSuccess ||
-                   hipEventCreateWithFlags(&h->ev_join, hipEventDisableTiming) != hipSuccess)) {
-        (void)hipStreamDestroy(h->st2);
-        h->st2 = nullptr;
+    if (h->st2) {
+        hipEvent_t* ev[4] = {&h->ev_fork, &h->ev_join, &h->ev_pre_go, &h->ev_pre_done};
+        int n = 0;
+        while (n < 4 && hipEventCreateWithFlags(ev[n], hipEventDisableTiming) == hipSuccess) ++n;
+        if (n < 4) {
+            while (n > 0) (void)hipEventDestroy(*ev[--n]);
+            (void)hipStreamDestroy(h->st2);
+            h->st2 = nullptr;
+        }
     }
     *out = h;
     return GENIE_OK;
@@ -139,7 +144,8 @@
     free(h->sched_host);
     for (int i = 0; i < h->prof_n; ++i) { (void)hipEventDestroy(h->prof_recs[i].a); (void)hipEventDestroy(h->prof_recs[i].b); }
     free(h->prof_recs);
-    if (h->st2) { (void)hipStreamSynchronize(h->st2); (void)hipEventDestroy(h->ev_fork); (void)hipEventDestroy(h->ev_join); (void)hipStreamDestroy(h->st2); }
+    if (h->st2) { (void)hipStreamSynchronize(h->st2); (void)hipEventDestroy(h->ev_fork); (void)hipEventDestroy(h->ev_join);
+                  (void)hipEventDestroy(h->ev_pre_go); (void)hipEventDestroy(h->ev_pre_done); (void)hipStreamDestroy(h->st2); }
     delete[] h->pair;
     delete[] h->st;
     delete h;
@@ -421,7 +427,7 @@
         }
         slot(&L.pt_w2, img.pack(w2, (int)cp, (int)nh)); slot(&L.pt_b2, img.raw(b2, cp));
     }
-    {
+    auto emit_fused = [&](const std::vector<float>& wb_all) {
         auto ck = [](int kc, int hh, int e) { return 16 * kc + (e & 3) + 8 * (e >> 2) + 4 * hh; };
         auto emit_O = [&](const TmSave& t) {
             for (int which = 0; which < 2; ++which)
@@ -456,9 +462,18 @@
             emit_O(tm_save[2 * l]); emit_P(tm_save[2 * l + 1]);
             hxfix.push_back({&h->pair[l].fb.img, hx.begin()});
             emit_O(tm_save[2 * l + 1]); emit_T(pt_save[l]);
-            if (l + 1 < d.n_pair_transform_layer) emit_P(tm_save[2 * l + 2]);
-        }
-    }
+            h->pair[l].fa.n_bias = 0; h->pair[l].fa.bias_inv_s = 0.f;
+            h->pair[l].fb.n_bias = 0; h->pair[l].fb.bias_inv_s = 0.f;
+            if (l + 1 < d.n_pair_transform_layer) { emit_P(tm_save[2 * l + 2]); continue; }
+            const int LH = d.n_structure_layer * d.n_head_ipa;
+            if (LH > 96 || cp != 128) continue;
+            const float sw = p2floor(16384.0 / max_abs(wb_all.data(), wb_all.size()));
+            for (int blk = 0; blk < 4; ++blk)
+                for (int kc = 0; kc < 8; ++kc)
+                    hx.unit([&](int i, int hh, int e) { const int r = 32 * blk + i; return r < LH ? wb_all[(size_t)r * cp + ck(kc, hh, e)] * sw : 0.f; });
+            h->pair[l].fb.n_bias = LH; h->pair[l].fb.bias_inv_s = 1.0f / sw;
+        }
+    };
     const size_t H = d.n_head_ipa, C = d.c_hidden_ipa, Pq = d.n_qk_point, Pv = d.n_v_point;
     const size_t ncat = ipa_cat_n(d);
     std::vector<float> wb_all, bb_all;
@@ -495,6 +510,7 @@
     }
     pack_gemm(&h->ipa_bias_w, wb_all.data(), (int)(d.n_structure_layer * H), (int)cp);
     slot(&h->ipa_bias_b, img.raw(bb_all.data(), bb_all.size()));
+    emit_fused(wb_all);
     if (c.left != 0) { SET_ERR(h, "genie_load_weights: %zu floats left over", c.left); return GENIE_E_ARG; }
 
     if (h->wdev) { (void)hipFree(h->wdev); h->wdev = nullptr; }
@@ -577,12 +593,12 @@
     want(&h->xsingle, M * ldx * 4);
     want(&h->s0, M * cs * 4); want(&h->s, M * cs * 4); want(&h->s1, M * cs * 4); want(&h->s2, M * cs * 4);
     want(&h->h1, M * cs * 4); want(&h->h2, M * cs * 4);
-    want(&h->pij, M * 2 * cp * 4); want(&h->proj, M * ipa_proj_n(d) * 4); want(&h->cat, M * ipa_cat_n(d) * 4);
+    want(&h->pij, M * 2 * cp * 4); want(&h->pij2, M * 2 * cp * 4); want(&h->proj, M * ipa_proj_n(d) * 4); want(&h->cat, M * ipa_cat_n(d) * 4);
     want(&h->kT, M * H * C * 4); want(&h->v, M * H * C * 4); want(&h->qp, M * H * Pq * 3 * 4);
     want(&h->kpT, M * H * Pq * 3 * 4); want(&h->vp, M * H * Pv * 3 * 4);
     want(&h->vf, ipa_vf_floats(d, B, N) * 4); want(&h->vmax, M * 2 * 4);
     want(&h->rots_w, M * 9 * 4); want(&h->trans_w, M * 3 * 4); want(&h->loop_z, M * 3 * 4);
-    want(&h->tsteps, (size_t)B * 4); want(&h->rmaskf, M * 4); want(&h->pmax, 4); want(&h->spart, 3 * M * cs * 4);
+    want(&h->rmaskf, M * 4); want(&h->pmax, 4); want(&h->spart, 3 * M * cs * 4);
     want(&h->f_aatype, M * 20 * 4); want(&h->f_rmask, M * 4); want(&h->f_ridx, M * 4); want(&h->f_cidx, M * 4);
     want(&h->f_pos, M * 3 * 4); want(&h->f_fsm, M); want(&h->f_fstm, P); want(&h->f_ifm, M);
     if (d.n_head_tri > 0) {
@@ -629,24 +645,51 @@
     return GENIE_OK;
 }
 
+struct LoopHint {
+    int step;
+    bool have_frames;
+    bool have_single;
+    int next_step;
+};
+
+static void timestep_work(genie_ctx* h, hipStream_t st, const int32_t* ts_dev, int ts, float* s_out, float* pij_out) {
+    const genie_dims_t& d = h->d;
+    const int M = h->B * h->N, cs = d.c_s, cp = d.c_p;
+    const int ldx = (single_in(d) + 7) / 8 * 8;
+    launch_single_input(h, st, ts_dev, ts);
+    launch_gemm_rows(h, st, h->xsingle, ldx, M, ldx, h->single_w, cs, nullptr, nullptr, 0, h->rmaskf, 0, s_out, cs);
+    launch_gemm_rows(h, st, s_out, cs, M, cs, h->pij_w, 2 * cp, nullptr, nullptr, 0, nullptr, 0, pij_out, 2 * cp);
+}
+
 static int denoise_internal(genie_ctx* h, hipStream_t st, const float* trans, const float* rots, const int32_t* ts_dev,
-                            const int8_t* codes, float* z_out, const genie_taps_t* taps) {
+                            const int8_t* codes, float* z_out, const genie_taps_t* taps, const LoopHint* hint = nullptr) {
     const genie_dims_t& d = h->d;
     const int B = h->B, N = h->N, M = B * N;
     const size_t P = (size_t)M * N;
     const int cs = d.c_s, cp = d.c_p;
-    const int ldx = (single_in(d) + 7) / 8 * 8;
     auto d2d = [&](void* dst, const void* src, size_t bytes) { return hipMemcpyAsync(dst, src, bytes, hipMemcpyDeviceToDevice, st); };
 
     h->hx_launches = 1;
-    launch_scale_copy(h, st, trans, h->trans_w, M * 3, d.rescale);
-    HIP_TRY(h, d2d(h->rots_w, rots, (size_t)M * 9 * 4));
-
-    launch_single_input(h, st, ts_dev);
-    launch_gemm_rows(h, st, h->xsingle, ldx, M, ldx, h->single_w, cs, nullptr, nullptr, 0, h->rmaskf, 0, h->s0, cs);
-    if (taps && taps->s) HIP_TRY(h, d2d(taps->s, h->s0, (size_t)M * cs * 4));
-
-    launch_gemm_rows(h, st, h->s0, cs, M, cs, h->pij_w, 2 * cp, nullptr, nullptr, 0, nullptr, 0, h->pij, 2 * cp);
+    if (!(hint && hint->have_frames)) {
+        launch_scale_copy(h, st, trans, h->trans_w, M * 3, d.rescale);
+        HIP_TRY(h, d2d(h->rots_w, rots, (size_t)M * 9 * 4));
+    }
+
+    if (hint && hint->have_single) {
+        HIP_TRY(h, hipStreamWaitEvent(st, h->ev_pre_done, 0));
+        std::swap(h->s, h->s0);
+        std::swap(h->pij, h->pij2);
+    } else {
+        timestep_work(h, st, ts_dev, hint ? hint->step : 0, h->s, h->pij);
+    }
+    if (taps && taps->s) HIP_TRY(h, d2d(taps->s, h->s, (size_t)M * cs * 4));
+    if (hint && hint->next_step > 0) {
+        HIP_TRY(h, hipEventRecord(h->ev_pre_go, st));
+        HIP_TRY(h, hipStreamWaitEvent(h->st2, h->ev_pre_go, 0));
+        timestep_work(h, h->st2, nullptr, hint->next_step, h->s0, h->pij2);
+        HIP_TRY(h, hipEventRecord(h->ev_pre_done, h->st2));
+    }
+
     launch_pair_init(h, st, h->trans_w, h->rots_w, codes);
     if (taps && taps->p_init) HIP_TRY(h, d2d(taps->p_init, h->p, P * cp * 4));
 
@@ -665,9 +708,8 @@
     }
     if (taps && taps->p) HIP_TRY(h, d2d(taps->p, h->p, P * cp * 4));
 
-    launch_ipa_bias(h, st);
-    HIP_TRY(h, d2d(h->s, h->s0, (size_t)M * cs * 4));
-    if (taps && taps->states) HIP_TRY(h, d2d(taps->states, h->s0, (size_t)M * cs * 4));
+    if (!(fused && pair_stack_fused_has_bias(h))) launch_ipa_bias(h, st);
+    if (taps && taps->states) HIP_TRY(h, d2d(taps->states, h->s, (size_t)M * cs * 4));
     int n_state = 1;
     const int nproj = ipa_proj_n(d), ncat = ipa_cat_n(d);
     bool split = h->st2 && B >= 2 && M >= 1024 && ipa_attn_splits(h) && !getenv("GENIE_NO_STRUCT_SPLIT");
@@ -801,12 +843,17 @@
         launch_frenet(h, st, 0, 0, 0.f, trans_io, rots_io, nullptr, nullptr);
     }
     int it = 0;
+    LoopHint hint = {0, false, false, 0};
     for (int step = first_step; step >= last_step; --step, ++it) {
-        launch_fill_i32(h, st, h->tsteps, h->B, step);
+        const bool more = step > last_step;
+        hint.step = step;
+        hint.next_step = (more && h->st2) ? step - 1 : 0;
         const int8_t* codes = quat_codes ? quat_codes + (size_t)it * nn : nullptr;
-        if (int rc = denoise_internal(h, st, trans_io, rots_io, h->tsteps, codes, h->loop_z, nullptr)) return rc;
+        if (int rc = denoise_internal(h, st, trans_io, rots_io, nullptr, codes, h->loop_z, nullptr, &hint)) return rc;
         const float* eps = (step == 1) ? nullptr : noise + (size_t)(T - step + 1) * n3;
-        launch_frenet(h, st, 1, step, scale, trans_io, rots_io, h->loop_z, eps);
+        launch_frenet(h, st, 1, step, scale, trans_io, rots_io, h->loop_z, eps, more);
+        hint.have_frames = true;
+        hint.have_single = hint.next_step > 0;
         if (record) HIP_TRY(h, hipMemcpyAsync(record + (size_t)it * n3, trans_io, n3 * 4, hipMemcpyDeviceToDevice, st));
     }
     HIP_TRY(h, hipGetLastError());
@@ -851,12 +898,17 @@
         HIP_TRY(h, hipMemcpyAsync(trans_io, noise, n3 * 4, hipMemcpyDeviceToDevice, st));
         launch_frenet(h, st, 0, 0, 0.f, trans_io, rots_io, nullptr, nullptr);
     }
+    LoopHint hint = {0, false, false, 0};
     for (int it = 0; it < n_iter; ++it) {
-        launch_fill_i32(h, st, h->tsteps, h->B, steps[it]);
+        const bool more = it + 1 < n_iter;
+        hint.step = steps[it];
+        hint.next_step = (more && h->st2) ? steps[it + 1] : 0;
         const int8_t* codes = quat_codes ? quat_codes + (size_t)it * nn : nullptr;
-        if (int rc = denoise_internal(h, st, trans_io, rots_io, h->tsteps, codes, h->loop_z, nullptr)) return rc;
+        if (int rc = denoise_internal(h, st, trans_io, rots_io, nullptr, codes, h->loop_z, nullptr, &hint)) return rc;
         const float* eps = (it == n_iter - 1) ? nullptr : noise + (size_t)(it + 1) * n3;
-        launch_reverse_step(h, st, coef[3 * it], coef[3 * it + 1], coef[3 * it + 2], trans_io, rots_io, h->loop_z, eps);
+        launch_reverse_step(h, st, coef[3 * it], coef[3 * it + 1], coef[3 * it + 2], trans_io, rots_io, h->loop_z, eps, more);
+        hint.have_frames = true;
+        hint.have_single = hint.next_step > 0;
         if (record) HIP_TRY(h, hipMemcpyAsync(record + (size_t)it * n3, trans_io, n3 * 4, hipMemcpyDeviceToDevice, st));
     }
     HIP_TRY(h, hipGetLastError());
diff --git a/genie2_amd/csrc/hx_fused.h b/genie2_amd/csrc/hx_fused.h
--- a/genie2_amd/csrc/hx_fused.h
+++ b/genie2_amd/csrc/hx_fused.h
@@ -18,6 +18,9 @@
     unsigned cm_bytes, z_bytes;
     float sx, cgo, cz, c1, c2, inv_c2, cpa, cpb, cg;
     int rev;
+    const float* bias_b; float* bias_out; unsigned* pmax;
+    int n_bias; unsigned bias_bytes, bias_ostride;
+    float bias_inv_sw;
 };
 
 __device__ __forceinline__ void fz_zt_read(float4 (&raw)[16], const unsigned char* zt, int pl, int h, int half) {
diff --git a/genie2_amd/csrc/pair_fused_kernels.hip b/genie2_amd/csrc/pair_fused_kernels.hip
--- a/genie2_amd/csrc/pair_fused_kernels.hip
+++ b/genie2_amd/csrc/pair_fused_kernels.hip
@@ -15,7 +15,9 @@
     const int rev = A.rev;
     const int n_hb = HAS_T ? A.n_hb : 0;
     const int PBASE = 4 + n_hb;
-    const rsrc_t rw = hx_rsrc(A.wimg, (unsigned)((PBASE + (HAS_P ? 8 : 0)) * HX_STAGE_BYTES));
+    const bool has_b = !HAS_P && A.n_bias > 0;
+    const rsrc_t rw = hx_rsrc(A.wimg, (unsigned)((PBASE + (HAS_P ? 8 : has_b ? 2 : 0)) * HX_STAGE_BYTES));
+    const rsrc_t rbias = hx_rsrc(A.bias_out, has_b ? A.bias_bytes : 0u);
     const rsrc_t rx = hx_rsrc(A.xcm, A.cm_bytes), rz = hx_rsrc(A.z, A.z_bytes);
     const rsrc_t ra = hx_rsrc(A.acm, A.cm_bytes), rb = hx_rsrc(A.bcm, A.cm_bytes);
     const int lane16 = lane * 16;
@@ -55,8 +57,11 @@
         else if (u < FZ_SB_B2) { if (HAS_T && u - FZ_SB_B1 < n_hb * 32) v = A.b1s[u - FZ_SB_B1]; }
         else if (u < FZ_SB_BP) { if (HAS_T) v = A.b2s[u - FZ_SB_B2]; }
         else if (HAS_P) v = A.bproj[u - FZ_SB_BP];
+        else if (has_b && u - FZ_SB_BP < A.n_bias) v = A.bias_b[u - FZ_SB_BP];
         sb[u] = v;
     }
+    if (COL && A.pmax && blockIdx.x == 0 && threadIdx.x == 0) *A.pmax = 0u;
+    float amax = 0.f;
     float4 raw[16];
     {
         int zs, nv, cm;
@@ -213,7 +218,7 @@
 #pragma unroll
             for (int r = 0; r < 16; ++r) d[r] = sbt[FZ_SB_B1 + acc_row(r, lane)];
             auto t_stage = [&](int hb) {
-                if (HAS_P || hb + 1 < n_hb) issue(4 + hb + 1, (hb + 1) & 1);
+                if (HAS_P || has_b || hb + 1 < n_hb) issue(4 + hb + 1, (hb + 1) & 1);
                 else if (more) issue(0, 0);
                 const unsigned char* stage = smb + (hb & 1) * HX_STAGE_BYTES;
                 {
@@ -274,6 +279,79 @@
         hx_lds_done();
         if constexpr (!HAS_P) {
             if (more) hx_zt_dma(rz, zt, lane_t, n_zsoff, zstride, n_nv, 1);
+        }
+
+        if constexpr (!HAS_P) {
+            if (has_b) {
+                float m = 0.f;
+#pragma unroll
+                for (int ob = 0; ob < 4; ++ob)
+#pragma unroll
+                    for (int r = 0; r < 16; ++r) m = fmaxf(m, fabsf(v[ob][r]));
+                m = fmaxf(m, __shfl_xor(m, 32));
+                amax = fmaxf(amax, m);
+                const int ex = (int)((__builtin_bit_cast(unsigned, m) >> 23) & 255u);
+                const bool tiny = ex < 16;
+                const float bsc = tiny ? 1.0f : __builtin_bit_cast(float, (unsigned)(268 - ex) << 23);
+                const float isc = (tiny ? 1.0f : __builtin_bit_cast(float, (unsigned)(ex - 14) << 23)) * A.bias_inv_sw;
+#pragma unroll
+                for (int c = 0; c < 8; ++c) {
+                    float x[8];
+#pragma unroll
+                    for (int e = 0; e < 8; ++e) x[e] = v[c >> 1][8 * (c & 1) + e];
+                    hx_split8(x, bsc, zh[c], zl[c]);
+                }
+                const float* sbias = sbt + FZ_SB_BP;
+                const int ostride = (int)A.bias_ostride;
+                const int bvoff = (pl < nvalid) ? 4 * h * ostride + pl * 4 : FZ_OOR;
+                const int bso = ((b * N + line) * N + t0i) * 4;
+                const int olim = A.n_bias - 4 * h;
+#define FZ_BIAS_STORE(ACC, blk, r) do { const int o_ = (blk) * 32 + ((r) & 3) + 8 * ((r) >> 2);                               \
+        hx_store(rbias, fmaf(ACC[r], isc, sbias[o_ + 4 * h_t]), o_ < olim ? bvoff : FZ_OOR, bso + o_ * ostride); } while (0)
+                f32x16 acc0, acc1, acc2;
+#pragma unroll
+                for (int r = 0; r < 16; ++r) { acc0[r] = 0.f; acc1[r] = 0.f; acc2[r] = 0.f; }
+                {
+                    issue(PBASE + 1, 1);
+                    const unsigned char* stage = smb;
+                    h8 f0 = hx_frag(stage, 0, 0, lane), f0l = hx_frag(stage, 0, 1, lane), f1 = hx_frag(stage, 8, 0, lane),
+                       f1l = hx_frag(stage, 8, 1, lane);
+#pragma unroll
+                    for (int kc = 0; kc < 8; ++kc) {
+                        const int kn = min(kc + 1, 7);
+                        const h8 n0 = hx_frag(stage, kn, 0, lane), n0l = hx_frag(stage, kn, 1, lane), n1 = hx_frag(stage, 8 + kn, 0, lane),
+                                 n1l = hx_frag(stage, 8 + kn, 1, lane);
+                        PIPE_FENCE();
+                        MFH3(f0, f0l, zh[kc], zl[kc], acc0);
+                        MFH3(f1, f1l, zh[kc], zl[kc], acc1);
+                        PIPE_FENCE();
+                        f0 = n0; f0l = n0l; f1 = n1; f1l = n1l;
+                    }
+                    hx_stage_landed();
+                    hx_stage_barrier();
+                }
+                {
+                    if (more) issue(0, 0);
+                    const unsigned char* stage = smb + HX_STAGE_BYTES;
+                    h8 f0 = hx_frag(stage, 0, 0, lane), f0l = hx_frag(stage, 0, 1, lane);
+#pragma unroll
+                    for (int kc = 0; kc < 8; ++kc) {
+                        const int kn = min(kc + 1, 7);
+                        const h8 n0 = hx_frag(stage, kn, 0, lane), n0l = hx_frag(stage, kn, 1, lane);
+                        PIPE_FENCE();
+                        MFH3(f0, f0l, zh[kc], zl[kc], acc2);
+                        PIPE_FENCE();
+                        FZ_BIAS_STORE(acc0, 0, 2 * kc); FZ_BIAS_STORE(acc0, 0, 2 * kc + 1);
+                        FZ_BIAS_STORE(acc1, 1, 2 * kc); FZ_BIAS_STORE(acc1, 1, 2 * kc + 1);
+                        f0 = n0; f0l = n0l;
+                    }
+                    asm volatile("s_waitcnt vmcnt(32)" ::: "memory");
+                    hx_stage_barrier();
+#pragma unroll
+                    for (int r = 0; r < 16; ++r) FZ_BIAS_STORE(acc2, 2, r);
+                }
+#undef FZ_BIAS_STORE
+            }
         }
 
         if constexpr (HAS_P) {
@@ -334,6 +412,13 @@
 #pragma unroll
                 for (int r = 0; r < 16; ++r) HX_PROJ_PIECE_C_NOW(r, t[r], u[r]);
             }
+        }
+    }
+    if constexpr (!HAS_P) {
+        if (has_b) {
+#pragma unroll
+            for (int o = 32; o > 0; o >>= 1) amax = fmaxf(amax, __shfl_xor(amax, o));
+            if (lane == 0 && __float_as_uint(amax) > *reinterpret_cast<volatile unsigned*>(A.pmax)) atomicMax(A.pmax, __float_as_uint(amax));
         }
     }
 #undef FZ_XLOAD
@@ -365,6 +450,13 @@
     a.c1 = t ? t->c1 : 0.f; a.c2 = t ? t->c2 : 1.f; a.inv_c2 = t ? 1.0f / t->c2 : 1.f;
     a.cpa = p.cpa; a.cpb = p.cpb; a.cg = p.cg;
     a.rev = (int)(h->hx_launches++ & 1);
+    a.pmax = h->pmax;
+    a.bias_b = nullptr; a.bias_out = nullptr; a.n_bias = 0; a.bias_bytes = 0; a.bias_ostride = 0; a.bias_inv_sw = 0.f;
+    if (!pp && f.n_bias > 0) {
+        a.n_bias = f.n_bias; a.bias_b = h->ipa_bias_b; a.bias_out = h->ipa_bias; a.bias_inv_sw = f.bias_inv_s;
+        a.bias_ostride = (unsigned)((size_t)h->B * N * N * 4);
+        a.bias_bytes = (unsigned)((size_t)f.n_bias * h->B * N * N * 4);
+    }
     const long long n_tiles = ((long long)a.n_wtiles + 7) / 8;
     const unsigned grid = (unsigned)(n_tiles < fz_num_cu() ? n_tiles : fz_num_cu());
     if (!pp) hipLaunchKernelGGL((k_pair_fused<false, true, false>), dim3(grid), dim3(512), FZ_LDS_BYTES, st, a);
diff --git a/genie2_amd/csrc/pair_hx_kernels.hip b/genie2_amd/csrc/pair_hx_kernels.hip
--- a/genie2_amd/csrc/pair_hx_kernels.hip
+++ b/genie2_amd/csrc/pair_hx_kernels.hip
@@ -765,6 +765,10 @@
     }
     return true;
 }
+bool pair_stack_fused_has_bias(const genie_ctx* h) {
+    const int L = h->d.n_pair_transform_layer;
+    return L >= 1 && h->pair[L - 1].fb.n_bias > 0;
+}
 
 
 #define IB_UNITS 24
diff --git a/genie2_amd/csrc/single_kernels.hip b/genie2_amd/csrc/single_kernels.hip
--- a/genie2_amd/csrc/single_kernels.hip
+++ b/genie2_amd/csrc/single_kernels.hip
@@ -4,7 +4,7 @@
 
 __global__ void k_single_input(float* __restrict__ x, int ldx, const float* __restrict__ pos_tab, int n_pos, int c_pos,
                                const float* __restrict__ chain_tab, int n_chain, int c_chain,
-                               const float* __restrict__ t_tab, int c_t, const int32_t* __restrict__ timesteps,
+                               const float* __restrict__ t_tab, int c_t, const int32_t* __restrict__ timesteps, int uniform_ts,
                                const int32_t* __restrict__ ridx, const int32_t* __restrict__ cidx,
                                const int32_t* __restrict__ aatype, const uint8_t* __restrict__ fsm,
                                const uint8_t* __restrict__ ifm, int N, int n_timestep) {
@@ -13,7 +13,7 @@
     float* xr = x + (size_t)row * ldx;
     const int ri = min(max(ridx[row], 0), n_pos - 1);
     const int ci = min(max(cidx[row], 0), n_chain - 1);
-    const int ts = min(max(timesteps[b], 0), n_timestep);
+    const int ts = min(max(timesteps ? timesteps[b] : uniform_ts, 0), n_timestep);
     const float f = fsm[row] ? 1.f : 0.f;
     const int o1 = c_pos, o2 = o1 + c_chain, o3 = o2 + c_t, o4 = o3 + 20;
     for (int c = threadIdx.x; c < ldx; c += blockDim.x) {
@@ -999,7 +999,8 @@
                                                          const float* __restrict__ z, const float* __restrict__ eps,
                                                          const int32_t* __restrict__ rmask, const int32_t* __restrict__ cidx,
                                                          int N, float alpha, float sqrt_alpha, float somac, float sqrt_beta,
-                                                         float scale, float a, float bz, float c_scaled) {
+                                                         float scale, float a, float bz, float c_scaled,
+                                                         float* __restrict__ trans_w, float* __restrict__ rots_w, float rescale) {
     extern __shared__ __attribute__((aligned(16))) float sm[];
     float* x = sm;
     float* tv = x + 3 * N;
@@ -1023,6 +1024,7 @@
             if (eps) { v = v + scale * sqrt_beta * eps[(size_t)b * N * 3 + u]; v = v * m; }
             x[u] = v;
             tr[u] = v;
+            if (trans_w) trans_w[(size_t)b * N * 3 + u] = v * rescale;
         }
     } else if (mode == 2) {
         for (int u = tid; u < 3 * N; u += 256) {
@@ -1032,6 +1034,7 @@
             if (eps) { v = v + c_scaled * eps[(size_t)b * N * 3 + u]; v = v * m; }
             x[u] = v;
             tr[u] = v;
+            if (trans_w) trans_w[(size_t)b * N * 3 + u] = v * rescale;
         }
     } else {
         for (int u = tid; u < 3 * N; u += 256) x[u] = tr[u];
@@ -1079,12 +1082,11 @@
         }
 #pragma unroll
         for (int q = 0; q < 9; ++q) ro[9 * n + q] = st1[9 * k + q];
-    }
-}
-
-__global__ void k_fill_i32(int32_t* p, int n, int v) {
-    const int i = blockIdx.x * blockDim.x + threadIdx.x;
-    if (i < n) p[i] = v;
+        if (rots_w) {
+#pragma unroll
+            for (int q = 0; q < 9; ++q) rots_w[(size_t)b * N * 9 + 9 * n + q] = st1[9 * k + q];
+        }
+    }
 }
 
 __global__ void k_scale_copy(const float* __restrict__ in, float* __restrict__ out, int n, float s) {
@@ -1548,12 +1550,12 @@
                        (float)(1.0 - b1), (float)b2, (float)(1.0 - b2), (float)eps, (float)(lr / bc1), (float)sqrt(bc2));
 }
 
-void launch_single_input(genie_ctx* h, hipStream_t st, const int32_t* timesteps) {
+void launch_single_input(genie_ctx* h, hipStream_t st, const int32_t* timesteps, int uniform_ts) {
     ProfScope ps(h, st, KC_SINGLE_INPUT);
     const genie_dims_t& d = h->d;
     const int ldx = (d.c_pos_emb + d.c_chain_emb + d.c_timestep_emb + 23 + 7) / 8 * 8;
     hipLaunchKernelGGL(k_single_input, dim3(h->B * h->N), dim3(256), 0, st, h->xsingle, ldx, h->pos_tab, h->n_pos, d.c_pos_emb,
-                       h->chain_tab, h->n_chain, d.c_chain_emb, h->t_tab, d.c_timestep_emb, timesteps, h->f_ridx, h->f_cidx,
+                       h->chain_tab, h->n_chain, d.c_chain_emb, h->t_tab, d.c_timestep_emb, timesteps, uniform_ts, h->f_ridx, h->f_cidx,
                        h->f_aatype, h->f_fsm, h->f_ifm, h->N, d.n_timestep);
 }
 
@@ -1698,7 +1700,7 @@
 }
 
 void launch_frenet(genie_ctx* h, hipStream_t st, int mode, int step, float scale, float* trans, float* rots, const float* z,
-                   const float* eps) {
+                   const float* eps, bool working) {
     ProfScope ps(h, st, KC_P_SAMPLE);
     float al = 1.f, sa = 1.f, so = 1.f, sb = 0.f;
     if (mode == 1) {
@@ -1710,15 +1712,15 @@
     }
     const size_t lds = (size_t)(3 + 3 + 9 + 9) * h->N * sizeof(float);
     hipLaunchKernelGGL(k_p_sample_frenet, dim3(h->B), dim3(256), lds, st, mode, trans, rots, z, eps, h->f_rmask, h->f_cidx, h->N,
-                       al, sa, so, sb, scale, 0.f, 0.f, 0.f);
+                       al, sa, so, sb, scale, 0.f, 0.f, 0.f, working ? h->trans_w : nullptr, working ? h->rots_w : nullptr, h->d.rescale);
 }
 
 void launch_reverse_step(genie_ctx* h, hipStream_t st, float a, float bz, float c_scaled, float* trans, float* rots, const float* z,
-                         const float* eps) {
+                         const float* eps, bool working) {
     ProfScope ps(h, st, KC_P_SAMPLE);
     const size_t lds = (size_t)(3 + 3 + 9 + 9) * h->N * sizeof(float);
     hipLaunchKernelGGL(k_p_sample_frenet, dim3(h->B), dim3(256), lds, st, 2, trans, rots, z, eps, h->f_rmask, h->f_cidx, h->N,
-                       1.f, 1.f, 1.f, 0.f, 0.f, a, bz, c_scaled);
+                       1.f, 1.f, 1.f, 0.f, 0.f, a, bz, c_scaled, working ? h->trans_w : nullptr, working ? h->rots_w : nullptr, h->d.rescale);
 }
 
 int genie_frenet_frames(genie_stream_t stream, int B, int N, const float* coords, const int32_t* chains, const int32_t* mask,
@@ -1729,13 +1731,9 @@
     if (lds > 64 * 1024)
         (void)hipFuncSetAttribute(reinterpret_cast<const void*>(k_p_sample_frenet), hipFuncAttributeMaxDynamicSharedMemorySize, (int)lds);
     hipLaunchKernelGGL(k_p_sample_frenet, dim3(B), dim3(256), lds, (hipStream_t)stream, 0, const_cast<float*>(coords), rots_out,
-                       (const float*)nullptr, (const float*)nullptr, mask, chains, N, 1.f, 1.f, 1.f, 0.f, 0.f, 0.f, 0.f, 0.f);
+                       (const float*)nullptr, (const float*)nullptr, mask, chains, N, 1.f, 1.f, 1.f, 0.f, 0.f, 0.f, 0.f, 0.f,
+                       (float*)nullptr, (float*)nullptr, 1.f);
     return hipGetLastError() == hipSuccess ? GENIE_OK : GENIE_E_HIP;
-}
-
-void launch_fill_i32(genie_ctx* h, hipStream_t st, int32_t* p, int n, int v) {
-    ProfScope ps(h, st, KC_MISC);
-    hipLaunchKernelGGL(k_fill_i32, dim3((n + 255) / 256), dim3(256), 0, st, p, n, v);
 }
 
 void launch_scale_copy(genie_ctx* h, hipStream_t st, const float* in, float* out, int n, float s) {
```

Result: no change. 111.9 batch-steps/s (median of 6 runs) (+1.0%).
